# PeihaoChen/WS-MGMap

Measured on AMD Instinct MI355X. Metric: policy steps/sec (fwd+bwd), CMA batch=8 seq=64, higher is better.
Workload: dtype bf16

## Files before the change

include/wsmgmap.h:

```cpp
#ifndef WSMGMAP_H
#define WSMGMAP_H

#include <stdint.h>

#ifdef __cplusplus
extern "C" {
#endif

typedef void* wsmg_stream_t;

#define WSMG_EINVAL (-1)
#define WSMG_ENOMEM (-2)

int wsmg_abi_version(void);
const char* wsmg_build_info(void);


int wsmg_bev_index(const float* depth, int B, int Hd, int Wd, float depth_scale, int Hf, int Wf, int E,
                   float local_scale, int32_t* lin_idx, wsmg_stream_t stream);

int wsmg_bev_scatter_max(const float* feat, const int32_t* lin_idx, int B, int Cf, int Hf, int Wf, int C,
                         int E, float* out, wsmg_stream_t stream);

int wsmg_bev_rotate(const float* in, const float* heading, float sign, int B, int C, int E, float* out,
                    wsmg_stream_t stream);

int wsmg_map_fuse(const float* ego_rot, float* global_map, const float* gps, const float* masks, int B,
                  int C, int E, int G, float resolution, wsmg_stream_t stream);

int wsmg_bev_scatter_rotate(const float* feat, const int32_t* lin_idx, const float* heading, float sign, int B, int Cf, int Hf,
                            int Wf, int C, int E, float* out_planes, wsmg_stream_t stream);
int wsmg_bev_index_compact(const float* depth, int B, int Hd, int Wd, float depth_scale, int Hf, int Wf, int E, float local_scale,
                           int32_t* lin_idx, uint32_t* clist, int32_t* cnt, wsmg_stream_t stream);
int wsmg_bev_scatter_rotate_compact(const float* feat, const uint32_t* clist, const int32_t* cnt, const float* heading, float sign, int B,
                                    int Cf, int Hf, int Wf, int C, int E, float* out_planes, wsmg_stream_t stream);
int wsmg_map_fuse_planes(const float* ego_rot_planes, float* global_map, const float* gps, const float* masks, int B, int C,
                         int E, int G, float resolution, wsmg_stream_t stream);

int wsmg_map_retrieve(const float* global_map, const float* gps, const float* compass, int B, int C, int E,
                      int G, float resolution, float* scratch, float* out, wsmg_stream_t stream);
int wsmg_map_retrieve_fused(const float* global_map, const float* gps, const float* compass, int B, int C, int E, int G,
                            float resolution, float* out, wsmg_stream_t stream);
int wsmg_map_retrieve_tiled(const float* global_map, const float* gps, const float* compass, int B, int C, int E, int G,
                            float resolution, float* out, wsmg_stream_t stream);

int wsmg_bev_project(const float* depth, const float* feat, const float* heading, float sign, int B, int Hd, int Wd, float depth_scale,
                     int Cf, int Hf, int Wf, int C, int E, float local_scale, int32_t* lin_idx , float* out_planes,
                     wsmg_stream_t stream);
int wsmg_map_fuse_retrieve(const float* ego_rot_planes, float* global_map, const float* gps, const float* compass,
                           const float* masks, int B, int C, int E, int G, float resolution, float* out, wsmg_stream_t stream);

int wsmg_conv2d_fwd(const float* x, const float* w_ohwi, const float* bias, float* y, int B, int H, int W,
                    int Cin, int Cout, int KH, int KW, int stride, int pad, int OH, int OW,
                    wsmg_stream_t stream);

int wsmg_conv2d_bwd_data(const float* dy, const float* w_ihwo, float* dx, int B, int H, int W, int Cin,
                         int Cout, int KH, int KW, int stride, int pad, int OH, int OW,
                         wsmg_stream_t stream);

int wsmg_conv2d_bwd_weight(const float* x, const float* dy, float* dw_ohwi, int B, int H, int W, int Cin,
                           int Cout, int KH, int KW, int stride, int pad, int OH, int OW,
                           wsmg_stream_t stream);

int wsmg_channel_sum(const float* x, int64_t rows, int C, float* out, double* workspace,
                     int64_t workspace_bytes, wsmg_stream_t stream);
int64_t wsmg_channel_reduce_workspace_bytes(int64_t rows, int C);

int wsmg_bn_act_fwd(const float* x, const float* residual, const float* gamma, const float* beta,
                    float* running_mean, float* running_var, float momentum, float eps, int train,
                    int relu, int64_t rows, int C, float* y, float* save_mean, float* save_invstd,
                    double* workspace, int64_t workspace_bytes, wsmg_stream_t stream);

int wsmg_bn_act_bwd(const float* dy, const float* x, const float* y, const float* gamma, const float* beta,
                    const float* save_mean, const float* save_invstd, int relu, int64_t rows, int C,
                    float* dx, float* dresidual, float* dgamma, float* dbeta, double* workspace,
                    int64_t workspace_bytes, wsmg_stream_t stream);

int wsmg_add3_bf16(const void* a, const void* b, const void* c, void* y, int64_t n, wsmg_stream_t stream);

int wsmg_relu_fwd(const float* x, float* y, int64_t n, wsmg_stream_t stream);
int wsmg_token_grad_merge(float* dx, const float* x, const float* g, int B, int I, int C, int relu, wsmg_stream_t stream);
int wsmg_relu_bwd(const float* dy, const float* y, float* dx, int64_t n, wsmg_stream_t stream);
int wsmg_maxpool3x3s2_fwd(const float* x, float* y, int B, int H, int W, int C, int OH, int OW,
                          wsmg_stream_t stream);
int wsmg_maxpool3x3s2_bwd(const float* dy, const float* x, float* dx, int B, int H, int W, int C, int OH,
                          int OW, wsmg_stream_t stream);
int wsmg_upsample2x_fwd(const float* x, float* y, int B, int H, int W, int C, wsmg_stream_t stream);
int wsmg_upsample2x_bwd(const float* dy, float* dx, int B, int H, int W, int C, wsmg_stream_t stream);
int wsmg_avgpool2_fwd(const float* x, float* y, int B, int H, int W, int C, wsmg_stream_t stream);
int wsmg_avgpool2_bwd(const float* dy, float* dx, int B, int H, int W, int C, wsmg_stream_t stream);

int wsmg_nchw_to_nhwc(const float* x, float* y, int B, int C_src, int H, int W, int C_dst,
                      wsmg_stream_t stream);
int wsmg_nhwc_to_nchw(const float* x, float* y, int B, int C_src, int H, int W, int C_dst,
                      wsmg_stream_t stream);

int wsmg_attn_fwd(const float* q, const float* k, const float* v, const uint8_t* mask, float scale, int B,
                  int I, int C, float* out, float* attn, wsmg_stream_t stream);

int wsmg_attn_bwd(const float* q, const float* k, const float* v, const float* attn, const float* dout,
                  const float* dattn, float scale, int B, int I, int C, float* dq, float* dk, float* dv,
                  wsmg_stream_t stream);

int wsmg_conv2d_fwd_bf16(const void* x, const void* w_ohwi, const float* bias, void* y, int out_f32, int B, int H,
                         int W, int Cin, int Cout, int KH, int KW, int stride, int pad, int OH, int OW,
                         wsmg_stream_t stream);
int wsmg_conv2d_splitk_plan(int B, int OH, int OW, int Cin, int Cout, int KH, int KW, int* ksplit, long long* part_floats);
int wsmg_conv2d_fwd_bf16_splitk(const void* x, const void* w_ohwi, const float* bias, void* y, int flags, int ksplit,
                                float* part, int B, int H, int W, int Cin, int Cout, int KH, int KW, int stride, int pad,
                                int OH, int OW, wsmg_stream_t stream);
int wsmg_conv_transpose2d_infer_bf16(const void* x, const void* w_ihwo, const float* bias, void* y, int flags, int B, int H, int W,
                                     int Cin, int Cout, int KH, int KW, int stride, int pad, int OH, int OW, wsmg_stream_t stream);
int wsmg_conv2d_bwd_data_bf16(const void* dy, const void* w_ihwo, void* dx, int out_f32, int B, int H, int W,
                              int Cin, int Cout, int KH, int KW, int stride, int pad, int OH, int OW,
                              wsmg_stream_t stream);
int wsmg_conv2d_fwd_bf16_stats(const void* x, const void* w_ohwi, const float* bias, void* y, int out_f32, double* stats,
                               int nslab, int B, int H, int W, int Cin, int Cout, int KH, int KW, int stride, int pad, int OH,
                               int OW, wsmg_stream_t stream);
int wsmg_conv2d_bwd_data_bf16_stats(const void* dy, const void* w_ihwo, void* dx, int out_f32, double* stats, int nslab, int B,
                                    int H, int W, int Cin, int Cout, int KH, int KW, int stride, int pad, int OH, int OW,
                                    wsmg_stream_t stream);
int wsmg_conv2d_bwd_data_bf16_ex(const void* dy, const void* w_ihwo, void* dx, const void* relu_y, void* dx2, int split_c, int B, int H,
                                 int W, int Cin, int Cout, int KH, int KW, int stride, int pad, int OH, int OW, wsmg_stream_t stream);
int wsmg_conv2d_fwd_bf16_ex(const void* x, const void* w_ohwi, const float* bias, void* y, int flags, double* stats, int nslab, int y_ld,
                            int B, int H, int W, int Cin, int Cout, int KH, int KW, int stride, int pad, int OH, int OW,
                            wsmg_stream_t stream);
typedef struct {
  const float* x;
  float* out;
  int rows, cols;
} WsmgColsumDesc;
int wsmg_colsum_multi(const WsmgColsumDesc* descs, int n, wsmg_stream_t stream);
typedef struct {
  void* dst;
  const void* src;
  long long bytes;
} WsmgCopyDesc;
int wsmg_copy_multi(const WsmgCopyDesc* descs, int n, wsmg_stream_t stream);
int wsmg_copy_multi_guarded(const WsmgCopyDesc* descs, int n, const float* guard, wsmg_stream_t stream);
int wsmg_linear_rows(const float* x, const float* w, const float* bias, float* y, int B, int K, int O, int act, int pool,
                     wsmg_stream_t stream);
int wsmg_act_heads(const float* feat, int B, int K, const float* w_prog, const float* b_prog, const float* w_mean,
                   const float* b_mean, const float* logstd, int A, const float* w_crit, const float* b_crit, const float* noise,
                   float* prog, float* value, float* action, float* logp, wsmg_stream_t stream);
int wsmg_path_kl_fwd(const float* dis, const float* lo, const float* hi, const float* att, int B, int H, int W, int S, float tau,
                     float* target, float* kl, wsmg_stream_t stream);
int wsmg_path_kl_bwd(const float* gkl, const float* target, const float* att, int B, int n, float* datt, wsmg_stream_t stream);

typedef struct {
  float* param;
  const float* grad;
  float* exp_avg;
  float* exp_avg_sq;
  long long n;
} WsmgAdamDesc;
int wsmg_adam_step_multi(const WsmgAdamDesc* descs, int n, float lr, float beta1, float beta2, float eps, float weight_decay,
                         double bias_correction1, double bias_correction2, wsmg_stream_t stream);
int wsmg_adam_step_multi_dev(const WsmgAdamDesc* descs, int n, float lr, float beta1, float beta2, float eps, float weight_decay,
                             const float* step_dev, wsmg_stream_t stream);
int wsmg_grad_norm_multi(const WsmgAdamDesc* descs, int n, double* partials, long long partials_cap, float max_norm,
                         int skip_nonfinite, float* guard, float* step_dev, wsmg_stream_t stream);
int wsmg_adam_step_multi_guarded(const WsmgAdamDesc* descs, int n, float lr, float beta1, float beta2, float eps, float weight_decay,
                                 const float* step_dev, const float* guard, wsmg_stream_t stream);

int wsmg_conv_debug_win3_tile(int mt);
int wsmg_bn_act_fwd_bf16_pre(const void* x, const void* residual, const float* gamma, const float* beta, float* running_mean,
                             float* running_var, float momentum, float eps, int relu, int64_t rows, int C, void* y,
                             float* save_mean, float* save_invstd, double* stats, int nslab, wsmg_stream_t stream);
int wsmg_conv2d_bwd_weight_bf16(const void* x, const void* dy, float* dw_ohwi, int B, int H, int W, int Cin,
                                int Cout, int KH, int KW, int stride, int pad, int OH, int OW,
                                wsmg_stream_t stream);
int wsmg_channel_sum_bf16(const void* x, int64_t rows, int C, float* out, double* workspace,
                          int64_t workspace_bytes, wsmg_stream_t stream);
int wsmg_bn_act_fwd_bf16(const void* x, const void* residual, const float* gamma, const float* beta,
                         float* running_mean, float* running_var, float momentum, float eps, int train,
                         int relu, int64_t rows, int C, void* y, float* save_mean, float* save_invstd,
                         double* workspace, int64_t workspace_bytes, wsmg_stream_t stream);
int wsmg_bn_act_bwd_bf16(const void* dy, const void* x, const void* y, const float* gamma, const float* beta,
                         const float* save_mean, const float* save_invstd, int relu, int64_t rows, int C,
                         void* dx, void* dresidual, float* dgamma, float* dbeta, double* workspace,
                         int64_t workspace_bytes, wsmg_stream_t stream);
int wsmg_relu_fwd_bf16(const void* x, void* y, int64_t n, wsmg_stream_t stream);
int wsmg_token_grad_merge_bf16(void* dx, const void* x, const float* g, int B, int I, int C, int relu, wsmg_stream_t stream);
int wsmg_relu_bwd_bf16(const void* dy, const void* y, void* dx, int64_t n, wsmg_stream_t stream);
int wsmg_maxpool3x3s2_fwd_bf16(const void* x, void* y, int B, int H, int W, int C, int OH, int OW,
                               wsmg_stream_t stream);
int wsmg_maxpool3x3s2_bwd_bf16(const void* dy, const void* x, void* dx, int B, int H, int W, int C, int OH,
                               int OW, wsmg_stream_t stream);
int wsmg_maxpool3x3s2_fwd_idx_bf16(const void* x, void* y, uint32_t* idx, int B, int H, int W, int C, int OH, int OW, wsmg_stream_t stream);
int wsmg_maxpool3x3s2_bwd_idx_bf16(const void* dy, const uint32_t* idx, void* dx, int B, int H, int W, int C, int OH, int OW,
                                   wsmg_stream_t stream);
int wsmg_upsample2x_fwd_bf16(const void* x, void* y, int B, int H, int W, int C, wsmg_stream_t stream);
int wsmg_upsample2x_bwd_bf16(const void* dy, void* dx, int B, int H, int W, int C, wsmg_stream_t stream);
int wsmg_avgpool2_fwd_bf16(const void* x, void* y, int B, int H, int W, int C, wsmg_stream_t stream);
int wsmg_avgpool2_bwd_bf16(const void* dy, void* dx, int B, int H, int W, int C, wsmg_stream_t stream);
int wsmg_nchw_to_nhwc_bf16(const float* x, void* y, int B, int C_src, int H, int W, int C_dst,
                           wsmg_stream_t stream);
int wsmg_nhwc_to_nchw_bf16(const void* x, float* y, int B, int C_src, int H, int W, int C_dst,
                           wsmg_stream_t stream);
int wsmg_attn_fwd_bf16(const float* q, const void* k, const void* v, const uint8_t* mask, float scale, int B,
                       int I, int C, float* out, float* attn, wsmg_stream_t stream);
int wsmg_attn_bwd_bf16(const float* q, const void* k, const void* v, const float* attn, const float* dout,
                       const float* dattn, float scale, int B, int I, int C, float* dq, void* dk, void* dv,
                       wsmg_stream_t stream);

int wsmg_attn_shared_fwd(const float* q, const float* k_sets, const float* v_sets, const uint8_t* mask_sets,
                         const int64_t* row_index, float scale, int B, int I, int C, float* out, float* attn,
                         wsmg_stream_t stream);
int wsmg_attn_shared_bwd(const float* q, const float* k_sets, const float* v_sets, const float* attn, const float* dout,
                         const float* dattn, const int64_t* row_index, float scale, int B, int I, int C, float* dq,
                         float* dlogits, wsmg_stream_t stream);
int wsmg_attn_shared_fwd_bf16(const float* q, const void* k_sets, const void* v_sets, const uint8_t* mask_sets,
                              const int64_t* row_index, float scale, int B, int I, int C, float* out, float* attn,
                              wsmg_stream_t stream);
int wsmg_attn_shared_bwd_bf16(const float* q, const void* k_sets, const void* v_sets, const float* attn, const float* dout,
                              const float* dattn, const int64_t* row_index, float scale, int B, int I, int C, float* dq,
                              float* dlogits, wsmg_stream_t stream);

int wsmg_attn_fp8_row_fwd(const float* q, const float* w_k, const uint8_t* x_e4m3, const float* x_scale, const int* lengths,
                          float scale, int B, int L, int C, float* q_folded, float* out, float* attn, wsmg_stream_t stream);
int wsmg_attn_fp8_fold(const float* in, const float* w, int B, int C, int transpose, float* out, wsmg_stream_t stream);
int wsmg_attn_fp8_splits(int B, int L);
int64_t wsmg_attn_fp8_workspace_bytes(int B, int L);
int wsmg_attn_fp8_fwd(const float* q_folded, const uint8_t* x_e4m3, const float* x_scale, const int* lengths, float scale, int B,
                      int L, int C, float* out, float* attn, void* workspace, unsigned* ticket, wsmg_stream_t stream);
int wsmg_attn_fp8_bwd(const float* q_folded, const uint8_t* x_e4m3, const float* x_scale, const float* attn, const float* dout,
                      const float* dattn, float scale, int B, int L, int C, float* dq_folded, float* dx, wsmg_stream_t stream);
int wsmg_quantize_e4m3_dev(const float* x, int64_t n, const float* scale, uint8_t* y, wsmg_stream_t stream);
int wsmg_quantize_e4m3(const float* x, int64_t n, float inv_scale, uint8_t* y, wsmg_stream_t stream);

#define WSMG_RELAYOUT_MAX 32
typedef struct {
  const float* w_oihw;
  void* w_ohwi;
  void* w_ihwo;
  int O, I, KH, KW, I_pad, reserved;
} WsmgRelayoutDesc;
int wsmg_weight_relayout_multi(const WsmgRelayoutDesc* descs, int n, int bf16, wsmg_stream_t stream);
int wsmg_weight_relayout(const float* w_oihw, int O, int I, int KH, int KW, int I_pad, float* w_ohwi, float* w_ihwo,
                         wsmg_stream_t stream);
int wsmg_weight_relayout_bf16(const float* w_oihw, int O, int I, int KH, int KW, int I_pad, void* w_ohwi, void* w_ihwo,
                              wsmg_stream_t stream);
int wsmg_weight_grad_to_oihw(const float* dw_ohwi, int O, int I, int KH, int KW, int I_pad, float* dw_oihw,
                             wsmg_stream_t stream);

int wsmg_conv2d_bwd_weight_bf16_plan(int B, int H, int W, int Cin, int Cout, int KH, int KW, int stride, int pad, int OH, int OW,
                                     int* nsplit, long long* ws_floats);
int wsmg_conv2d_bwd_weight_bf16_slabs(const void* x, const void* dy, float* ws, int nsplit, long long ws_floats, int B, int H, int W,
                                      int Cin, int Cout, int KH, int KW, int stride, int pad, int OH, int OW, wsmg_stream_t stream);
int wsmg_conv2d_bwd_weight_plan(int B, int H, int W, int Cin, int Cout, int KH, int KW, int stride, int pad, int OH, int OW,
                                int* nsplit, long long* ws_floats);
int wsmg_conv2d_bwd_weight_slabs(const float* x, const float* dy, float* ws, int nsplit, long long ws_floats, int B, int H, int W,
                                 int Cin, int Cout, int KH, int KW, int stride, int pad, int OH, int OW, wsmg_stream_t stream);
int wsmg_weight_grad_reduce_oihw(const float* ws, int nsplit, int O, int I, int KH, int KW, int I_pad, float* dw_oihw,
                                 wsmg_stream_t stream);

int wsmg_bn_act_bwd_ld(const float* dy, int64_t ld_dy, const float* x, const float* y, const float* gamma, const float* beta,
                       const float* save_mean, const float* save_invstd, int relu, int64_t rows, int C, float* dx, float* dresidual,
                       float* dgamma, float* dbeta, double* workspace, int64_t workspace_bytes, wsmg_stream_t stream);
int wsmg_bn_act_bwd_ld_bf16(const void* dy, int64_t ld_dy, const void* x, const void* y, const float* gamma, const float* beta,
                            const float* save_mean, const float* save_invstd, int relu, int64_t rows, int C, void* dx,
                            void* dresidual, float* dgamma, float* dbeta, double* workspace, int64_t workspace_bytes,
                            wsmg_stream_t stream);
int wsmg_bn_act_bwd_ld_bf16_lo(const void* dy, int64_t ld_dy, const void* x, const void* y, const float* gamma, const float* beta,
                               const float* save_mean, const float* save_invstd, int relu, int64_t rows, int C, void* dx, void* dx_lo,
                               void* dresidual, float* dgamma, float* dbeta, double* workspace, int64_t workspace_bytes,
                               wsmg_stream_t stream);
int wsmg_relu_bwd_rows_bf16(const void* dy, int64_t ld_dy, const void* y, void* dx, int64_t rows, int C, wsmg_stream_t stream);
int wsmg_upsample2x_bwd_ld(const float* dy, int64_t ld_dy, float* dx, int B, int H, int W, int C, wsmg_stream_t stream);
int wsmg_upsample2x_bwd_ld_bf16(const void* dy, int64_t ld_dy, void* dx, int B, int H, int W, int C, wsmg_stream_t stream);
int wsmg_cat_channels(const void* a, const void* b, void* y, int64_t rows, int bytes_a, int bytes_b, wsmg_stream_t stream);
int wsmg_upsample2x_cat_bf16(const void* a, const void* b, void* y, int B, int H, int W, int Ca, int Cb, wsmg_stream_t stream);

int wsmg_ce_nhwc_fwd(const float* logits, const int64_t* target, int64_t rows, int classes, float* loss, wsmg_stream_t stream);
int wsmg_ce_nhwc_bwd(const float* logits, const int64_t* target, const float* gloss, int64_t rows, int classes,
                     float* dlogits, wsmg_stream_t stream);
int wsmg_ce_nhwc_fwd_bf16(const void* logits, const int64_t* target, int64_t rows, int classes, float* loss, wsmg_stream_t stream);
int wsmg_ce_nhwc_bwd_bf16(const void* logits, const int64_t* target, const float* gloss, int64_t rows, int classes,
                          void* dlogits, wsmg_stream_t stream);

int wsmg_collate_pad(const void* const* src, const int* lengths, int N, int T, int64_t elems, int src_dtype,
                     float pad, float* dst, wsmg_stream_t stream);
int wsmg_collate_pad_nhwc_bf16(const void* const* src, const int* lengths, int N, int T, int C, int HW, float pad, void* dst,
                               wsmg_stream_t stream);
int wsmg_collate_ego_sparse_nhwc_bf16(const void* const* bits, const void* const* off, const void* const* base,
                                      const void* const* vals, const int* lengths, int N, int T, int C, int HW, float pad,
                                      void* dst, wsmg_stream_t stream);
int wsmg_ego_sparse_pack(const float* x, int B, int C, int HW, uint8_t* bits, uint32_t* off, int64_t* nnz, void* vals,
                         wsmg_stream_t stream);

int64_t wsmg_gru_workspace_bytes(int T);
int wsmg_gru_fwd(const float* gi, const float* w_hh, const float* b_hh, const float* h0, const float* masks,
                 int T, int N, int hidden, float* y, float* save_r, float* save_z, float* save_n,
                 float* save_ghn, void* sync_ws, wsmg_stream_t stream);
int wsmg_gru_bwd(const float* dy, const float* dhT, const float* w_hh, const float* h0, const float* masks,
                 const float* y, const float* save_r, const float* save_z, const float* save_n,
                 const float* save_ghn, int T, int N, int hidden, float* dgi, float* dgh, float* dh0,
                 void* sync_ws, wsmg_stream_t stream);
int wsmg_gru_fwd_owned(const float* gi, const float* w_hh, const float* b_hh, const float* h0, const float* masks,
                       int T, int N, int hidden, float* y, float* save_r, float* save_z, float* save_n,
                       float* save_ghn, void* sync_ws, wsmg_stream_t stream);
int wsmg_gru_bwd_owned(const float* dy, const float* dhT, const float* w_hh, const float* h0, const float* masks,
                       const float* y, const float* save_r, const float* save_z, const float* save_n, const float* save_ghn,
                       int T, int N, int hidden, float* dgi, float* dgh, float* dh0, void* sync_ws, wsmg_stream_t stream);

int64_t wsmg_lstm_state_workspace_bytes(int T);
int wsmg_lstm_state_fwd(const float* gi, const float* w_hh, const float* b_hh, const float* h0, const float* c0,
                        const float* masks, int T, int N, int hidden, float* y, float* c_T, float* save_gates,
                        float* save_c, void* sync_ws, wsmg_stream_t stream);
int wsmg_lstm_state_bwd(const float* dy, const float* dhT, const float* dcT, const float* w_hh, const float* c0,
                        const float* masks, const float* save_gates, const float* save_c, int T, int N, int hidden,
                        float* dgates, float* dh0, float* dc0, void* sync_ws, wsmg_stream_t stream);

#define WSMG_CELL_LSTM 0
#define WSMG_CELL_GRU 1
int64_t wsmg_instr_rnn_workspace_bytes(int cell, int hidden, int dirs, int L);
int wsmg_instr_rnn_fwd(int cell, const float* gi, const float* w_hh, const float* b_hh, const int32_t* lengths, int U, int L,
                       int hidden, int dirs, float* out, float* save_gates, float* save_c, void* state_ws,
                       wsmg_stream_t stream);
int wsmg_instr_rnn_bwd(int cell, const float* dout, const float* w_hh, const int32_t* lengths, const float* out,
                       const float* save_gates, const float* save_c, int U, int L, int hidden, int dirs, float* dgi,
                       float* dgh, void* state_ws, wsmg_stream_t stream);
int64_t wsmg_lstm_workspace_bytes(int L);
int wsmg_lstm_fwd(const float* gi, const float* w_hh, const float* b_hh, const int32_t* lengths, int U, int L,
                  int hidden, float* out, float* save_gates, float* save_c, void* state_ws,
                  wsmg_stream_t stream);
int wsmg_lstm_bwd(const float* dout, const float* w_hh, const int32_t* lengths, const float* save_gates,
                  const float* save_c, int U, int L, int hidden, float* dgates, void* state_ws,
                  wsmg_stream_t stream);

int wsmg_group_norm_nhwc_bf16(const void* x, int x_f32, const void* residual, const float* gamma, const float* beta, int B,
                              int HW, int C, int G, float eps, int relu, void* y, wsmg_stream_t stream);

int wsmg_rnn_status(int clear);
int wsmg_rnn_debug_inject(unsigned bits);
int wsmg_gru_fwd_chain(const float* gi, const float* w_hh, const float* b_hh, const float* h0, const float* masks,
                       int T, int N, int hidden, float* y, float* save_r, float* save_z, float* save_n,
                       float* save_ghn, void* sync_ws, int steps_per_chunk, const unsigned* in_count, unsigned in_target,
                       unsigned* out_count, wsmg_stream_t stream);
int wsmg_gru_bwd_chain(const float* dy, const float* dhT, const float* w_hh, const float* h0, const float* masks,
                       const float* y, const float* save_r, const float* save_z, const float* save_n,
                       const float* save_ghn, int T, int N, int hidden, float* dgi, float* dgh, float* dh0,
                       void* sync_ws, int steps_per_chunk, const unsigned* in_count, unsigned in_target, unsigned* out_count,
                       wsmg_stream_t stream);
int wsmg_gru_chain_workgroups(void);
int wsmg_lstm_state_fwd_chain(const float* gi, const float* w_hh, const float* b_hh, const float* h0, const float* c0,
                              const float* masks, int T, int N, int hidden, float* y, float* c_T, float* save_gates,
                              float* save_c, void* sync_ws, int steps_per_chunk, const unsigned* in_count, unsigned in_target,
                              unsigned* out_count, wsmg_stream_t stream);
int wsmg_lstm_state_bwd_chain(const float* dy, const float* dhT, const float* dcT, const float* w_hh, const float* c0,
                              const float* masks, const float* save_gates, const float* save_c, int T, int N, int hidden,
                              float* dgates, float* dh0, float* dc0, void* sync_ws, int steps_per_chunk, const unsigned* in_count,
                              unsigned in_target, unsigned* out_count, wsmg_stream_t stream);
int wsmg_lstm_state_chain_workgroups(void);
int wsmg_rnn_debug_spin_limit(unsigned limit);

int wsmg_update_heads_fwd(const float* x, const float* wm, const float* bm, const float* wp, const float* bp, const float* progress,
                          int B, int K, int A, float* pred, float* prog, float* prog_rows, wsmg_stream_t stream);
int wsmg_update_heads_bwd(const float* x, const float* wm, const float* wp, const float* prog, const float* progress,
                          const float* dpred, const float* dprog, const float* dprog_rows, int B, int K, int A, float* dx, float* dwm,
                          float* dbm, float* dwp, float* dbp, wsmg_stream_t stream);
int wsmg_aux_reduce_fwd(const float* const* rows, const float* alpha, int L, const unsigned char* mask, int B, float* out2,
                        wsmg_stream_t stream);
int wsmg_aux_reduce_bwd(const float* alpha, int L, const unsigned char* mask, const float* nsel, const float* daux, int B,
                        float* drows, wsmg_stream_t stream);
int wsmg_dagger_loss_fwd(const float* pred, const float* waypoint, int ld_waypoint, const float* weights, const float* aux, int T,
                         int N, int A, float* out2, float* den, wsmg_stream_t stream);
int wsmg_dagger_loss_bwd(const float* pred, const float* waypoint, int ld_waypoint, const float* weights, const float* den,
                         const float* dloss, int T, int N, int A, float* dpred, wsmg_stream_t stream);

long long wsmg_cls_tail_workspace_floats(int B);
int wsmg_cls_tail_fwd_bf16(const void* y2, const float* gamma, const float* beta, const float* mean, const float* invstd,
                           const float* w6, const float* b6, int classes, const float* gt, int Hg, int Wg, int B, int H, int W,
                           void* sem, void* pooled, float* ce_rows, wsmg_stream_t stream);
int wsmg_cls_tail_bwd_bf16(const void* y2, const float* gamma, const float* beta, const float* mean, const float* invstd,
                           const float* w6, const float* b6, int classes, const float* gt, int Hg, int Wg, const float* g_rows,
                           const void* dpooled, int B, int H, int W, void* dbn, float* workspace, long long workspace_floats,
                           float* dgamma, float* dbeta, float* dw6, float* db6, wsmg_stream_t stream);
int wsmg_bn_stats_finalize(double* stats, int nslab, int C, int64_t rows, float momentum, float eps, float* running_mean,
                           float* running_var, float* save_mean, float* save_invstd, wsmg_stream_t stream);
int wsmg_bn_bwd_apply_bf16(const void* dy, const void* x, const float* gamma, const float* mean, const float* invstd,
                           const float* dgamma, const float* dbeta, int64_t rows, int C, void* dx, wsmg_stream_t stream);

int wsmg_attn_fp8_mfma_fwd(const uint8_t* q_codes, const float* q_scale, const uint8_t* k_codes, const float* k_scale,
                           const uint8_t* v_codes, const float* v_scale, const int* lengths, const int* row_ids,
                           const int* set_start, float scale, int B, int U, int L, int C, float* out, float* attn,
                           wsmg_stream_t stream);

int wsmg_attn_fp8_mfma_bwd(const uint8_t* q_codes, const float* q_scale, const uint8_t* k_codes, const float* k_scale,
                           const uint8_t* v_codes, const float* v_scale, const int* row_ids, const int* set_start,
                           const int64_t* inverse, const float* attn, const float* dout, const float* dattn, float scale, int B, int U,
                           int L, int C, float* dq, float* dk, float* dv, float* dl_scratch, wsmg_stream_t stream);

int wsmg_attn_fp8_prep(const float* q, const float* k_sets, const float* v_sets, const int64_t* inverse, int B, int U, int L, int C,
                       float q_scale, float k_scale, float v_scale, uint8_t* q_codes, uint8_t* k_codes, uint8_t* v_codes,
                       float* scales, int* row_ids, int* set_start, unsigned* amax_ws, wsmg_stream_t stream);

int wsmg_attn_fp8_mfma_fused(const float* q, const float* k_sets, const float* v_sets, const int64_t* inverse, const int* lengths,
                             float q_scale, float k_scale, float v_scale, float scale, int B, int U, int L, int C,
                             unsigned* workspace, unsigned arrivals_before, int epoch, float* scales_out, float* out, float* attn,
                             wsmg_stream_t stream);
int wsmg_attn_fp8_mfma_fused_arrivals(int B, int U, int L, int C);

int wsmg_mean_rows(const float* x, int64_t R, int n, float* out, wsmg_stream_t stream);

int wsmg_instruction_dedup(const void* tokens, int is_f32, int B, int L, long long* uniq, long long* inverse, long long* meta,
                           wsmg_stream_t stream);

int wsmg_rows_gemm_f32(const float* a0, int lda0, int ka0, const float* a1, int lda1, int ka1, const float* a2, int lda2, int ka2,
                       const float* w, int ldw, int w_is_kn, const float* bias, const float* mask, int ldmask, int relu,
                       float* c0, int ldc0, int nc0, float* c1, int ldc1, int nc1, float* c2, int ldc2, int nc2,
                       const float* cin0, int ldcin0, const float* cin1, int ldcin1, const float* cin2, int ldcin2,
                       int M, const unsigned* wait_count, unsigned wait_target, unsigned* signal_count, int fail_bit,
                       unsigned* gate_word, wsmg_stream_t stream);
int wsmg_rows_gemm_supported(int K);
int wsmg_rows_gemm_workgroups(int M, int N);

int wsmg_debug_occupy(int n_workgroups, int lds_bytes, int max_ms, const int* stop_flag, unsigned* arrived, wsmg_stream_t stream);

#ifdef __cplusplus
}
#endif
#endif
```

ws-mgmap_amd/csrc/wsmg_conv_bf16.hip:

```cpp
#include <stdlib.h>

#include "wsmg_common.h"
#include "wsmg_relu_mask.h"

namespace {

typedef __bf16 bf16_t;
typedef short bf16x8 __attribute__((ext_vector_type(8)));
typedef short bf16x4 __attribute__((ext_vector_type(4)));
typedef unsigned int u32x4 __attribute__((ext_vector_type(4)));

constexpr int BM = 128;

__device__ __forceinline__ int xcd_swizzle(int bid, int nb) {
  const int q = nb >> 3, r = nb & 7, x = bid & 7;
  return x * q + (x < r ? x : r) + (bid >> 3);
}

__device__ __forceinline__ unsigned short f2bf_bits(float f) {
  bf16_t b = (bf16_t)f;
  return __builtin_bit_cast(unsigned short, b);
}

__device__ __forceinline__ __amdgpu_buffer_rsrc_t make_rsrc(const void* p, unsigned bytes) {
  return __builtin_amdgcn_make_buffer_rsrc(const_cast<void*>(p), 0, (int)bytes, 0x00020000);
}
__device__ __forceinline__ u32x4 buf_load16(__amdgpu_buffer_rsrc_t r, int byte_off) {
  return __builtin_amdgcn_raw_buffer_load_b128(r, byte_off, 0, 0);
}

struct ConvArgsB {
  const bf16_t* src;
  const bf16_t* wt;
  const float* bias;
  void* dst;
  int B, SH, SW, Kc, TH, TW, N, KH, KW, stride, pad;
  int mtiles, ntiles;
  int out_f32;
  unsigned src_bytes, wt_bytes;
  double* stats;
  int nslab;
  int ksplit;
  float* part;
  int dst_ld;
  const bf16_t* relu_z;
  void* dst2;
  int split_c;
};

template <bool BWD, int BN, int BK, int PF, bool SPLIT = false>
__global__ __launch_bounds__(256) void conv_igemm_bf16_kernel(ConvArgsB a) {
  constexpr int LDB = BK * 2 + 16;
  constexpr int SEGS = BK / 8;
  constexpr int RPP = 256 / SEGS;
  constexpr int APASS = BM / RPP;
  constexpr int BPASS = BN / RPP;
  constexpr int NT = BN / 64;
  constexpr int OPITCH = BN * 2 + 16;
  constexpr int SMEM = (BM + BN) * LDB > BM * OPITCH ? (BM + BN) * LDB : BM * OPITCH;
  __shared__ __attribute__((aligned(16))) unsigned char smem[SMEM];
  unsigned char* const As = smem;
  unsigned char* const Bs = smem + BM * LDB;
  __shared__ int dpix[BM];
  const int tid = threadIdx.x;
  const int lane = tid & 63, wave = tid >> 6;
  const int tiles = a.mtiles * a.ntiles;
  const int swz = xcd_swizzle(blockIdx.x, gridDim.x);
  const int split = SPLIT ? swz / tiles : 0;
  const int logical = SPLIT ? swz - split * tiles : swz;
  const int m0 = (logical / a.ntiles) * BM, n0 = (logical % a.ntiles) * BN;
  const int seg = tid % SEGS;
  const int lrow = tid / SEGS;

  int cy = 0, cx = 0, ty0 = 0, tx0 = 0, tstep = 1, THc = a.TH, TWc = a.TW, KHc = a.KH, KWc = a.KW;
  if (BWD && a.stride == 2) {
    cy = blockIdx.y >> 1; cx = blockIdx.y & 1;
    ty0 = (cy + a.pad) & 1; tx0 = (cx + a.pad) & 1;
    tstep = 2;
    THc = (a.TH - ty0 + 1) >> 1; TWc = (a.TW - tx0 + 1) >> 1;
    KHc = (a.KH - cy + 1) >> 1; KWc = (a.KW - cx + 1) >> 1;
  }
  const int Mc = a.B * THc * TWc;
  if (m0 >= Mc) return;

  const int sg = BWD ? -1 : 1;
  int roff[APASS];
  unsigned ymask[APASS], xmask[APASS];
  int rb_ = (m0 + lrow) / (THc * TWc);
  int ry_, rx_;
  {
    const int r0 = (m0 + lrow) - rb_ * (THc * TWc);
    ry_ = r0 / TWc;
    rx_ = r0 - ry_ * TWc;
  }
#pragma unroll
  for (int i = 0; i < APASS; ++i) {
    int m = m0 + lrow + RPP * i;
    bool pv = m < Mc;
    const int b = pv ? rb_ : 0, iy = pv ? ry_ : 0, ix = pv ? rx_ : 0;
    rx_ += RPP;
    while (rx_ >= TWc) { rx_ -= TWc; ++ry_; }
    while (ry_ >= THc) { ry_ -= THc; ++rb_; }
    int ty = ty0 + iy * tstep, tx = tx0 + ix * tstep;
    int py, px;
    if (BWD) {
      py = (a.stride == 2) ? ((ty + a.pad - cy) >> 1) : ty + a.pad;
      px = (a.stride == 2) ? ((tx + a.pad - cx) >> 1) : tx + a.pad;
    } else {
      py = ty * a.stride - a.pad;
      px = tx * a.stride - a.pad;
    }
    auto tapmask = [&](int p, int S_, int n) -> unsigned {
      int lo = BWD ? p - (S_ - 1) : -p, hi = BWD ? p : S_ - 1 - p;
      lo = lo < 0 ? 0 : lo;
      hi = hi > n - 1 ? n - 1 : hi;
      return hi >= lo ? ((2u << hi) - 1u) & ~((1u << lo) - 1u) : 0u;
    };
    const unsigned ym = tapmask(py, a.SH, KHc), xm = tapmask(px, a.SW, KWc);
    ymask[i] = pv ? ym : 0u;
    xmask[i] = xm;
    roff[i] = ((b * a.SH + py) * a.SW + px) * a.Kc + seg * 8;
    if (seg == 0) dpix[lrow + RPP * i] = pv ? (b * a.TH + ty) * a.TW + tx : -1;
  }
  const int taps = a.KH * a.KW;
  int woff[BPASS];
#pragma unroll
  for (int i = 0; i < BPASS; ++i) {
    int n = n0 + lrow + RPP * i;
    woff[i] = n < a.N ? n * taps * a.Kc + seg * 8 : -0x40000000;
  }
  const int kchunks = a.Kc / BK;
  const int all_steps = KHc * KWc * kchunks;
  const int per_split = SPLIT ? (all_steps + a.ksplit - 1) / a.ksplit : all_steps;
  const int step_begin = split * per_split;
  const int steps = SPLIT ? (all_steps - step_begin < per_split ? all_steps - step_begin : per_split) : all_steps;
  const __amdgpu_buffer_rsrc_t rs_src = make_rsrc(a.src, a.src_bytes);
  const __amdgpu_buffer_rsrc_t rs_wt = make_rsrc(a.wt, a.wt_bytes);

  int it_ch = 0, it_ay = 0, it_ax = 0, it_left = steps;
  if (SPLIT) {
    const int tp = KHc * KWc;
    it_ch = step_begin / tp;
    const int rem = step_begin - it_ch * tp;
    it_ay = rem / KWc;
    it_ax = rem - it_ay * KWc;
  }
  u32x4 ra[PF][APASS], rb[PF][BPASS];
  auto gload = [&](u32x4 (&ra)[APASS], u32x4 (&rb)[BPASS]) {
    const int ky = BWD ? cy + it_ay * tstep : it_ay, kx = BWD ? cx + it_ax * tstep : it_ax;
    const int sdelta = sg * (it_ay * a.SW + it_ax) * a.Kc + it_ch * BK;
    const bool more = SPLIT ? it_left > 0 : it_ch < kchunks;
    if (SPLIT) --it_left;
    const int wdelta = more ? (ky * a.KW + kx) * a.Kc + it_ch * BK : -0x20000000;
    const unsigned live = more ? 1u : 0u;
#pragma unroll
    for (int i = 0; i < APASS; ++i) {
      bool ok = ((ymask[i] >> it_ay) & (xmask[i] >> it_ax) & live) != 0;
      ra[i] = buf_load16(rs_src, ok ? (roff[i] + sdelta) * 2 : -1);
    }
#pragma unroll
    for (int i = 0; i < BPASS; ++i) rb[i] = buf_load16(rs_wt, (woff[i] + wdelta) * 2);
    if (++it_ax == KWc) { it_ax = 0; if (++it_ay == KHc) { it_ay = 0; ++it_ch; } }
  };
  auto lstore = [&](const u32x4 (&ra)[APASS], const u32x4 (&rb)[BPASS]) {
#pragma unroll
    for (int i = 0; i < APASS; ++i) *reinterpret_cast<u32x4*>(&As[(lrow + RPP * i) * LDB + seg * 16]) = ra[i];
#pragma unroll
    for (int i = 0; i < BPASS; ++i) *reinterpret_cast<u32x4*>(&Bs[(lrow + RPP * i) * LDB + seg * 16]) = rb[i];
  };

  const int wm = (wave & 1) * 64, wn = (wave >> 1) * (BN / 2);
  const int r = lane & 31, h = lane >> 5;
  f32x16 acc[2][NT];
#pragma unroll
  for (int t = 0; t < 2; ++t)
#pragma unroll
    for (int u = 0; u < NT; ++u)
#pragma unroll
      for (int i = 0; i < 16; ++i) acc[t][u][i] = 0.f;

  gload(ra[0], rb[0]);
  lstore(ra[0], rb[0]);
  __syncthreads();
#pragma unroll
  for (int j = 1; j < PF; ++j) gload(ra[j], rb[j]);
  for (int step0 = 0; step0 < steps; step0 += PF) {
#pragma unroll
    for (int j = 0; j < PF; ++j) {
      gload(ra[j], rb[j]);
#pragma unroll
      for (int ks = 0; ks < BK / 16; ++ks) {
        bf16x8 af[2], bf[NT];
#pragma unroll
        for (int t = 0; t < 2; ++t)
          af[t] = *reinterpret_cast<const bf16x8*>(&As[(wm + 32 * t + r) * LDB + ks * 32 + h * 16]);
#pragma unroll
        for (int u = 0; u < NT; ++u)
          bf[u] = *reinterpret_cast<const bf16x8*>(&Bs[(wn + 32 * u + r) * LDB + ks * 32 + h * 16]);
#pragma unroll
        for (int t = 0; t < 2; ++t)
#pragma unroll
          for (int u = 0; u < NT; ++u)
            acc[t][u] = __builtin_amdgcn_mfma_f32_32x32x16_bf16(af[t], bf[u], acc[t][u], 0, 0, 0);
      }
      __syncthreads();
      lstore(ra[(j + 1) % PF], rb[(j + 1) % PF]);
      __syncthreads();
    }
  }

  if (SPLIT) {
    float* const mine = a.part + (size_t)split * Mc * a.N;
#pragma unroll
    for (int u = 0; u < NT; ++u) {
      const int n = n0 + wn + 32 * u + r;
      if (n >= a.N) continue;
#pragma unroll
      for (int t = 0; t < 2; ++t)
#pragma unroll
        for (int g = 0; g < 16; ++g) {
          const int m = m0 + wm + 32 * t + (g & 3) + 8 * (g >> 2) + 4 * h;
          if (m < Mc) mine[(size_t)m * a.N + n] = acc[t][u][g];
        }
    }
    return;
  }

  constexpr int OP = OPITCH;
  {
    if ((a.out_f32 & 1) == 0 && (a.N & 7) == 0) {
      const bool relu_here = (a.out_f32 & 6) == 2;
#pragma unroll
      for (int u = 0; u < NT; ++u) {
        const int col = wn + 32 * u + r;
        const float bv = (a.bias && n0 + col < a.N) ? a.bias[n0 + col] : 0.f;
        float sv = 0.f, qv = 0.f;
#pragma unroll
        for (int t = 0; t < 2; ++t)
#pragma unroll
          for (int g = 0; g < 16; ++g) {
            const int row = wm + 32 * t + (g & 3) + 8 * (g >> 2) + 4 * h;
            float v = acc[t][u][g] + bv;
            if (relu_here) v = v > 0.f ? v : 0.f;
            const unsigned short o = f2bf_bits(v);
            *reinterpret_cast<unsigned short*>(smem + row * OP + col * 2) = o;
            if (a.stats) {
              const float vr = m0 + row < Mc ? __uint_as_float((unsigned)o << 16) : 0.f;
              sv += vr;
              qv = fmaf(vr, vr, qv);
            }
          }
        if (a.stats) {
          sv += __shfl_xor(sv, 32, 64);
          qv += __shfl_xor(qv, 32, 64);
          if (h == 0 && n0 + col < a.N) {
            double* st = a.stats + (size_t)((logical / a.ntiles) % a.nslab) * 2 * a.N + n0 + col;
            atomicAdd(st, (double)sv);
            atomicAdd(st + a.N, (double)qv);
          }
        }
      }
      __syncthreads();
      constexpr int CPR = BN / 8;
      const int ldd = a.dst_ld ? a.dst_ld : a.N;
      constexpr int ROWS = BM * CPR / 256;
      u32x4 zr[ROWS];
      if (a.relu_z) {
#pragma unroll
        for (int j = 0; j < ROWS; ++j) {
          const int c = tid + 256 * j;
          const int row = c / CPR, ch = c - row * CPR;
          const int dp = dpix[row];
          const int n = n0 + ch * 8;
          zr[j] = (dp >= 0 && n < a.N) ? *reinterpret_cast<const u32x4*>(a.relu_z + (size_t)dp * a.N + n) : u32x4{0u, 0u, 0u, 0u};
        }
      }
#pragma unroll
      for (int j = 0; j < BM * CPR / 256; ++j) {
        const int c = tid + 256 * j;
        const int row = c / CPR, ch = c - row * CPR;
        const int dp = dpix[row];
        const int n = n0 + ch * 8;
        if (dp < 0 || n >= a.N) continue;
        u32x4* out = reinterpret_cast<u32x4*>(reinterpret_cast<unsigned char*>(a.dst) + ((size_t)dp * ldd + n) * 2);
        if (a.dst2) {
          const bool hi = n >= a.split_c;
          out = reinterpret_cast<u32x4*>(reinterpret_cast<unsigned char*>(hi ? a.dst2 : a.dst) +
                                         ((size_t)dp * (hi ? a.N - a.split_c : a.split_c) + (hi ? n - a.split_c : n)) * 2);
        }
        u32x4 v = *reinterpret_cast<const u32x4*>(smem + row * OP + ch * 16);
        if (a.relu_z) v = relu_mask8(v, zr[j]);
        if (a.out_f32 & 4) {
          const u32x4 old = *out;
#pragma unroll
          for (int q = 0; q < 4; ++q) {
            float lo = __uint_as_float(v[q] << 16) + __uint_as_float(old[q] << 16);
            float hi = __uint_as_float(v[q] & 0xffff0000u) + __uint_as_float(old[q] & 0xffff0000u);
            if (a.out_f32 & 2) { lo = lo > 0.f ? lo : 0.f; hi = hi > 0.f ? hi : 0.f; }
            v[q] = (unsigned)f2bf_bits(lo) | ((unsigned)f2bf_bits(hi) << 16);
          }
        }
        *out = v;
      }
      return;
    }
  }
#pragma unroll
  for (int u = 0; u < NT; ++u) {
    const int n = n0 + wn + 32 * u + r;
    if (n >= a.N) continue;
    const float bv = a.bias ? a.bias[n] : 0.f;
#pragma unroll
    for (int t = 0; t < 2; ++t) {
#pragma unroll
      for (int g = 0; g < 16; ++g) {
        int row = wm + 32 * t + (g & 3) + 8 * (g >> 2) + 4 * h;
        int dp = dpix[row];
        if (dp < 0) continue;
        float v = acc[t][u][g] + bv;
        if (a.out_f32 & 4) {
          const size_t o = (size_t)dp * a.N + n;
          v += (a.out_f32 & 1) ? reinterpret_cast<const float*>(a.dst)[o]
                               : __uint_as_float((unsigned)reinterpret_cast<const unsigned short*>(a.dst)[o] << 16);
        }
        if (a.out_f32 & 2) v = v > 0.f ? v : 0.f;
        if (a.out_f32 & 1)
          reinterpret_cast<float*>(a.dst)[(size_t)dp * a.N + n] = v;
        else
          reinterpret_cast<unsigned short*>(a.dst)[(size_t)dp * a.N + n] = f2bf_bits(v);
      }
    }
  }
}

constexpr int WKP = 64;
constexpr int X_LD = 64;

struct WgradArgsB {
  const bf16_t* x;
  const bf16_t* dy;
  float* dw;
  int B, H, W, Cin, Cout, KH, KW, stride, pad, OH, OW;
  int units;
  int64_t npix, chunk;
  unsigned x_bytes, dy_bytes;
  int gx, gy;
  int64_t slab;
};

__device__ __forceinline__ bf16x4 tr_read(const unsigned char* p) {
  return __builtin_amdgcn_ds_read_tr16_b64_v4i16((bf16x4 __attribute__((address_space(3)))*)(p));
}

template <int TC, int TU, int PF, int UPT>
__global__ __launch_bounds__(256) void conv_wgrad_bf16_kernel(WgradArgsB a) {
  constexpr int WCO = 32 * TC;
  constexpr int WUN = 4 * TU;
  constexpr int NG = WUN / UPT;
  constexpr int D_LD = TC == 4 ? 320 : 192;
  constexpr int DSEG = 4 * TC;
  constexpr int DROWS = 256 / DSEG;
  __shared__ __attribute__((aligned(16))) unsigned char Ds[WKP * D_LD];
  __shared__ __attribute__((aligned(16))) unsigned char Xs[WUN * WKP * X_LD];
  const int tid = threadIdx.x;
  const int lane = tid & 63, wave = tid >> 6;
  const int logical = xcd_swizzle(blockIdx.x, gridDim.x);
  const int gxy = a.gx * a.gy;
  const int bz = logical / gxy, bxy = logical - bz * gxy;
  const int u0 = (bxy % a.gx) * WUN;
  const int co0 = (bxy / a.gx) * WCO;
  const int64_t p_begin = (int64_t)bz * a.chunk;
  int64_t p_end = p_begin + a.chunk;
  if (p_end > a.npix) p_end = a.npix;
  const int cchunks = a.Cin / 32;
  const int ohw = a.OH * a.OW;

  int gky[NG], gkx[NG], gci[NG];
  bool gok[NG];
#pragma unroll
  for (int g = 0; g < NG; ++g) {
    int uu = u0 + g * UPT;
    gok[g] = uu < a.units;
    int t = gok[g] ? uu / cchunks : 0;
    gci[g] = gok[g] ? (uu - t * cchunks) * 32 : 0;
    gky[g] = t / a.KW;
    gkx[g] = t - gky[g] * a.KW;
  }
  const int dpx = tid / DSEG, dseg = tid % DSEG;
  const int xpx = tid >> 2, xseg = tid & 3;

  f32x16 acc[TC][TU];
#pragma unroll
  for (int t = 0; t < TC; ++t)
#pragma unroll
    for (int u = 0; u < TU; ++u)
#pragma unroll
      for (int i = 0; i < 16; ++i) acc[t][u][i] = 0.f;

  const __amdgpu_buffer_rsrc_t rs_x = make_rsrc(a.x, a.x_bytes);
  const __amdgpu_buffer_rsrc_t rs_dy = make_rsrc(a.dy, a.dy_bytes);
  const bool co_ok = (co0 + dseg * 8) < a.Cout;
  int gdelta[NG];
#pragma unroll
  for (int g = 0; g < NG; ++g) gdelta[g] = (gky[g] * a.W + gkx[g]) * a.Cin + gci[g] + xseg * 8;
  int it_b, it_oy, it_ox;
  {
    int64_t p = p_begin + xpx;
    if (p >= a.npix) p = a.npix - 1;
    it_b = (int)(p / ohw);
    int rem = (int)(p - (int64_t)it_b * ohw);
    it_oy = rem / a.OW;
    it_ox = rem - it_oy * a.OW;
  }
  const int adv_b = WKP / ohw, adv_rem = WKP - adv_b * ohw;
  const int adv_oy = adv_rem / a.OW, adv_ox = adv_rem - adv_oy * a.OW;
  int it_p = (int)p_begin;
  const int pend = (int)p_end;
  u32x4 rd[PF][TC], rx[PF][WUN];
  auto gload = [&](u32x4 (&rd)[TC], u32x4 (&rx)[WUN]) {
#pragma unroll
    for (int i = 0; i < TC; ++i) {
      int p = it_p + dpx + DROWS * i;
      bool ok = co_ok && p < pend;
      rd[i] = buf_load16(rs_dy, ok ? (p * a.Cout + co0 + dseg * 8) * 2 : -1);
    }
    const bool pok = (it_p + xpx) < pend;
    const int y0 = it_oy * a.stride - a.pad, x0 = it_ox * a.stride - a.pad;
    const int base = ((it_b * a.H + y0) * a.W + x0) * a.Cin;
#pragma unroll
    for (int g = 0; g < NG; ++g) {
      bool ok = pok && gok[g] && (unsigned)(y0 + gky[g]) < (unsigned)a.H && (unsigned)(x0 + gkx[g]) < (unsigned)a.W;
      const int off = ok ? (base + gdelta[g]) * 2 : (int)0x80000000;
#pragma unroll
      for (int j = 0; j < UPT; ++j) rx[g * UPT + j] = buf_load16(rs_x, off + 64 * j);
    }
    it_p += WKP;
    it_ox += adv_ox;
    if (it_ox >= a.OW) { it_ox -= a.OW; ++it_oy; }
    it_oy += adv_oy;
    if (it_oy >= a.OH) { it_oy -= a.OH; ++it_b; }
    it_b += adv_b;
  };
  auto lstore = [&](const u32x4 (&rd)[TC], const u32x4 (&rx)[WUN]) {
#pragma unroll
    for (int i = 0; i < TC; ++i) *reinterpret_cast<u32x4*>(&Ds[(dpx + DROWS * i) * D_LD + dseg * 16]) = rd[i];
#pragma unroll
    for (int u = 0; u < WUN; ++u) *reinterpret_cast<u32x4*>(&Xs[(u * WKP + xpx) * X_LD + xseg * 16]) = rx[u];
  };

  const int li = lane & 15, q = li >> 2, p4 = li & 3;
  const int half16 = (lane >> 4) & 1;
  const int h = lane >> 5;
  const unsigned char* a_base = &Ds[(8 * h + q) * D_LD + (half16 * 16 + p4 * 4) * 2];
  const unsigned char* b_base = &Xs[(wave * TU * WKP + 8 * h + q) * X_LD + (half16 * 16 + p4 * 4) * 2];

  gload(rd[0], rx[0]);
  lstore(rd[0], rx[0]);
  __syncthreads();
#pragma unroll
  for (int j = 1; j < PF; ++j) gload(rd[j], rx[j]);
  for (int64_t pb = p_begin; pb < p_end; pb += (int64_t)PF * WKP) {
#pragma unroll
    for (int j = 0; j < PF; ++j) {
      gload(rd[j], rx[j]);
#pragma unroll
      for (int ks = 0; ks < WKP / 16; ++ks) {
        bf16x8 af[TC], bfr[TU];
#pragma unroll
        for (int t = 0; t < TC; ++t) {
          bf16x4 l = tr_read(a_base + 64 * t + (16 * ks) * D_LD), hh = tr_read(a_base + 64 * t + (16 * ks + 4) * D_LD);
          af[t] = __builtin_shufflevector(l, hh, 0, 1, 2, 3, 4, 5, 6, 7);
        }
#pragma unroll
        for (int u = 0; u < TU; ++u) {
          const unsigned char* bp = b_base + u * WKP * X_LD;
          bf16x4 l = tr_read(bp + (16 * ks) * X_LD), hh = tr_read(bp + (16 * ks + 4) * X_LD);
          bfr[u] = __builtin_shufflevector(l, hh, 0, 1, 2, 3, 4, 5, 6, 7);
        }
#pragma unroll
        for (int u = 0; u < TU; ++u)
#pragma unroll
          for (int t = 0; t < TC; ++t) acc[t][u] = __builtin_amdgcn_mfma_f32_32x32x16_bf16(af[t], bfr[u], acc[t][u], 0, 0, 0);
      }
      __syncthreads();
      lstore(rd[(j + 1) % PF], rx[(j + 1) % PF]);
      __syncthreads();
    }
  }
  const int r = lane & 31;
  const int taps = a.KH * a.KW;
#pragma unroll
  for (int u = 0; u < TU; ++u) {
    const int uu = u0 + wave * TU + u;
    if (uu >= a.units) continue;
    const int tap = uu / cchunks;
    const int ci = (uu - tap * cchunks) * 32 + r;
#pragma unroll
    for (int t = 0; t < TC; ++t) {
#pragma unroll
      for (int g = 0; g < 16; ++g) {
        int co = co0 + 32 * t + (g & 3) + 8 * (g >> 2) + 4 * h;
        if (co < a.Cout) {
          float* const q = a.dw + (size_t)bz * a.slab + ((size_t)co * taps + tap) * a.Cin + ci;
          if (a.slab) *q = acc[t][u][g];
          else atomicAdd(q, acc[t][u][g]);
        }
      }
    }
  }
}

int check_conv(int B, int H, int W, int Cin, int Cout, int KH, int KW, int stride, int pad, int OH, int OW) {
  if (B <= 0 || H <= 0 || W <= 0 || Cin <= 0 || Cout <= 0 || KH <= 0 || KW <= 0) return WSMG_EINVAL;
  if (Cin % 32 || Cout % 32) return WSMG_EINVAL;
  if (stride != 1 && stride != 2) return WSMG_EINVAL;
  if (OH != (H + 2 * pad - KH) / stride + 1 || OW != (W + 2 * pad - KW) / stride + 1) return WSMG_EINVAL;
  if ((int64_t)B * H * W >= (1ll << 31) || (int64_t)B * OH * OW >= (1ll << 31)) return WSMG_EINVAL;
  if ((int64_t)B * H * W * Cin * 2 >= (1ll << 31) || (int64_t)B * OH * OW * Cout * 2 >= (1ll << 31)) return WSMG_EINVAL;
  return 0;
}


int g_win3_tile = -1;
int win3_tile() {
  if (g_win3_tile < 0) g_win3_tile = WSMG_TUNE("WSMG_CONV_WIN3", 1);
  return g_win3_tile;
}
bool k32_choice(int64_t M, int Kc, int N) {
  return win3_tile() == 1 && Kc == 32 && (N == 32 || N == 64 || N == 128) && M >= 2 * 256 * 256 && WSMG_TUNE("WSMG_CONV_K32", 1) != 0;
}
int win3_choice(int64_t M, int Kc, int N) {
  const int t = win3_tile();
  if (t == 0 || M < 256 * 256 || Kc % 32 || N % 32) return 0;
  if (N % 64) {
    const int n32 = WSMG_TUNE("WSMG_CONV_WIN3_N32", 256);
    if (t != 1) return t;
    if (n32 == 0 || M < 2 * 256 * 256) return 0;
    return n32;
  }
  if (Kc < 64) return 0;
  if (N % 128) {
    const int n64 = WSMG_TUNE("WSMG_CONV_WIN3_N64", 1);
    if (t != 1) return t;
    if (n64 == 0 || M < 2 * 256 * 256 || (Kc < 128 && N < 192)) return 0;
    return n64 == 1 ? 512 : n64;
  }
  if (t != 1) return t;
  if (M < 2 * 256 * 256) return 0;
  return ((M + 511) / 512) * (N / 128) >= 1024 ? 512 : 256;
}

template <bool BWD>
int launch_igemm(ConvArgsB& a, int64_t mrows, int classes, hipStream_t s) {
  const bool bk64 = (a.Kc % 64) == 0;
  const bool bn128 = a.N >= 128;
  const int bn = bn128 ? 128 : 64;
  a.mtiles = (int)wsmg_cdiv(mrows, BM);
  a.ntiles = (int)wsmg_cdiv(a.N, bn);
  dim3 grid((unsigned)(a.mtiles * a.ntiles), (unsigned)classes);
  if (bk64 && bn128)
    hipLaunchKernelGGL((conv_igemm_bf16_kernel<BWD, 128, 64, 1>), grid, dim3(256), 0, s, a);
  else if (bk64)
    hipLaunchKernelGGL((conv_igemm_bf16_kernel<BWD, 64, 64, 1>), grid, dim3(256), 0, s, a);
  else if (bn128)
    hipLaunchKernelGGL((conv_igemm_bf16_kernel<BWD, 128, 32, 1>), grid, dim3(256), 0, s, a);
  else
    hipLaunchKernelGGL((conv_igemm_bf16_kernel<BWD, 64, 32, 1>), grid, dim3(256), 0, s, a);
  return 0;
}

int splitk_plan(int64_t M, int Kc, int N, int KH, int KW) {
  const int bk = (Kc % 64) == 0 ? 64 : 32;
  const int steps = KH * KW * (Kc / bk);
  const int tiles = (int)(wsmg_cdiv(M, BM) * wsmg_cdiv(N, 64));
  const int target = 256, minsteps = 4, maxtiles = 128;
  if (tiles >= maxtiles || steps < 4 * minsteps || (N & 7)) return 1;
  int ks = (int)wsmg_cdiv(target, tiles);
  if (ks > steps / minsteps) ks = steps / minsteps;
  if (ks > 32) ks = 32;
  if (ks < 2) return 1;
  const int per = (int)wsmg_cdiv(steps, ks);
  return (int)wsmg_cdiv(steps, per);
}

__global__ __launch_bounds__(256) void splitk_finish_kernel(const float* __restrict__ part, const float* __restrict__ bias,
                                                            void* __restrict__ y, int64_t MN8, int N, int ksplit, int flags) {
  const int64_t i = (int64_t)blockIdx.x * 256 + threadIdx.x;
  if (i >= MN8) return;
  typedef float f32x4v __attribute__((ext_vector_type(4)));
  const int n = (int)((i * 8) % N);
  float v[8];
#pragma unroll
  for (int j = 0; j < 8; ++j) v[j] = 0.f;
  const f32x4v* p = reinterpret_cast<const f32x4v*>(part) + i * 2;
  for (int s = 0; s < ksplit; ++s, p += MN8 * 2) {
    const f32x4v a0 = p[0], a1 = p[1];
#pragma unroll
    for (int j = 0; j < 4; ++j) { v[j] += a0[j]; v[4 + j] += a1[j]; }
  }
  if (bias) {
#pragma unroll
    for (int j = 0; j < 8; ++j) v[j] += bias[n + j];
  }
  if (flags & 1) {
    f32x4v* o = reinterpret_cast<f32x4v*>(y) + i * 2;
    if (flags & 4) {
      const f32x4v a0 = o[0], a1 = o[1];
#pragma unroll
      for (int j = 0; j < 4; ++j) { v[j] += a0[j]; v[4 + j] += a1[j]; }
    }
    if (flags & 2) {
#pragma unroll
      for (int j = 0; j < 8; ++j) v[j] = v[j] > 0.f ? v[j] : 0.f;
    }
    o[0] = f32x4v{v[0], v[1], v[2], v[3]};
    o[1] = f32x4v{v[4], v[5], v[6], v[7]};
  } else {
    u32x4* o = reinterpret_cast<u32x4*>(y) + i;
    if (flags & 4) {
      const u32x4 old = *o;
#pragma unroll
      for (int j = 0; j < 4; ++j) {
        v[2 * j] += __uint_as_float(old[j] << 16);
        v[2 * j + 1] += __uint_as_float(old[j] & 0xffff0000u);
      }
    }
    u32x4 out;
#pragma unroll
    for (int j = 0; j < 4; ++j) {
      float lo = v[2 * j], hi = v[2 * j + 1];
      if (flags & 2) { lo = lo > 0.f ? lo : 0.f; hi = hi > 0.f ? hi : 0.f; }
      out[j] = (unsigned)f2bf_bits(lo) | ((unsigned)f2bf_bits(hi) << 16);
    }
    *o = out;
  }
}

}

extern "C" int wsmg_conv2d_splitk_plan(int B, int OH, int OW, int Cin, int Cout, int KH, int KW, int* ksplit,
                                       long long* part_floats) {
  if (!ksplit || !part_floats) return WSMG_EINVAL;
  *ksplit = splitk_plan((int64_t)B * OH * OW, Cin, Cout, KH, KW);
  *part_floats = (long long)*ksplit * B * OH * OW * Cout;
  return 0;
}

extern "C" int wsmg_conv2d_fwd_bf16_splitk(const void* x, const void* w_ohwi, const float* bias, void* y, int flags, int ksplit,
                                           float* part, int B, int H, int W, int Cin, int Cout, int KH, int KW,
                                           int stride, int pad, int OH, int OW, wsmg_stream_t stream) {
  if (int e = check_conv(B, H, W, Cin, Cout, KH, KW, stride, pad, OH, OW)) return e;
  const int64_t M = (int64_t)B * OH * OW;
  if (ksplit < 2 || ksplit != splitk_plan(M, Cin, Cout, KH, KW) || !part || (flags & ~7)) return WSMG_EINVAL;
  ConvArgsB a{(const bf16_t*)x, (const bf16_t*)w_ohwi, nullptr, y, B, H, W, Cin, OH, OW, Cout, KH, KW, stride, pad, 0, 0, flags,
              (unsigned)((size_t)B * H * W * Cin * 2), (unsigned)((size_t)Cout * KH * KW * Cin * 2), nullptr, 0, ksplit, part};
  a.mtiles = (int)wsmg_cdiv(M, BM);
  a.ntiles = (int)wsmg_cdiv(Cout, 64);
  dim3 grid((unsigned)(a.mtiles * a.ntiles * ksplit));
  if (Cin % 64 == 0)
    hipLaunchKernelGGL((conv_igemm_bf16_kernel<false, 64, 64, 1, true>), grid, dim3(256), 0, wsmg_s(stream), a);
  else
    hipLaunchKernelGGL((conv_igemm_bf16_kernel<false, 64, 32, 1, true>), grid, dim3(256), 0, wsmg_s(stream), a);
  const int64_t mn8 = M * Cout / 8;
  hipLaunchKernelGGL(splitk_finish_kernel, dim3((unsigned)wsmg_cdiv(mn8, 256)), dim3(256), 0, wsmg_s(stream), part, bias, y, mn8,
                     Cout, ksplit, flags);
  WSMG_RETURN_LAUNCH();
}

namespace {
int conv_fwd_bf16_impl(const void* x, const void* w_ohwi, const float* bias, void* y, int out_f32, double* stats, int nslab, int y_ld, int B, int H, int W, int Cin, int Cout, int KH, int KW, int stride, int pad,
                       int OH, int OW, wsmg_stream_t stream) {
  if (int e = check_conv(B, H, W, Cin, Cout, KH, KW, stride, pad, OH, OW)) return e;
  if (stats && (nslab <= 0 || (out_f32 & 5) != 0 || (Cout & 7) != 0)) return WSMG_EINVAL;
  const bool ex = y_ld && y_ld != Cout;
  if (ex) {
    if ((out_f32 & 5) != 0 || (Cout & 7) != 0) return WSMG_EINVAL;
    if (y_ld && (y_ld < Cout || (y_ld & 7) || ((uintptr_t)y & 15))) return WSMG_EINVAL;
    if ((int64_t)B * OH * OW * (y_ld ? y_ld : Cout) * 2 >= (1ll << 31)) return WSMG_EINVAL;
  }
  if (!ex && Cin == 64 && Cout == 64 && KH == 8 && KW == 8 && stride == 2 && pad == 3 && (out_f32 & 5) == 0) {
    if (WSMG_TUNE("WSMG_CONV_WIN", 1)) {
      int rc = wsmg_conv_win_fwd_bf16(x, w_ohwi, bias, y, (out_f32 & 2) != 0, stats, nslab, B, H, W, Cin, Cout, KH, KW, stride, pad, OH, OW, wsmg_s(stream));
      if (rc != WSMG_EINVAL) return rc;
    }
  }
  if (KH == 3 && KW == 3 && stride == 1 && pad == 1 && OH == H && OW == W && (out_f32 & 5) == 0) {
    if (k32_choice((int64_t)B * OH * OW, Cin, Cout)) {
      int rc = wsmg_conv_win3_k32_bf16(0, x, w_ohwi, bias, y, (out_f32 & 2) != 0, stats, nslab, B, H, W, Cout, y_ld, wsmg_s(stream));
      if (rc != WSMG_EINVAL) return rc;
    }
    if (const int mt = win3_choice((int64_t)B * OH * OW, Cin, Cout)) {
      int rc = wsmg_conv_win3_bf16(0, x, w_ohwi, bias, y, (out_f32 & 2) != 0, stats, nslab, B, H, W, Cin, Cout, mt, win3_tile() == 1, nullptr, y_ld, nullptr, 0, wsmg_s(stream));
      if (rc != WSMG_EINVAL) return rc;
    }
  }
  ConvArgsB a{(const bf16_t*)x, (const bf16_t*)w_ohwi, bias, y, B, H, W, Cin, OH, OW, Cout, KH, KW, stride, pad, 0, 0, out_f32,
              (unsigned)((size_t)B * H * W * Cin * 2), (unsigned)((size_t)Cout * KH * KW * Cin * 2), stats, nslab};
  a.dst_ld = y_ld;
  if (int e = launch_igemm<false>(a, (int64_t)B * OH * OW, 1, wsmg_s(stream))) return e;
  WSMG_RETURN_LAUNCH();
}
}

extern "C" int wsmg_conv2d_fwd_bf16_stats(const void* x, const void* w_ohwi, const float* bias, void* y, int out_f32,
                                          double* stats, int nslab, int B, int H, int W, int Cin, int Cout, int KH, int KW,
                                          int stride, int pad, int OH, int OW, wsmg_stream_t stream) {
  return conv_fwd_bf16_impl(x, w_ohwi, bias, y, out_f32, stats, nslab, 0, B, H, W, Cin, Cout, KH, KW, stride, pad, OH, OW, stream);
}

extern "C" int wsmg_conv2d_fwd_bf16_ex(const void* x, const void* w_ohwi, const float* bias, void* y, int flags, double* stats, int nslab,
                                       int y_ld, int B, int H, int W, int Cin, int Cout, int KH, int KW,
                                       int stride, int pad, int OH, int OW, wsmg_stream_t stream) {
  return conv_fwd_bf16_impl(x, w_ohwi, bias, y, flags, stats, nslab, y_ld, B, H, W, Cin, Cout, KH, KW, stride, pad, OH, OW, stream);
}

extern "C" int wsmg_conv_debug_win3_tile(int mt) {
  const int old = win3_tile();
  if (mt == 0 || mt == 1 || mt == 256 || mt == 512) g_win3_tile = mt;
  return old;
}

extern "C" int wsmg_conv2d_fwd_bf16(const void* x, const void* w_ohwi, const float* bias, void* y, int out_f32, int B,
                                    int H, int W, int Cin, int Cout, int KH, int KW, int stride, int pad, int OH,
                                    int OW, wsmg_stream_t stream) {
  return wsmg_conv2d_fwd_bf16_stats(x, w_ohwi, bias, y, out_f32, nullptr, 0, B, H, W, Cin, Cout, KH, KW, stride, pad, OH, OW, stream);
}

namespace {
int conv_bwd_data_bf16_impl(const void* dy, const void* w_ihwo, void* dx, int out_f32, double* stats, int nslab, const void* relu_y,
                            void* dx2, int split_c, int B, int H, int W, int Cin, int Cout, int KH, int KW, int stride, int pad, int OH,
                            int OW, wsmg_stream_t stream) {
  if (int e = check_conv(B, H, W, Cin, Cout, KH, KW, stride, pad, OH, OW)) return e;
  if (stats && (nslab <= 0 || (out_f32 & 5) != 0 || (Cin & 7) != 0)) return WSMG_EINVAL;
  if (relu_y && ((out_f32 & 5) != 0 || (Cin & 7) != 0 || ((uintptr_t)relu_y & 15))) return WSMG_EINVAL;
  if (dx2 && ((out_f32 & 5) != 0 || (Cin & 7) != 0 || split_c <= 0 || split_c >= Cin || (split_c & 7) || ((uintptr_t)dx2 & 15))) return WSMG_EINVAL;
  if (KH == 3 && KW == 3 && stride == 1 && pad == 1 && OH == H && OW == W && (out_f32 & 7) == 0) {
    if (!relu_y && !dx2 && k32_choice((int64_t)B * H * W, Cout, Cin)) {
      int rc = wsmg_conv_win3_k32_bf16(1, dy, w_ihwo, nullptr, dx, 0, stats, nslab, B, H, W, Cin, 0, wsmg_s(stream));
      if (rc != WSMG_EINVAL) return rc;
    }
    if (const int mt = win3_choice((int64_t)B * H * W, Cout, Cin)) {
      int rc = wsmg_conv_win3_bf16(1, dy, w_ihwo, nullptr, dx, 0, stats, nslab, B, H, W, Cout, Cin, mt, win3_tile() == 1, relu_y, 0, dx2, split_c, wsmg_s(stream));
      if (rc != WSMG_EINVAL) return rc;
    }
  }
  if (KH == 4 && KW == 4 && stride == 2 && pad == 1 && Cin == 32 && Cout == 64 && H == 2 * OH && W == 2 * OW && (out_f32 & 7) == 0 &&
      !relu_y && !dx2 && win3_tile() == 1 && (int64_t)B * OH * OW >= 2 * 256 * 256 && WSMG_TUNE("WSMG_CONVT_K4S2", 1) != 0) {
    int rc = wsmg_convt_k4s2_bf16(dy, w_ihwo, dx, stats, nslab, B, OH, OW, wsmg_s(stream));
    if (rc != WSMG_EINVAL) return rc;
  }
  ConvArgsB a{(const bf16_t*)dy, (const bf16_t*)w_ihwo, nullptr, dx, B, OH, OW, Cout, H, W, Cin, KH, KW, stride, pad, 0, 0, out_f32,
              (unsigned)((size_t)B * OH * OW * Cout * 2), (unsigned)((size_t)Cout * KH * KW * Cin * 2), stats, nslab};
  a.relu_z = (const bf16_t*)relu_y;
  a.dst2 = dx2;
  a.split_c = split_c;
  int classes = 1;
  int64_t mmax = (int64_t)B * H * W;
  if (stride == 2) {
    classes = 4;
    mmax = (int64_t)B * ((H + 1) / 2) * ((W + 1) / 2);
  }
  if (int e = launch_igemm<true>(a, mmax, classes, wsmg_s(stream))) return e;
  WSMG_RETURN_LAUNCH();
}
}

extern "C" int wsmg_conv2d_bwd_data_bf16_stats(const void* dy, const void* w_ihwo, void* dx, int out_f32, double* stats, int nslab,
                                               int B, int H, int W, int Cin, int Cout, int KH, int KW, int stride, int pad,
                                               int OH, int OW, wsmg_stream_t stream) {
  return conv_bwd_data_bf16_impl(dy, w_ihwo, dx, out_f32, stats, nslab, nullptr, nullptr, 0, B, H, W, Cin, Cout, KH, KW, stride, pad, OH, OW, stream);
}

extern "C" int wsmg_conv2d_bwd_data_bf16_ex(const void* dy, const void* w_ihwo, void* dx, const void* relu_y, void* dx2, int split_c,
                                            int B, int H, int W, int Cin, int Cout, int KH, int KW, int stride, int pad, int OH, int OW,
                                            wsmg_stream_t stream) {
  return conv_bwd_data_bf16_impl(dy, w_ihwo, dx, 0, nullptr, 0, relu_y, dx2, split_c, B, H, W, Cin, Cout, KH, KW, stride, pad, OH, OW, stream);
}

extern "C" int wsmg_conv_transpose2d_infer_bf16(const void* x, const void* w_ihwo, const float* bias, void* y, int flags, int B,
                                                int H, int W, int Cin, int Cout, int KH, int KW, int stride, int pad, int OH,
                                                int OW, wsmg_stream_t stream) {
  if (int e = check_conv(B, H, W, Cin, Cout, KH, KW, stride, pad, OH, OW)) return e;
  if (flags & ~3) return WSMG_EINVAL;
  ConvArgsB a{(const bf16_t*)x, (const bf16_t*)w_ihwo, bias, y, B, OH, OW, Cout, H, W, Cin, KH, KW, stride, pad, 0, 0, flags,
              (unsigned)((size_t)B * OH * OW * Cout * 2), (unsigned)((size_t)Cout * KH * KW * Cin * 2), nullptr, 0};
  int classes = 1;
  int64_t mmax = (int64_t)B * H * W;
  if (stride == 2) {
    classes = 4;
    mmax = (int64_t)B * ((H + 1) / 2) * ((W + 1) / 2);
  }
  launch_igemm<true>(a, mmax, classes, wsmg_s(stream));
  WSMG_RETURN_LAUNCH();
}

extern "C" int wsmg_conv2d_bwd_data_bf16(const void* dy, const void* w_ihwo, void* dx, int out_f32, int B, int H, int W,
                                         int Cin, int Cout, int KH, int KW, int stride, int pad, int OH, int OW,
                                         wsmg_stream_t stream) {
  return wsmg_conv2d_bwd_data_bf16_stats(dy, w_ihwo, dx, out_f32, nullptr, 0, B, H, W, Cin, Cout, KH, KW, stride, pad, OH, OW, stream);
}

namespace {
struct WgradPlan {
  int kind;
  int nsplit;
  int tc, tu, gx, gy;
  int64_t chunk;
};

WgradPlan wgrad_plan_bf16(int B, int H, int W, int Cin, int Cout, int KH, int KW, int stride, int pad, int OH, int OW) {
  WgradPlan p{0, 0, 0, 0, 0, 0, 0};
  if (WSMG_TUNE("WSMG_WGRAD_WIN", 1)) {
    if (const int n = wsmg_conv_win_wgrad_splits(B, H, W, Cin, Cout, KH, KW, stride, pad, OH, OW)) { p.kind = 1; p.nsplit = n; return p; }
  }
  if (const int n = wsmg_conv_s2_wgrad_splits(B, H, W, Cin, Cout, KH, KW, stride, pad, OH, OW)) { p.kind = 3; p.nsplit = n; return p; }
  const int use_w3w = WSMG_TUNE("WSMG_WGRAD_WIN3", 1);
  if (KH == 3 && KW == 3 && stride == 1 && pad == 1 && OH == H && OW == W && use_w3w && win3_tile() && (int64_t)B * H * W >= 256 * 256) {
    if (const int n = wsmg_conv_win3_wgrad_splits(B, H, W, Cin, Cout)) { p.kind = 2; p.nsplit = n; return p; }
  }
  const int units = KH * KW * (Cin / 32);
  const int64_t npix = (int64_t)B * OH * OW;
  int tc = (Cout % 128 == 0 && units >= 48) ? 4 : 2, tu = (tc == 4 || (Cin == 64 && units >= 128)) ? 2 : 1;
  const int gx = (int)wsmg_cdiv(units, 4 * tu), gy = (int)wsmg_cdiv(Cout, 32 * tc);
  const double gflop = 2.0 * (double)npix * Cout * Cin * KH * KW * 1e-9;
  int64_t target = tc == 4 ? 1024 : (gflop < 40.0 ? 768 : 2048);
  int64_t want = wsmg_cdiv(target, (int64_t)gx * gy);
  int64_t maxz = wsmg_cdiv(npix, WKP * 8);
  int64_t gz = want < 1 ? 1 : (want > maxz ? maxz : want);
  if (gz < 1) gz = 1;
  if (gz > 65535) gz = 65535;
  p.chunk = wsmg_cdiv(wsmg_cdiv(npix, gz), WKP) * WKP;
  p.nsplit = (int)wsmg_cdiv(npix, p.chunk);
  p.tc = tc; p.tu = tu; p.gx = gx; p.gy = gy;
  return p;
}

int launch_wgrad_bf16(const void* x, const void* dy, float* dw, long long slab_floats, int B, int H, int W, int Cin, int Cout, int KH,
                      int KW, int stride, int pad, int OH, int OW, hipStream_t stream) {
  const WgradPlan p = wgrad_plan_bf16(B, H, W, Cin, Cout, KH, KW, stride, pad, OH, OW);
  if (p.kind == 1) return wsmg_conv_win_wgrad_bf16(x, dy, dw, slab_floats, B, H, W, Cin, Cout, KH, KW, stride, pad, OH, OW, stream);
  if (p.kind == 2) return wsmg_conv_win3_wgrad_bf16(x, dy, dw, slab_floats, B, H, W, Cin, Cout, stream);
  if (p.kind == 3) return wsmg_conv_s2_wgrad_bf16(x, dy, dw, slab_floats, B, H, W, Cin, Cout, KH, KW, stride, pad, OH, OW, stream);
  WgradArgsB a{(const bf16_t*)x, (const bf16_t*)dy, dw, B, H, W, Cin, Cout, KH, KW, stride, pad, OH, OW, 0, 0, 0,
               (unsigned)((size_t)B * H * W * Cin * 2), (unsigned)((size_t)B * OH * OW * Cout * 2), 0, 0, (int64_t)slab_floats};
  a.units = KH * KW * (Cin / 32);
  a.npix = (int64_t)B * OH * OW;
  a.chunk = p.chunk;
  a.gx = p.gx;
  a.gy = p.gy;
  const int tc = p.tc, tu = p.tu;
  dim3 grid((unsigned)((int64_t)p.gx * p.gy * p.nsplit));
  const int cch = Cin / 32, wun = 4 * tu;
  int upt = 1;
  for (int c = wun; c > 1; c >>= 1)
    if (cch % c == 0) { upt = c; break; }
#define WSMG_WGRAD(TC_, TU_, UPT_) \
  hipLaunchKernelGGL((conv_wgrad_bf16_kernel<TC_, TU_, 1, UPT_>), grid, dim3(256), 0, stream, a)
#define WSMG_WGRAD_U4(TC_, TU_) \
  do { if (upt >= 4) WSMG_WGRAD(TC_, TU_, 4); else if (upt == 2) WSMG_WGRAD(TC_, TU_, 2); else WSMG_WGRAD(TC_, TU_, 1); } while (0)
  if (tc == 4) {
    if (upt == 8) WSMG_WGRAD(4, 2, 8); else WSMG_WGRAD_U4(4, 2);
  } else if (tu == 2) {
    if (upt != 2) return WSMG_EINVAL;
    WSMG_WGRAD(2, 2, 2);
  } else {
    WSMG_WGRAD_U4(2, 1);
  }
#undef WSMG_WGRAD_U4
#undef WSMG_WGRAD
  WSMG_RETURN_LAUNCH();
}
}

extern "C" int wsmg_conv2d_bwd_weight_bf16(const void* x, const void* dy, float* dw_ohwi, int B, int H, int W, int Cin,
                                           int Cout, int KH, int KW, int stride, int pad, int OH, int OW,
                                           wsmg_stream_t stream) {
  if (int e = check_conv(B, H, W, Cin, Cout, KH, KW, stride, pad, OH, OW)) return e;
  return launch_wgrad_bf16(x, dy, dw_ohwi, 0, B, H, W, Cin, Cout, KH, KW, stride, pad, OH, OW, wsmg_s(stream));
}

extern "C" int wsmg_conv2d_bwd_weight_bf16_plan(int B, int H, int W, int Cin, int Cout, int KH, int KW, int stride, int pad, int OH,
                                                int OW, int* nsplit, long long* ws_floats) {
  if (!nsplit || !ws_floats) return WSMG_EINVAL;
  if (int e = check_conv(B, H, W, Cin, Cout, KH, KW, stride, pad, OH, OW)) return e;
  const WgradPlan p = wgrad_plan_bf16(B, H, W, Cin, Cout, KH, KW, stride, pad, OH, OW);
  *nsplit = p.nsplit;
  *ws_floats = (long long)p.nsplit * Cout * KH * KW * Cin;
  return 0;
}

extern "C" int wsmg_conv2d_bwd_weight_bf16_slabs(const void* x, const void* dy, float* ws, int nsplit, long long ws_floats, int B, int H,
                                                 int W, int Cin, int Cout, int KH, int KW, int stride, int pad, int OH, int OW,
                                                 wsmg_stream_t stream) {
  if (int e = check_conv(B, H, W, Cin, Cout, KH, KW, stride, pad, OH, OW)) return e;
  const WgradPlan p = wgrad_plan_bf16(B, H, W, Cin, Cout, KH, KW, stride, pad, OH, OW);
  const long long slab = (long long)Cout * KH * KW * Cin;
  if (!ws || nsplit != p.nsplit || ws_floats < slab * p.nsplit) return WSMG_EINVAL;
  return launch_wgrad_bf16(x, dy, ws, slab, B, H, W, Cin, Cout, KH, KW, stride, pad, OH, OW, wsmg_s(stream));
}
```

ws-mgmap_amd/wsmgmap/_abi.py:

```python
import ctypes
import os

_HERE = os.path.dirname(os.path.abspath(__file__))
LIB_PATH = os.path.join(_HERE, "lib", "libwsmgmap.so")
if os.environ.get("WSMG_LIB"):
    LIB_PATH = os.environ["WSMG_LIB"]

c_p = ctypes.c_void_p
c_i = ctypes.c_int
c_l = ctypes.c_int64
c_f = ctypes.c_float


class WsmgError(RuntimeError):
    pass


class CopyDesc(ctypes.Structure):
    _fields_ = [("dst", ctypes.c_void_p), ("src", ctypes.c_void_p), ("bytes", ctypes.c_longlong)]


class RelayoutDesc(ctypes.Structure):
    _fields_ = [("w_oihw", c_p), ("w_ohwi", c_p), ("w_ihwo", c_p), ("O", c_i), ("I", c_i), ("KH", c_i), ("KW", c_i),
                ("I_pad", c_i), ("reserved", c_i)]


class ColsumDesc(ctypes.Structure):
    _fields_ = [("x", c_p), ("out", c_p), ("rows", c_i), ("cols", c_i)]


_SIG = {
    "wsmg_abi_version": [],
    "wsmg_build_info": [],
    "wsmg_bev_index": [c_p, c_i, c_i, c_i, c_f, c_i, c_i, c_i, c_f, c_p, c_p],
    "wsmg_bev_scatter_max": [c_p, c_p, c_i, c_i, c_i, c_i, c_i, c_i, c_p, c_p],
    "wsmg_bev_rotate": [c_p, c_p, c_f, c_i, c_i, c_i, c_p, c_p],
    "wsmg_map_fuse": [c_p, c_p, c_p, c_p, c_i, c_i, c_i, c_i, c_f, c_p],
    "wsmg_map_retrieve": [c_p, c_p, c_p, c_i, c_i, c_i, c_i, c_f, c_p, c_p, c_p],
    "wsmg_map_retrieve_fused": [c_p, c_p, c_p, c_i, c_i, c_i, c_i, c_f, c_p, c_p],
    "wsmg_map_retrieve_tiled": [c_p, c_p, c_p, c_i, c_i, c_i, c_i, c_f, c_p, c_p],
    "wsmg_bev_scatter_rotate": [c_p, c_p, c_p, c_f, c_i, c_i, c_i, c_i, c_i, c_i, c_p, c_p],
    "wsmg_map_fuse_planes": [c_p, c_p, c_p, c_p, c_i, c_i, c_i, c_i, c_f, c_p],
    "wsmg_conv2d_fwd": [c_p, c_p, c_p, c_p] + [c_i] * 11 + [c_p],
    "wsmg_conv2d_bwd_data": [c_p, c_p, c_p] + [c_i] * 11 + [c_p],
    "wsmg_conv2d_bwd_weight": [c_p, c_p, c_p] + [c_i] * 11 + [c_p],
    "wsmg_channel_sum": [c_p, c_l, c_i, c_p, c_p, c_l, c_p],
    "wsmg_channel_reduce_workspace_bytes": [c_l, c_i],
    "wsmg_bn_act_fwd": [c_p, c_p, c_p, c_p, c_p, c_p, c_f, c_f, c_i, c_i, c_l, c_i, c_p, c_p, c_p, c_p, c_l, c_p],
    "wsmg_bn_act_bwd": [c_p, c_p, c_p, c_p, c_p, c_p, c_p, c_i, c_l, c_i, c_p, c_p, c_p, c_p, c_p, c_l, c_p],
    "wsmg_relu_fwd": [c_p, c_p, c_l, c_p],
    "wsmg_relu_bwd": [c_p, c_p, c_p, c_l, c_p],
    "wsmg_token_grad_merge": [c_p, c_p, c_p, c_i, c_i, c_i, c_i, c_p],
    "wsmg_maxpool3x3s2_fwd": [c_p, c_p, c_i, c_i, c_i, c_i, c_i, c_i, c_p],
    "wsmg_maxpool3x3s2_bwd": [c_p, c_p, c_p, c_i, c_i, c_i, c_i, c_i, c_i, c_p],
    "wsmg_upsample2x_fwd": [c_p, c_p, c_i, c_i, c_i, c_i, c_p],
    "wsmg_upsample2x_bwd": [c_p, c_p, c_i, c_i, c_i, c_i, c_p],
    "wsmg_avgpool2_fwd": [c_p, c_p, c_i, c_i, c_i, c_i, c_p],
    "wsmg_avgpool2_bwd": [c_p, c_p, c_i, c_i, c_i, c_i, c_p],
    "wsmg_nchw_to_nhwc": [c_p, c_p, c_i, c_i, c_i, c_i, c_i, c_p],
    "wsmg_nhwc_to_nchw": [c_p, c_p, c_i, c_i, c_i, c_i, c_i, c_p],
    "wsmg_attn_fwd": [c_p, c_p, c_p, c_p, c_f, c_i, c_i, c_i, c_p, c_p, c_p],
    "wsmg_attn_bwd": [c_p, c_p, c_p, c_p, c_p, c_p, c_f, c_i, c_i, c_i, c_p, c_p, c_p, c_p],
}
for _n in ["wsmg_token_grad_merge", "wsmg_channel_sum", "wsmg_bn_act_fwd", "wsmg_bn_act_bwd", "wsmg_relu_fwd", "wsmg_relu_bwd",
           "wsmg_maxpool3x3s2_fwd", "wsmg_maxpool3x3s2_bwd", "wsmg_upsample2x_fwd", "wsmg_upsample2x_bwd",
           "wsmg_avgpool2_fwd", "wsmg_avgpool2_bwd", "wsmg_nchw_to_nhwc", "wsmg_nhwc_to_nchw", "wsmg_attn_fwd",
           "wsmg_attn_bwd", "wsmg_conv2d_bwd_weight"]:
    _SIG[_n + "_bf16"] = list(_SIG[_n])
_SIG["wsmg_conv2d_fwd_bf16"] = [c_p, c_p, c_p, c_p, c_i] + [c_i] * 11 + [c_p]
_SIG["wsmg_conv2d_bwd_data_bf16"] = [c_p, c_p, c_p, c_i] + [c_i] * 11 + [c_p]
_SIG["wsmg_conv_transpose2d_infer_bf16"] = [c_p, c_p, c_p, c_p, c_i] + [c_i] * 11 + [c_p]
_SIG["wsmg_conv2d_splitk_plan"] = [c_i] * 7 + [c_p, c_p]
_SIG["wsmg_conv2d_fwd_bf16_splitk"] = [c_p, c_p, c_p, c_p, c_i, c_i, c_p] + [c_i] * 11 + [c_p]
_SIG["wsmg_conv2d_fwd_bf16_stats"] = [c_p, c_p, c_p, c_p, c_i, c_p, c_i] + [c_i] * 11 + [c_p]
_SIG["wsmg_conv2d_bwd_data_bf16_stats"] = [c_p, c_p, c_p, c_i, c_p, c_i] + [c_i] * 11 + [c_p]
_SIG["wsmg_bn_act_fwd_bf16_pre"] = [c_p, c_p, c_p, c_p, c_p, c_p, c_f, c_f, c_i, c_l, c_i, c_p, c_p, c_p, c_p, c_i, c_p]
_SIG["wsmg_attn_shared_fwd"] = [c_p, c_p, c_p, c_p, c_p, c_f, c_i, c_i, c_i, c_p, c_p, c_p]
_SIG["wsmg_attn_shared_bwd"] = [c_p, c_p, c_p, c_p, c_p, c_p, c_p, c_f, c_i, c_i, c_i, c_p, c_p, c_p]
_SIG["wsmg_attn_shared_fwd_bf16"] = list(_SIG["wsmg_attn_shared_fwd"])
_SIG["wsmg_attn_shared_bwd_bf16"] = list(_SIG["wsmg_attn_shared_bwd"])
_SIG["wsmg_attn_fp8_fold"] = [c_p, c_p, c_i, c_i, c_i, c_p, c_p]
_SIG["wsmg_attn_fp8_splits"] = [c_i, c_i]
_SIG["wsmg_attn_fp8_workspace_bytes"] = [c_i, c_i]
_SIG["wsmg_attn_fp8_fwd"] = [c_p, c_p, c_p, c_p, c_f, c_i, c_i, c_i, c_p, c_p, c_p, c_p, c_p]
_SIG["wsmg_attn_fp8_bwd"] = [c_p, c_p, c_p, c_p, c_p, c_p, c_f, c_i, c_i, c_i, c_p, c_p, c_p]
_SIG["wsmg_quantize_e4m3_dev"] = [c_p, c_l, c_p, c_p, c_p]
_SIG["wsmg_quantize_e4m3"] = [c_p, c_l, c_f, c_p, c_p]
_SIG["wsmg_weight_relayout"] = [c_p, c_i, c_i, c_i, c_i, c_i, c_p, c_p, c_p]
_SIG["wsmg_weight_relayout_bf16"] = list(_SIG["wsmg_weight_relayout"])
_SIG["wsmg_weight_relayout_multi"] = [c_p, c_i, c_i, c_p]
_SIG["wsmg_weight_grad_to_oihw"] = [c_p, c_i, c_i, c_i, c_i, c_i, c_p, c_p]
_SIG["wsmg_conv2d_bwd_weight_plan"] = [c_i] * 11 + [c_p, c_p]
_SIG["wsmg_conv2d_bwd_weight_bf16_plan"] = list(_SIG["wsmg_conv2d_bwd_weight_plan"])
_SIG["wsmg_conv2d_bwd_weight_slabs"] = [c_p, c_p, c_p, c_i, c_l] + [c_i] * 11 + [c_p]
_SIG["wsmg_conv2d_bwd_weight_bf16_slabs"] = list(_SIG["wsmg_conv2d_bwd_weight_slabs"])
_SIG["wsmg_weight_grad_reduce_oihw"] = [c_p, c_i, c_i, c_i, c_i, c_i, c_i, c_p, c_p]
_SIG["wsmg_update_heads_fwd"] = [c_p] * 6 + [c_i] * 3 + [c_p] * 3 + [c_p]
_SIG["wsmg_update_heads_bwd"] = [c_p] * 8 + [c_i] * 3 + [c_p] * 5 + [c_p]
_SIG["wsmg_aux_reduce_fwd"] = [c_p, c_p, c_i, c_p, c_i, c_p, c_p]
_SIG["wsmg_aux_reduce_bwd"] = [c_p, c_i, c_p, c_p, c_p, c_i, c_p, c_p]
_SIG["wsmg_dagger_loss_fwd"] = [c_p, c_p, c_i, c_p, c_p, c_i, c_i, c_i, c_p, c_p, c_p]
_SIG["wsmg_dagger_loss_bwd"] = [c_p, c_p, c_i, c_p, c_p, c_p, c_i, c_i, c_i, c_p, c_p]
_SIG["wsmg_cls_tail_workspace_floats"] = [c_i]
_SIG["wsmg_cls_tail_fwd_bf16"] = [c_p] * 7 + [c_i, c_p, c_i, c_i, c_i, c_i, c_i, c_p, c_p, c_p, c_p]
_SIG["wsmg_cls_tail_bwd_bf16"] = [c_p] * 7 + [c_i, c_p, c_i, c_i, c_p, c_p, c_i, c_i, c_i, c_p, c_p, c_l, c_p, c_p, c_p, c_p, c_p]
_SIG["wsmg_bn_stats_finalize"] = [c_p, c_i, c_i, c_l, c_f, c_f, c_p, c_p, c_p, c_p, c_p]
_SIG["wsmg_bn_bwd_apply_bf16"] = [c_p] * 7 + [c_l, c_i, c_p, c_p]
_SIG["wsmg_attn_fp8_mfma_fwd"] = [c_p] * 9 + [c_f, c_i, c_i, c_i, c_i, c_p, c_p, c_p]
_SIG["wsmg_maxpool3x3s2_fwd_idx_bf16"] = [c_p, c_p, c_p, c_i, c_i, c_i, c_i, c_i, c_i, c_p]
_SIG["wsmg_maxpool3x3s2_bwd_idx_bf16"] = [c_p, c_p, c_p, c_i, c_i, c_i, c_i, c_i, c_i, c_p]
_SIG["wsmg_add3_bf16"] = [c_p, c_p, c_p, c_p, c_l, c_p]
_SIG["wsmg_attn_fp8_prep"] = [c_p] * 4 + [c_i, c_i, c_i, c_i, c_f, c_f, c_f] + [c_p] * 8
_SIG["wsmg_mean_rows"] = [c_p, c_l, c_i, c_p, c_p]
_SIG["wsmg_bn_act_bwd_ld"] = [c_p, c_l] + _SIG["wsmg_bn_act_bwd"][1:]
_SIG["wsmg_bn_act_bwd_ld_bf16"] = list(_SIG["wsmg_bn_act_bwd_ld"])
_SIG["wsmg_bn_act_bwd_ld_bf16_lo"] = [c_p, c_l] + [c_p] * 6 + [c_i, c_l, c_i] + [c_p] * 6 + [c_l, c_p]
_SIG["wsmg_upsample2x_bwd_ld"] = [c_p, c_l, c_p, c_i, c_i, c_i, c_i, c_p]
_SIG["wsmg_upsample2x_bwd_ld_bf16"] = list(_SIG["wsmg_upsample2x_bwd_ld"])
_SIG["wsmg_relu_bwd_rows_bf16"] = [c_p, c_l, c_p, c_p, c_l, c_i, c_p]
_SIG["wsmg_cat_channels"] = [c_p, c_p, c_p, c_l, c_i, c_i, c_p]
_SIG["wsmg_upsample2x_cat_bf16"] = [c_p, c_p, c_p, c_i, c_i, c_i, c_i, c_i, c_p]
_SIG["wsmg_ce_nhwc_fwd"] = [c_p, c_p, c_l, c_i, c_p, c_p]
_SIG["wsmg_ce_nhwc_bwd"] = [c_p, c_p, c_p, c_l, c_i, c_p, c_p]
_SIG["wsmg_ce_nhwc_fwd_bf16"] = list(_SIG["wsmg_ce_nhwc_fwd"])
_SIG["wsmg_ce_nhwc_bwd_bf16"] = list(_SIG["wsmg_ce_nhwc_bwd"])
_SIG["wsmg_collate_pad"] = [c_p, c_p, c_i, c_i, c_l, c_i, c_f, c_p, c_p]
_SIG["wsmg_collate_pad_nhwc_bf16"] = [c_p, c_p, c_i, c_i, c_i, c_i, c_f, c_p, c_p]
_SIG["wsmg_gru_workspace_bytes"] = [c_i]
_SIG["wsmg_gru_fwd"] = [c_p] * 5 + [c_i] * 3 + [c_p] * 6 + [c_p]
_SIG["wsmg_gru_bwd"] = [c_p] * 10 + [c_i] * 3 + [c_p] * 4 + [c_p]
_SIG["wsmg_gru_fwd_owned"] = list(_SIG["wsmg_gru_fwd"])
_SIG["wsmg_gru_bwd_owned"] = list(_SIG["wsmg_gru_bwd"])
_SIG["wsmg_lstm_state_workspace_bytes"] = [c_i]
_SIG["wsmg_lstm_state_fwd"] = [c_p] * 6 + [c_i] * 3 + [c_p] * 5 + [c_p]
_SIG["wsmg_lstm_state_bwd"] = [c_p] * 8 + [c_i] * 3 + [c_p] * 4 + [c_p]
_SIG["wsmg_lstm_workspace_bytes"] = [c_i]
_SIG["wsmg_lstm_fwd"] = [c_p] * 4 + [c_i] * 3 + [c_p] * 4 + [c_p]
_SIG["wsmg_lstm_bwd"] = [c_p] * 5 + [c_i] * 3 + [c_p] * 2 + [c_p]
_SIG["wsmg_instr_rnn_workspace_bytes"] = [c_i] * 4
_SIG["wsmg_instr_rnn_fwd"] = [c_i] + [c_p] * 4 + [c_i] * 4 + [c_p] * 4 + [c_p]
_SIG["wsmg_instr_rnn_bwd"] = [c_i] + [c_p] * 6 + [c_i] * 4 + [c_p] * 3 + [c_p]
_SIG["wsmg_group_norm_nhwc_bf16"] = [c_p, c_i, c_p, c_p, c_p, c_i, c_i, c_i, c_i, c_f, c_i, c_p, c_p]
_SIG["wsmg_rnn_status"] = [c_i]
_SIG["wsmg_rnn_debug_spin_limit"] = [ctypes.c_uint]
_SIG["wsmg_rnn_debug_inject"] = [ctypes.c_uint]
_SIG["wsmg_instruction_dedup"] = [c_p, c_i, c_i, c_i, c_p, c_p, c_p, c_p]
_SIG["wsmg_conv_debug_win3_tile"] = [c_i]
_SIG["wsmg_copy_multi"] = [c_p, c_i, c_p]
_SIG["wsmg_copy_multi_guarded"] = [c_p, c_i, c_p, c_p]
_SIG["wsmg_linear_rows"] = [c_p, c_p, c_p, c_p, c_i, c_i, c_i, c_i, c_i, c_p]
_SIG["wsmg_act_heads"] = [c_p, c_i, c_i, c_p, c_p, c_p, c_p, c_p, c_i, c_p, c_p, c_p, c_p, c_p, c_p, c_p, c_p]
_SIG["wsmg_path_kl_fwd"] = [c_p, c_p, c_p, c_p, c_i, c_i, c_i, c_i, c_f, c_p, c_p, c_p]
_SIG["wsmg_path_kl_bwd"] = [c_p, c_p, c_p, c_i, c_i, c_p, c_p]
_SIG["wsmg_adam_step_multi"] = [c_p, c_i, c_f, c_f, c_f, c_f, c_f, ctypes.c_double, ctypes.c_double, c_p]
_SIG["wsmg_adam_step_multi_dev"] = [c_p, c_i, c_f, c_f, c_f, c_f, c_f, c_p, c_p]
_SIG["wsmg_grad_norm_multi"] = [c_p, c_i, c_p, ctypes.c_longlong, c_f, c_i, c_p, c_p, c_p]
_SIG["wsmg_adam_step_multi_guarded"] = [c_p, c_i, c_f, c_f, c_f, c_f, c_f, c_p, c_p, c_p]
_SIG["wsmg_rows_gemm_f32"] = ([c_p, c_i, c_i] * 3 + [c_p, c_i, c_i, c_p, c_p, c_i, c_i] + [c_p, c_i, c_i] * 3 + [c_p, c_i] * 3
                              + [c_i, c_p, ctypes.c_uint, c_p, c_i, c_p, c_p])
_SIG["wsmg_rows_gemm_workgroups"] = [c_i, c_i]
_SIG["wsmg_rows_gemm_supported"] = [c_i]
_SIG["wsmg_gru_fwd_chain"] = [c_p] * 5 + [c_i] * 3 + [c_p] * 6 + [c_i, c_p, ctypes.c_uint, c_p, c_p]
_SIG["wsmg_gru_bwd_chain"] = [c_p] * 10 + [c_i] * 3 + [c_p] * 4 + [c_i, c_p, ctypes.c_uint, c_p, c_p]
_SIG["wsmg_gru_chain_workgroups"] = []
_SIG["wsmg_lstm_state_fwd_chain"] = [c_p] * 6 + [c_i] * 3 + [c_p] * 5 + [c_i, c_p, ctypes.c_uint, c_p, c_p]
_SIG["wsmg_lstm_state_bwd_chain"] = [c_p] * 8 + [c_i] * 3 + [c_p] * 4 + [c_i, c_p, ctypes.c_uint, c_p, c_p]
_SIG["wsmg_lstm_state_chain_workgroups"] = []
_SIG["wsmg_attn_fp8_mfma_fused"] = [c_p] * 5 + [c_f] * 4 + [c_i] * 4 + [c_p, ctypes.c_uint, c_i, c_p, c_p, c_p, c_p]
_SIG["wsmg_attn_fp8_mfma_fused_arrivals"] = [c_i] * 4
_SIG["wsmg_attn_fp8_mfma_bwd"] = [c_p] * 12 + [c_f] + [c_i] * 4 + [c_p] * 5
_SIG["wsmg_collate_ego_sparse_nhwc_bf16"] = [c_p] * 5 + [c_i] * 4 + [c_f, c_p, c_p]
_SIG["wsmg_ego_sparse_pack"] = [c_p, c_i, c_i, c_i, c_p, c_p, c_p, c_p, c_p]
_SIG["wsmg_debug_occupy"] = [c_i, c_i, c_i, c_p, c_p, c_p]
_SIG["wsmg_conv2d_bwd_data_bf16_ex"] = [c_p] * 5 + [c_i] * 12 + [c_p]
_SIG["wsmg_conv2d_fwd_bf16_ex"] = [c_p] * 4 + [c_i, c_p, c_i, c_i] + [c_i] * 11 + [c_p]
_SIG["wsmg_bev_index_compact"] = [c_p, c_i, c_i, c_i, c_f, c_i, c_i, c_i, c_f, c_p, c_p, c_p, c_p]
_SIG["wsmg_bev_scatter_rotate_compact"] = [c_p, c_p, c_p, c_p, c_f] + [c_i] * 6 + [c_p, c_p]
_SIG["wsmg_colsum_multi"] = [c_p, c_i, c_p]
_SIG["wsmg_map_fuse_retrieve"] = [c_p] * 5 + [c_i] * 4 + [c_f, c_p, c_p]
_SIG["wsmg_bev_project"] = [c_p, c_p, c_p, c_f, c_i, c_i, c_i, c_f] + [c_i] * 5 + [c_f, c_p, c_p, c_p]
_SIG["wsmg_attn_fp8_row_fwd"] = [c_p] * 5 + [c_f, c_i, c_i, c_i] + [c_p] * 4
_RESTYPE = {"wsmg_cls_tail_workspace_floats": c_l, "wsmg_attn_fp8_workspace_bytes": c_l, "wsmg_lstm_workspace_bytes": c_l, "wsmg_build_info": ctypes.c_char_p, "wsmg_channel_reduce_workspace_bytes": c_l, "wsmg_gru_workspace_bytes": c_l, "wsmg_lstm_state_workspace_bytes": c_l,
            "wsmg_instr_rnn_workspace_bytes": c_l}

_lib = None


def lib():
    global _lib
    if _lib is None:
        if not os.path.exists(LIB_PATH):
            raise WsmgError(
                f"{LIB_PATH} not found: build it with `make -C ws-mgmap_amd/csrc` "
                "(or __graft_entry__.build()). The HIP kernels are mandatory; there is no fallback path.")
        try:
            L = ctypes.CDLL(LIB_PATH)
        except OSError as e:
            raise WsmgError(f"cannot load {LIB_PATH}: {e}") from e
        for name, args in _SIG.items():
            try:
                fn = getattr(L, name)
            except AttributeError as e:
                raise WsmgError(f"{LIB_PATH} does not export {name}") from e
            fn.argtypes = args
            fn.restype = _RESTYPE.get(name, c_i)
        info = L.wsmg_build_info() or b""
        if b"rnn-nopk" not in info:
            raise WsmgError(f"{LIB_PATH} ({info.decode(errors='replace')}) was not built with the RNN kernels' compiler flags "
                            "(no 'rnn-nopk' in wsmg_build_info()): rebuild with `make -C ws-mgmap_amd/csrc`")
        _lib = L
    return _lib


def call(name, *args):
    rc = getattr(lib(), name)(*args)
    if rc != 0:
        kind = {-1: "WSMG_EINVAL (rejected arguments)", -2: "WSMG_ENOMEM (workspace too small)"}.get(rc, f"hipError_t {rc}")
        raise WsmgError(f"{name} failed: {kind}")


rnn_timeouts = 0


defer_rnn_status = False

STATUS_BITS = ((1, "gru_fwd"), (2, "gru_bwd"), (4, "lstm_fwd"), (8, "lstm_bwd"), (16, "attn_fp8_fused barrier"), (32, "lstm_state_fwd"),
               (64, "lstm_state_bwd"), (128, "instr_rnn_fwd"), (256, "instr_rnn_bwd"))


def check_rnn_status(sync=False, force=False):
    global rnn_timeouts
    if defer_rnn_status and not force:
        return
    if sync:
        import torch
        if torch.cuda.is_available():
            torch.cuda.synchronize()
    v = lib().wsmg_rnn_status(1)
    if v:
        rnn_timeouts += 1
        names = [n for b, n in STATUS_BITS if v & b]
        raise WsmgError("persistent kernel(s) timed out waiting for their cooperating workgroups: " + ", ".join(names) +
                        " — their outputs were filled with NaN; results since the previous check are invalid "
                        "(the persistent kernels need all their workgroups resident at once: too many concurrent persistent "
                        "kernels for the free CUs?  net.recurrent_chunks = 0 runs one at a time)")


def take_rnn_status():
    global rnn_timeouts
    v = int(lib().wsmg_rnn_status(1))
    if v:
        rnn_timeouts += 1
    return v


def status_names(bits):
    return [n for b, n in STATUS_BITS if bits & b]


def exported_names():
    return list(_SIG)
```

ws-mgmap_amd/wsmgmap/debug.py:

```python
import os

_TABLE = [
    ("recurrent_chunks", "WSMG_RECURRENT_CHUNKS", 4, int, "time chunks of the pipelined recurrent core (wsmgmap/recurrent.py); 0 = the staged route"),
    ("rows_gemm", "WSMG_ROWS_GEMM", True, bool, "the recurrent core's dense layers as one launch each (csrc/wsmg_rows_gemm.hip); 0: the GEMM library"),
    ("fp8_fused", "WSMG_FP8_FUSED", True, bool, "ops.attention_fp8_shared as one launch (wsmg_attn_fp8_mfma_fused) where its grid barrier is safe"),
    ("fp8_row_fused", "WSMG_FP8_ROW_FUSED", True, bool, "single-query fp8 attention (one token set per row) as one launch: fold + attention per row (round 6)"),
    ("recurrent_chain", "WSMG_RECURRENT_CHAIN", True, bool, "each recurrence of the pipelined core as ONE launch chained to the attention stage by device-side counters"),
    ("decoder_streams", "WSMG_DECODER_STREAMS", 1, int, "0: map decoder on one stream; 1: side stream unless ranks share a GPU; 2: always"),
    ("early_dedup", "WSMG_EARLY_DEDUP", True, bool, "instruction dedup on its own stream when the producer marked the tokens ready (ops.mark_inputs_ready)"),
    ("early_dedup_dp", "WSMG_EARLY_DEDUP_DP", False, bool, "the early dedup also under a process group (needs the exchange on a policy stream: GradAllReducer(exchange_stream=...))"),
    ("rollout_fold", "WSMG_ROLLOUT_FOLD", True, bool, "rollout map stack with BatchNorm-folded cached operands"),
    ("depth_engine", "WSMG_DEPTH_ENGINE", False, bool, "frozen depth ResNet50 on the bf16 NHWC engine (5 % error: opt-in)"),
    ("fused_cls_tail", "WSMG_FUSED_CLS_TAIL", True, bool, "classifier tail (BN + ReLU + 1x1 + CE + pool) in one pass per direction"),
    ("bn_fused_stats", "WSMG_BN_FUSED_STATS", True, bool, "BatchNorm sums in the producing convolution's epilogue"),
    ("relu_producer_mask", "WSMG_RELU_PRODUCER_MASK", True, bool, "fused-ReLU masks of map_encoded / map_classified_linear in map_cated_linear's backward-data epilogue (round 6)"),
    ("conv_into_cat", "WSMG_CONV_INTO_CAT", True, bool, "map_encoded / map_classified_linear write straight into their slices of the concatenation (round 6)"),
    ("strided_grads", "WSMG_STRIDED_GRADS", True, bool, "channel slices of a concatenation's gradient read in place"),
    ("wgrad_atomics", "WSMG_WGRAD_ATOMICS", False, bool, "weight gradients through float atomics instead of slabs + ordered reduce (not bit-reproducible)"),
    ("conv_splitk", "WSMG_CONV_SPLITK", True, bool, "split-K for rollout-size layers"),
    ("rows_linear", "WSMG_ROWS_LINEAR", True, bool, "one-launch dense layers for <= 16 rows"),
    ("bev_fused", "WSMG_BEV_FUSED", True, bool, "scatter + rotation in one launch, plane-consuming fuse"),
    ("bev_compact", "WSMG_BEV_COMPACT", True, bool, "BEV: the index launch packs the valid sources and the scatter walks only those (round 6)"),
    ("bev_one_launch", "WSMG_BEV_ONE_LAUNCH", -1, int, "BEV: index + scatter + rotation as one launch (wsmg_bev_project) and fuse + retrieve as one (wsmg_map_fuse_retrieve); -1: where profiles/bev_fuse_retrieve.txt has them measured and not slower (fuse + retrieve at B = 1 of E = 100, C = 64, G = 240), 0: never, 1: wherever the shapes allow"),
    ("rnn_stock", "WSMG_RNN_STOCK", False, bool, "the three recurrences on the stock (MIOpen) GRU / LSTM: no persistent kernel at all (bench.py's last fallback; needs recurrent_chunks = 0)"),
    ("rnn_poison", "WSMG_RNN_POISON", False, bool, "NaN-fill the persistent kernels' workspaces first (stress tool)"),
    ("feeder_pin", "WSMG_FEEDER_PIN", True, bool, "register the feeder's shared-memory ring as pinned memory"),
    ("keep_blas", "WSMG_KEEP_BLAS", False, bool, "leave torch's BLAS backend choice alone (default: rocBLAS)"),
]


class Switches:
    def __init__(self):
        self.reload()

    def reload(self):
        for attr, var, default, kind, _ in _TABLE:
            raw = os.environ.get(var)
            if raw is None:
                val = default
            elif kind is bool:
                val = raw not in ("0", "", "false", "False")
            else:
                val = kind(raw)
            setattr(self, attr, val)
        return self

    def describe(self):
        return "\n".join("    %-20s %-27s %-8s %s" % (a, v, d, m) for a, v, d, _, m in _TABLE)


sw = Switches()
__doc__ += sw.describe() + "\n"
```

ws-mgmap_amd/wsmgmap/ops/conv.py:

```python
import ctypes

import torch

from .. import _abi
from ..debug import sw
from .core import _p, _raw_stream, _stream, _req, _f32, _sfx, _workspace, _rows_of, _conv_out, _launch, _zeros_f32, _prelaid, _join_side_at_end, TokenGradSink
from .nhwc import cat_channels
from .norm import channel_sum



def prelayout_conv_weights(weights, dtype):
    descs, keep = [], []
    for w in weights:
        if w.dim() != 4 or not w.is_cuda or w.dtype != torch.float32 or not w.is_contiguous():
            continue
        O, I, KH, KW = w.shape
        cin_pad = (I + 31) // 32 * 32
        key = (w.data_ptr(), w._version, cin_pad, dtype)
        if key in _prelaid:
            continue
        ohwi = torch.empty(O, KH, KW, cin_pad, device=w.device, dtype=dtype)
        ihwo = torch.empty(cin_pad, KH, KW, O, device=w.device, dtype=dtype)
        _prelaid[key] = (ohwi, ihwo)
        descs.append(_abi.RelayoutDesc(w.data_ptr(), ohwi.data_ptr(), ihwo.data_ptr(), O, I, KH, KW, cin_pad, 0))
        keep.append(w)
    if descs:
        arr = (_abi.RelayoutDesc * len(descs))(*descs)
        _abi.call("wsmg_weight_relayout_multi", ctypes.cast(arr, ctypes.c_void_p), len(descs), int(dtype == torch.bfloat16), _stream())


def _weight_layouts(w_oihw, cin_pad, dtype, need_ihwo):
    hit = _prelaid.get((w_oihw.data_ptr(), w_oihw._version, cin_pad, dtype))
    if hit is not None:
        return hit[0], (hit[1] if need_ihwo else None)
    O, I, KH, KW = w_oihw.shape
    w_ohwi = torch.empty(O, KH, KW, cin_pad, device=w_oihw.device, dtype=dtype)
    w_ihwo = torch.empty(cin_pad, KH, KW, O, device=w_oihw.device, dtype=dtype) if need_ihwo else None
    _abi.call("wsmg_weight_relayout" + ("_bf16" if dtype == torch.bfloat16 else ""), _p(w_oihw), O, I, KH, KW, cin_pad,
              _p(w_ohwi), _p(w_ihwo), _stream())
    return w_ohwi, w_ihwo


def _weight_grad_oihw(dw_ohwi, I):
    O, KH, KW, Ipad = dw_ohwi.shape
    out = torch.empty(O, I, KH, KW, device=dw_ohwi.device, dtype=torch.float32)
    _abi.call("wsmg_weight_grad_to_oihw", _p(dw_ohwi), O, I, KH, KW, Ipad, _p(out), _stream())
    return out


_wgrad_ws = {}


def _wgrad_workspace(device, floats):
    key = (device.index, _raw_stream())
    ws = _wgrad_ws.get(key)
    if ws is None or ws.numel() < floats:
        if ws is not None:
            ws.record_stream(torch.cuda.current_stream())
        ws = torch.empty(max(int(floats), 1 << 24), device=device, dtype=torch.float32)
        _wgrad_ws[key] = ws
    return ws


def _weight_grad(sfx, x, dy, dims, fl, Cin_w):
    B, H, W, Cin, Cout, KH, KW, stride, pad, OH, OW = dims
    if sw.wgrad_atomics:
        dw_ohwi = _zeros_f32((Cout, KH, KW, Cin), x.device)
        _launch("wsmg_conv2d_bwd_weight" + sfx, fl, _p(x), _p(dy), _p(dw_ohwi), *dims, _stream())
        return _weight_grad_oihw(dw_ohwi, Cin_w)
    nsplit, floats = ctypes.c_int(0), ctypes.c_longlong(0)
    _abi.call("wsmg_conv2d_bwd_weight" + sfx + "_plan", *dims, ctypes.cast(ctypes.byref(nsplit), ctypes.c_void_p),
              ctypes.cast(ctypes.byref(floats), ctypes.c_void_p))
    ws = _wgrad_workspace(x.device, floats.value)
    _launch("wsmg_conv2d_bwd_weight" + sfx + "_slabs", fl, _p(x), _p(dy), _p(ws), nsplit.value, floats.value, *dims, _stream())
    out = torch.empty(Cout, Cin_w, KH, KW, device=x.device, dtype=torch.float32)
    _launch("wsmg_weight_grad_reduce_oihw", 0.0, _p(ws), nsplit.value, Cout, Cin_w, KH, KW, Cin, _p(out), _stream(),
            prof_as="wsmg_conv2d_bwd_weight" + sfx + "_slabs")
    return out


class ReluSink:

    def __init__(self):
        self.relu = False
        self.masked = False


def _mask_of(mask_z, mask_sinks):
    if mask_z is None or not mask_sinks or not sw.relu_producer_mask or not all(m.relu for m in mask_sinks):
        return None
    for m in mask_sinks:
        m.masked = True
    return mask_z


class _Conv2d(torch.autograd.Function):

    @staticmethod
    def forward(ctx, x, w_oihw, bias, stride, pad, bias_grad_zero=False, relu=False, stats=None, relu_sink=None, into=None, lo_sink=None):
        _req(x, w_oihw, bias)
        _f32(w_oihw, bias)
        sfx = _sfx(x)
        B, H, W, Cin = x.shape
        Cout, Cin_w, KH, KW = w_oihw.shape
        assert Cin >= Cin_w, (x.shape, w_oihw.shape)
        w, w_ihwo = _weight_layouts(w_oihw.contiguous(), Cin, x.dtype, ctx.needs_input_grad[0])
        OH, OW = _conv_out(H, KH, stride, pad), _conv_out(W, KW, stride, pad)
        fl = 2.0 * B * OH * OW * Cout * Cin * KH * KW
        dims = (B, H, W, Cin, Cout, KH, KW, stride, pad, OH, OW)
        if into is not None and sfx and stats is None:
            base, c_off = into
            y = base[..., c_off:c_off + Cout]
            _launch("wsmg_conv2d_fwd_bf16_ex", fl, _p(x), _p(w), _p(bias), ctypes.c_void_p(base.data_ptr() + c_off * 2), 2 if relu else 0,
                    None, 0, base.shape[-1], *dims, _stream())
        else:
            y = torch.empty(B, OH, OW, Cout, device=x.device, dtype=x.dtype)
            if sfx and stats is not None:
                _launch("wsmg_conv2d_fwd_bf16_stats", fl, _p(x), _p(w), _p(bias), _p(y), 2 if relu else 0, _p(stats), stats.shape[0],
                        *dims, _stream())
            elif sfx:
                _launch("wsmg_conv2d_fwd_bf16", fl, _p(x), _p(w), _p(bias), _p(y), 2 if relu else 0, *dims, _stream())
            else:
                _launch("wsmg_conv2d_fwd", fl, _p(x), _p(w), _p(bias), _p(y), *dims, _stream())
                if relu:
                    _abi.call("wsmg_relu_fwd", _p(y), _p(y), y.numel(), _stream())
        ctx.save_for_backward(x, w_ihwo, y if relu else None)
        ctx.cfg = dims + (bias is not None, sfx, Cin_w)
        ctx.bias_grad_zero = bool(bias_grad_zero)
        ctx.relu_sink = relu_sink if relu else None
        if ctx.relu_sink is not None:
            relu_sink.relu = True
        ctx.lo_sink = lo_sink if sfx else None
        return y

    @staticmethod
    def backward(ctx, dy):
        x, w_ihwo, y_relu = ctx.saved_tensors
        *dims, has_bias, sfx, Cin_w = ctx.cfg
        B, H, W, Cin, Cout, KH, KW, stride, pad, OH, OW = dims
        if ctx.relu_sink is not None and ctx.relu_sink.masked:
            y_relu = None
        if y_relu is not None:
            masked = torch.empty(y_relu.shape, device=y_relu.device, dtype=y_relu.dtype)
            dy, ld = _rows_of(dy, Cout) if sfx else (dy.contiguous(), Cout)
            if not y_relu.is_contiguous():
                y_relu = y_relu.contiguous()
            if ld != Cout:
                _abi.call("wsmg_relu_bwd_rows_bf16", _p(dy), ld, _p(y_relu), _p(masked), dy.numel() // Cout, Cout, _stream())
            else:
                _abi.call("wsmg_relu_bwd" + sfx, _p(dy), _p(y_relu), _p(masked), dy.numel(), _stream())
            dy = masked
        else:
            dy = dy.contiguous()
        dx = dw = db = None
        fl = 2.0 * B * OH * OW * Cout * Cin * KH * KW
        if ctx.needs_input_grad[0]:
            dx = torch.empty_like(x)
            if sfx:
                _launch("wsmg_conv2d_bwd_data_bf16", fl, _p(dy), _p(w_ihwo), _p(dx), 0, *dims, _stream())
            else:
                _launch("wsmg_conv2d_bwd_data", fl, _p(dy), _p(w_ihwo), _p(dx), *dims, _stream())
        if ctx.needs_input_grad[1]:
            dw = _weight_grad(sfx, x, dy, dims, fl, Cin_w)
            lo = ctx.lo_sink.take() if ctx.lo_sink is not None else None
            if lo is not None and lo.shape == dy.shape:
                dw = dw + _weight_grad(sfx, x, lo, dims, fl, Cin_w)
        if has_bias and ctx.needs_input_grad[2]:
            db = _zeros_f32((Cout,), dy.device) if ctx.bias_grad_zero else channel_sum(dy.view(-1, Cout))
        return dx, dw, db, None, None, None, None, None, None, None, None


class _ConvT2d(torch.autograd.Function):

    @staticmethod
    def forward(ctx, x, w_iohw, stride, pad, stats=None):
        _req(x, w_iohw)
        _f32(w_iohw)
        sfx = _sfx(x)
        B, Hs, Ws, Ct_in = x.shape
        O, I, KH, KW = w_iohw.shape
        assert O == Ct_in
        Hb, Wb = (Hs - 1) * stride - 2 * pad + KH, (Ws - 1) * stride - 2 * pad + KW
        w, w_ihwo = _weight_layouts(w_iohw.contiguous(), I, x.dtype, True)
        y = torch.empty(B, Hb, Wb, I, device=x.device, dtype=x.dtype)
        fl = 2.0 * B * Hs * Ws * O * I * KH * KW
        dims = (B, Hb, Wb, I, O, KH, KW, stride, pad, Hs, Ws)
        if sfx and stats is not None:
            _launch("wsmg_conv2d_bwd_data_bf16_stats", fl, _p(x), _p(w_ihwo), _p(y), 0, _p(stats), stats.shape[0], *dims, _stream())
        elif sfx:
            _launch("wsmg_conv2d_bwd_data_bf16", fl, _p(x), _p(w_ihwo), _p(y), 0, *dims, _stream())
        else:
            _launch("wsmg_conv2d_bwd_data", fl, _p(x), _p(w_ihwo), _p(y), *dims, _stream())
        ctx.save_for_backward(x, w)
        ctx.cfg = dims + (sfx,)
        return y

    @staticmethod
    def backward(ctx, dy):
        x, w = ctx.saved_tensors
        *dims, sfx = ctx.cfg
        B, Hb, Wb, I, O, KH, KW, stride, pad, Hs, Ws = dims
        dy = dy.contiguous()
        dx = dw = None
        fl = 2.0 * B * Hs * Ws * O * I * KH * KW
        if ctx.needs_input_grad[0]:
            dx = torch.empty_like(x)
            if sfx:
                _launch("wsmg_conv2d_fwd_bf16", fl, _p(dy), _p(w), None, _p(dx), 0, *dims, _stream())
            else:
                _launch("wsmg_conv2d_fwd", fl, _p(dy), _p(w), None, _p(dx), *dims, _stream())
        if ctx.needs_input_grad[1]:
            dw = _weight_grad(sfx, dy, x, tuple(dims), fl, I)
        return dx, dw, None, None, None


def conv2d(x, weight_oihw, bias, stride=1, pad=0, bias_grad_zero=False, relu=False, stats=None, relu_sink=None, into=None, lo_sink=None):
    return _Conv2d.apply(x, weight_oihw, bias, stride, pad, bias_grad_zero, relu, stats, relu_sink, into, lo_sink)


class _Conv2dCat2(torch.autograd.Function):

    @staticmethod
    def forward(ctx, a, b, base, w_oihw, bias, relu, relu_sink, mask_sinks):
        _req(base, w_oihw, bias)
        _f32(w_oihw, bias)
        B, H, W, Cin = base.shape
        Cout, Cin_w, KH, KW = w_oihw.shape
        assert Cin == Cin_w and KH == 3 and KW == 3 and base.dtype == torch.bfloat16
        w, w_ihwo = _weight_layouts(w_oihw.contiguous(), Cin, base.dtype, True)
        y = torch.empty(B, H, W, Cout, device=base.device, dtype=base.dtype)
        fl = 2.0 * B * H * W * Cout * Cin * 9
        dims = (B, H, W, Cin, Cout, 3, 3, 1, 1, H, W)
        _launch("wsmg_conv2d_fwd_bf16", fl, _p(base), _p(w), _p(bias), _p(y), 2 if relu else 0, *dims, _stream())
        ctx.save_for_backward(base, w_ihwo, y if relu else None)
        ctx.cfg = dims + (bias is not None, a.shape[-1])
        ctx.relu_sink = relu_sink if relu else None
        if ctx.relu_sink is not None:
            relu_sink.relu = True
        ctx.mask_sinks = mask_sinks
        return y

    @staticmethod
    def backward(ctx, dy):
        base, w_ihwo, y_relu = ctx.saved_tensors
        *dims, has_bias, ca = ctx.cfg
        B, H, W, Cin, Cout = dims[:5]
        if ctx.relu_sink is not None and ctx.relu_sink.masked:
            y_relu = None
        if y_relu is not None:
            masked = torch.empty_like(y_relu)
            dy = dy.contiguous()
            _abi.call("wsmg_relu_bwd_bf16", _p(dy), _p(y_relu), _p(masked), dy.numel(), _stream())
            dy = masked
        else:
            dy = dy.contiguous()
        fl = 2.0 * B * H * W * Cout * Cin * 9
        da = torch.empty(B, H, W, ca, device=dy.device, dtype=dy.dtype)
        db = torch.empty(B, H, W, Cin - ca, device=dy.device, dtype=dy.dtype)
        _launch("wsmg_conv2d_bwd_data_bf16_ex", fl, _p(dy), _p(w_ihwo), _p(da), _p(_mask_of(base, ctx.mask_sinks)), _p(db), ca, *dims, _stream())
        dw = _weight_grad("_bf16", base, dy, tuple(dims), fl, Cin) if ctx.needs_input_grad[3] else None
        dbias = channel_sum(dy.view(-1, Cout)) if (has_bias and ctx.needs_input_grad[4]) else None
        return da, db, None, dw, dbias, None, None, None


def conv2d_over_written_parts(a, b, base, weight_oihw, bias, relu=True, relu_sink=None, mask_sinks=None):
    ca, cb = a.shape[-1], b.shape[-1]
    ok = (base.dtype == torch.bfloat16 and base.is_contiguous() and base.shape[-1] == ca + cb and ca % 8 == 0 and cb % 8 == 0
          and a.data_ptr() == base.data_ptr() and b.data_ptr() == base.data_ptr() + ca * base.element_size()
          and a.stride() == base.stride() and b.stride() == base.stride() and tuple(weight_oihw.shape[1:]) == (ca + cb, 3, 3))
    if not ok:
        return conv2d(cat_channels(a.contiguous(), b.contiguous()), weight_oihw, bias, 1, 1, relu=relu, relu_sink=relu_sink)
    return _Conv2dCat2.apply(a, b, base, weight_oihw, bias, relu, relu_sink, mask_sinks)


def conv2d_cat(xs, weight_oihw, bias, stride=1, pad=0, bias_grad_zero=False, relu=False, relu_sink=None):
    xs = list(xs)
    x = xs[0] if len(xs) == 1 else (cat_channels(xs[0], xs[1]) if len(xs) == 2 else torch.cat(xs, dim=-1))
    return conv2d(x, weight_oihw, bias, stride, pad, bias_grad_zero, relu, relu_sink=relu_sink)


_splitk_plans = {}


def _splitk_plan(B, OH, OW, Cin, Cout, KH, KW):
    key = (B, OH, OW, Cin, Cout, KH, KW)
    plan = _splitk_plans.get(key)
    if plan is None:
        ks, floats = ctypes.c_int(0), ctypes.c_longlong(0)
        _abi.call("wsmg_conv2d_splitk_plan", B, OH, OW, Cin, Cout, KH, KW, ctypes.cast(ctypes.byref(ks), ctypes.c_void_p),
                  ctypes.cast(ctypes.byref(floats), ctypes.c_void_p))
        plan = _splitk_plans[key] = (ks.value, floats.value)
    return plan


def conv2d_infer_bf16(x, w_ohwi_bf16, bias, stride, pad, relu, out_f32=False, add_to=None):
    _req(x, w_ohwi_bf16, bias, add_to)
    if x.dtype != torch.bfloat16 or w_ohwi_bf16.dtype != torch.bfloat16:
        raise _abi.WsmgError("conv2d_infer_bf16 needs bf16 activations and weights")
    B, H, W, Cin = x.shape
    Cout, KH, KW, Cin2 = w_ohwi_bf16.shape
    assert Cin == Cin2, (x.shape, w_ohwi_bf16.shape)
    OH, OW = _conv_out(H, KH, stride, pad), _conv_out(W, KW, stride, pad)
    odt = torch.float32 if out_f32 else torch.bfloat16
    if add_to is not None:
        if add_to.shape != (B, OH, OW, Cout) or add_to.dtype != odt or add_to.device != x.device:
            raise _abi.WsmgError("conv2d_infer_bf16: add_to must have the output's shape, type and device")
        y = add_to
    else:
        y = torch.empty(B, OH, OW, Cout, device=x.device, dtype=odt)
    flags = (2 if relu else 0) | (1 if out_f32 else 0) | (4 if add_to is not None else 0)
    fl = 2.0 * B * OH * OW * Cout * Cin * KH * KW
    dims = (B, H, W, Cin, Cout, KH, KW, stride, pad, OH, OW)
    ks, floats = _splitk_plan(B, OH, OW, Cin, Cout, KH, KW) if sw.conv_splitk else (1, 0)
    if ks > 1:
        part = torch.empty(floats, device=x.device, dtype=torch.float32)
        _launch("wsmg_conv2d_fwd_bf16_splitk", fl, _p(x), _p(w_ohwi_bf16), _p(bias), _p(y), flags, ks, _p(part), *dims, _stream())
    else:
        _launch("wsmg_conv2d_fwd_bf16", fl, _p(x), _p(w_ohwi_bf16), _p(bias), _p(y), flags, *dims, _stream())
    return y


@torch.no_grad()
def copy_multi(dsts, srcs):
    pairs = []
    for d, s in zip(dsts, srcs):
        if (d.is_cuda and s.is_cuda and d.device == s.device and d.dtype == s.dtype and d.shape == s.shape and d.is_contiguous()
                and s.is_contiguous()):
            if d.numel():
                pairs.append((d, s))
        else:
            d.copy_(s)
    if not pairs:
        return
    arr = (_abi.CopyDesc * len(pairs))()
    for i, (d, s) in enumerate(pairs):
        arr[i].dst, arr[i].src, arr[i].bytes = d.data_ptr(), s.data_ptr(), d.numel() * d.element_size()
    _abi.call("wsmg_copy_multi", ctypes.cast(arr, ctypes.c_void_p), len(pairs), _stream())


def conv_transpose2d_infer_bf16(x, w_ihwo_bf16, bias, stride, pad, relu):
    _req(x, w_ihwo_bf16, bias)
    if x.dtype != torch.bfloat16 or w_ihwo_bf16.dtype != torch.bfloat16:
        raise _abi.WsmgError("conv_transpose2d_infer_bf16 needs bf16 activations and weights")
    B, Hs, Ws, Ct_in = x.shape
    I, KH, KW, O = w_ihwo_bf16.shape
    assert O == Ct_in, (x.shape, w_ihwo_bf16.shape)
    Hb, Wb = (Hs - 1) * stride - 2 * pad + KH, (Ws - 1) * stride - 2 * pad + KW
    y = torch.empty(B, Hb, Wb, I, device=x.device, dtype=torch.bfloat16)
    _launch("wsmg_conv_transpose2d_infer_bf16", 2.0 * B * Hs * Ws * O * I * KH * KW, _p(x), _p(w_ihwo_bf16), _p(bias), _p(y),
            2 if relu else 0, B, Hb, Wb, I, O, KH, KW, stride, pad, Hs, Ws, _stream())
    return y


def conv_transpose2d(x, weight_iohw, stride=2, pad=1, stats=None):
    return _ConvT2d.apply(x, weight_iohw, stride, pad, stats)
```

ws-mgmap_amd/wsmgmap/ops/core.py:

```python
import ctypes

import torch

from .. import _abi
from ..debug import sw

_ws_cache = {}


def _p(t):
    return None if t is None else ctypes.c_void_p(t.data_ptr())


if hasattr(torch._C, "_cuda_getCurrentRawStream") and hasattr(torch._C, "_cuda_getDevice"):
    def _raw_stream():
        return torch._C._cuda_getCurrentRawStream(torch._C._cuda_getDevice())
else:
    def _raw_stream():
        return torch.cuda.current_stream().cuda_stream


def _stream():
    return ctypes.c_void_p(_raw_stream())


def _req(*ts):
    for t in ts:
        if t is None:
            continue
        if not t.is_cuda:
            raise _abi.WsmgError("wsmgmap operators need GPU tensors: the HIP path is the only path (no CPU fallback)")
        if not t.is_contiguous():
            raise _abi.WsmgError(f"non-contiguous tensor passed to a wsmgmap kernel: shape {tuple(t.shape)} strides {t.stride()}")


def _f32(*ts):
    for t in ts:
        if t is not None and t.dtype != torch.float32:
            raise _abi.WsmgError(f"this wsmgmap argument must be float32, got {t.dtype}")


def _sfx(t):
    if t.dtype == torch.float32:
        return ""
    if t.dtype == torch.bfloat16:
        return "_bf16"
    raise _abi.WsmgError(f"wsmgmap activations are float32 or bfloat16, got {t.dtype}")


def _workspace(device):
    key = (device.type, device.index, _raw_stream())
    ws = _ws_cache.get(key)
    if ws is None:
        ws = torch.empty(1024 * 2 * 256, dtype=torch.float64, device=device)
        _ws_cache[key] = ws
    return ws


def _rows_of(dy, C):
    if dy.is_contiguous():
        return dy, C
    ld = dy.stride(-2) if dy.dim() >= 2 else 0
    ok = (dy.stride(-1) == 1 and ld >= C and ld % 8 == 0 and dy.data_ptr() % 16 == 0 and C % 8 == 0
          and all(dy.stride(i) == dy.stride(i + 1) * dy.shape[i + 1] for i in range(dy.dim() - 2))
          and sw.strided_grads)
    return (dy, ld) if ok else (dy.contiguous(), C)


def _conv_out(h, k, s, p):
    return (h + 2 * p - k) // s + 1


_prof = None

def _prof_key(name):
    return name.replace("_stats", "").replace("_slabs", "").replace("_ex", "")


KERNEL_OF = {
    "wsmg_conv2d_fwd_bf16_stats": "conv_igemm_bf16_kernel<false, *>",
    "wsmg_conv2d_bwd_data_bf16_stats": "conv_igemm_bf16_kernel<true, *>",
    "wsmg_conv2d_fwd": "conv_igemm_kernel<false, false>",
    "wsmg_conv2d_bwd_data": "conv_igemm_kernel<true, false>",
    "wsmg_conv2d_bwd_weight": "conv_wgrad_kernel<false>",
    "wsmg_conv2d_fwd_bf16": "conv_igemm_bf16_kernel<false, *>",
    "wsmg_conv2d_fwd_bf16_splitk": "conv_igemm_bf16_kernel<false, 64, *, 1, true>",
    "wsmg_conv2d_bwd_data_bf16": "conv_igemm_bf16_kernel<true, *>",
    "wsmg_conv2d_bwd_weight_bf16": "conv_wgrad_bf16_kernel",
}


_prof_only = None


def profile_begin(only=None):
    global _prof, _prof_only
    _prof = {}
    _prof_only = set(only) if only else None


def profile_set_only(only):
    global _prof_only
    if _prof is not None:
        _prof_only = set(only) if only else None


def profile_end():
    global _prof, _prof_only
    rec, _prof, _prof_only = _prof, None, None
    torch.cuda.synchronize()
    out = {}
    for name, items in (rec or {}).items():
        ms = sum(s.elapsed_time(e) for s, e, _, _ in items)
        o = out.setdefault(KERNEL_OF[_prof_key(name)], dict(launches=0, ms_total=0.0, flops_total=0.0, entry=_prof_key(name)))
        o["launches"] += sum(n for _, _, _, n in items)
        o["ms_total"] += ms
        o["flops_total"] += float(sum(f for _, _, f, _ in items))
    return out


def _launch(name, flops, *args, prof_as=None):
    key = prof_as or name
    if _prof is None or (_prof_only is not None and _prof_key(key) not in _prof_only):
        _abi.call(name, *args)
        return
    s, e = torch.cuda.Event(enable_timing=True), torch.cuda.Event(enable_timing=True)
    s.record()
    _abi.call(name, *args)
    e.record()
    _prof.setdefault(key, []).append((s, e, flops, 0 if prof_as else 1))


_marks = None


def marks_begin():
    global _marks
    _marks = []


def marks_end():
    global _marks
    out, _marks = _marks, None
    return out


def mark(name, tensor=None):
    if _marks is None:
        return
    e = torch.cuda.Event(enable_timing=True)
    e.record()
    _marks.append(("f:" + name, e))
    if tensor is not None and tensor.requires_grad:
        def hook(g, name=name):
            if _marks is not None:
                ev = torch.cuda.Event(enable_timing=True)
                ev.record()
                _marks.append(("b:" + name, ev))
            return g
        tensor.register_hook(hook)


_helper_streams = {}


def helper_stream(name, device=None, priority=0):
    dev = torch.cuda.current_device() if device is None else torch.device(device).index
    key = (dev, name)
    s = _helper_streams.get(key)
    if s is None:
        s = _helper_streams[key] = torch.cuda.Stream(device=dev, priority=priority)
    return s


def ranks_share_gpu():
    import os
    if not (torch.distributed.is_available() and torch.distributed.is_initialized() and torch.distributed.get_world_size() > 1):
        return False
    lws = int(os.environ.get("LOCAL_WORLD_SIZE", "0") or 0)
    return not (0 < lws <= torch.cuda.device_count())


import weakref

_inputs_ready = {}


def mark_inputs_ready(tensor, event=None):
    if not tensor.is_cuda:
        return None
    if event is None:
        event = torch.cuda.Event()
        event.record(torch.cuda.current_stream(tensor.device))
    key = id(tensor)
    _inputs_ready[key] = (weakref.ref(tensor, lambda _r, key=key: _inputs_ready.pop(key, None)), event)
    return event


_inputs_dedup = {}


def attach_instruction_dedup(tensor, dedup):
    key = id(tensor)
    _inputs_dedup[key] = (weakref.ref(tensor, lambda _r, key=key: _inputs_dedup.pop(key, None)), dedup)


def attached_instruction_dedup(tensor):
    e = _inputs_dedup.get(id(tensor))
    return e[1] if e is not None and e[0]() is tensor else None


def inputs_ready_event(tensor):
    e = _inputs_ready.get(id(tensor))
    return e[1] if e is not None and e[0]() is tensor else None


_prelaid = {}


_zero_pool = {}


def _zero_pool_retire():
    for z in _zero_pool.values():
        z["cap"] = max(z["cap"], z["used"])
        z["buf"], z["off"], z["used"], z["armed"] = None, 0, 0, False


chain_in_flight = False


def reset_pass_state():
    global chain_in_flight
    chain_in_flight = False
    TokenGradSink.check_none_pending()
    _prelaid.clear()
    if any(z["armed"] for z in _zero_pool.values()):
        _zero_pool_retire()
    if _side_join_armed:
        for main_id, side_id in list(_side_join_armed):
            for side in _leaf_streams:
                if side.cuda_stream == side_id:
                    torch.cuda.current_stream().wait_stream(side)
        _side_join_armed.clear()


def _zeros_f32(shape, device):
    numel = 1
    for d in shape:
        numel *= int(d)
    n = (numel + 63) // 64 * 64
    engine = torch.autograd.Variable._execution_engine
    z = _zero_pool.setdefault(_raw_stream(), dict(buf=None, off=0, used=0, cap=0, armed=False))
    z["used"] += n
    if not z["armed"]:
        try:
            engine.queue_callback(_zero_pool_retire)
            z["armed"] = True
        except RuntimeError:
            z["used"] -= n
            return torch.zeros(shape, device=device, dtype=torch.float32)
    if z["buf"] is None and z["cap"] >= n:
        z["buf"], z["off"] = torch.zeros(z["cap"], device=device, dtype=torch.float32), 0
    if z["buf"] is None or z["off"] + n > z["buf"].numel() or z["buf"].device != device:
        return torch.zeros(shape, device=device, dtype=torch.float32)
    out = z["buf"][z["off"]:z["off"] + numel].view(shape)
    z["off"] += n
    return out


_side_join_armed = set()
_leaf_streams = []


def _join_side_at_end(main, side, strict=False):
    key = (main.cuda_stream, side.cuda_stream)
    if key in _side_join_armed:
        return

    def join():
        _side_join_armed.discard(key)
        main.wait_stream(side)
        cur = torch.cuda.current_stream(main.device)
        if cur.cuda_stream != main.cuda_stream:
            cur.wait_stream(side)
    try:
        torch.autograd.Variable._execution_engine.queue_callback(join)
        _side_join_armed.add(key)
    except RuntimeError:
        if strict:
            raise
        main.wait_stream(side)


class TokenGradSink:
    _pending = []

    def __init__(self):
        self.dx = None
        self.relu = False
        self.masked = False

    def park(self, dx):
        self.dx = dx
        TokenGradSink._pending.append(self)

    def take(self):
        dx, self.dx = self.dx, None
        if self in TokenGradSink._pending:
            TokenGradSink._pending.remove(self)
        return dx

    @staticmethod
    def check_none_pending():
        if TokenGradSink._pending:
            TokenGradSink._pending.clear()
            raise _abi.WsmgError("a map-token gradient parked by the attention's backward was never merged (the token mean's "
                                 "backward did not run): gradients of the previous pass are incomplete")
```

Measured before the change: 51930.

## Fuse backward-data and weight-gradient of small conv layers into one launch

Adds a paired bf16 conv backward kernel that computes the input gradient and the weight-gradient slabs in a single launch, with the implicit-GEMM and wgrad bodies moved into shared include/helpers so one grid can dispatch both. Python picks the paired path when both gradients are needed and the combined workgroup count stays under a per-CU limit, then runs the ordered slab reduce. The goal is fewer launches and better occupancy for small layers whose two separate kernels each underfill the GPU. In exchange, LDS sizing becomes the maximum of both kernels, and a larger grid adds some scheduling overhead.

```diff
diff --git a/include/wsmgmap.h b/include/wsmgmap.h
--- a/include/wsmgmap.h
+++ b/include/wsmgmap.h
@@ -250,6 +250,12 @@
                                       int Cin, int Cout, int KH, int KW, int stride, int pad, int OH, int OW, wsmg_stream_t stream);
 int wsmg_conv2d_bwd_weight_plan(int B, int H, int W, int Cin, int Cout, int KH, int KW, int stride, int pad, int OH, int OW,
                                 int* nsplit, long long* ws_floats);
+
+int wsmg_conv2d_bwd_pair_bf16_plan(int B, int H, int W, int Cin, int Cout, int KH, int KW, int stride, int pad, int OH, int OW,
+                                   int* nsplit, long long* ws_floats, long long* workgroups);
+int wsmg_conv2d_bwd_pair_bf16(const void* dy, const void* w_ihwo, void* dx, const void* x, float* ws, int nsplit, long long ws_floats,
+                              int B, int H, int W, int Cin, int Cout, int KH, int KW, int stride, int pad, int OH, int OW,
+                              wsmg_stream_t stream);
 int wsmg_conv2d_bwd_weight_slabs(const float* x, const float* dy, float* ws, int nsplit, long long ws_floats, int B, int H, int W,
                                  int Cin, int Cout, int KH, int KW, int stride, int pad, int OH, int OW, wsmg_stream_t stream);
 int wsmg_weight_grad_reduce_oihw(const float* ws, int nsplit, int O, int I, int KH, int KW, int I_pad, float* dw_oihw,
diff --git a/ws-mgmap_amd/csrc/wsmg_conv_bf16.hip b/ws-mgmap_amd/csrc/wsmg_conv_bf16.hip
--- a/ws-mgmap_amd/csrc/wsmg_conv_bf16.hip
+++ b/ws-mgmap_amd/csrc/wsmg_conv_bf16.hip
@@ -48,289 +48,18 @@
   int split_c;
 };
 
+template <int BN, int BK>
+constexpr int igemm_tile_bytes() {
+  return (BM + BN) * (BK * 2 + 16) > BM * (BN * 2 + 16) ? (BM + BN) * (BK * 2 + 16) : BM * (BN * 2 + 16);
+}
+
 template <bool BWD, int BN, int BK, int PF, bool SPLIT = false>
 __global__ __launch_bounds__(256) void conv_igemm_bf16_kernel(ConvArgsB a) {
-  constexpr int LDB = BK * 2 + 16;
-  constexpr int SEGS = BK / 8;
-  constexpr int RPP = 256 / SEGS;
-  constexpr int APASS = BM / RPP;
-  constexpr int BPASS = BN / RPP;
-  constexpr int NT = BN / 64;
-  constexpr int OPITCH = BN * 2 + 16;
-  constexpr int SMEM = (BM + BN) * LDB > BM * OPITCH ? (BM + BN) * LDB : BM * OPITCH;
-  __shared__ __attribute__((aligned(16))) unsigned char smem[SMEM];
-  unsigned char* const As = smem;
-  unsigned char* const Bs = smem + BM * LDB;
+  __shared__ __attribute__((aligned(16))) unsigned char smem[igemm_tile_bytes<BN, BK>()];
   __shared__ int dpix[BM];
   const int tid = threadIdx.x;
-  const int lane = tid & 63, wave = tid >> 6;
-  const int tiles = a.mtiles * a.ntiles;
-  const int swz = xcd_swizzle(blockIdx.x, gridDim.x);
-  const int split = SPLIT ? swz / tiles : 0;
-  const int logical = SPLIT ? swz - split * tiles : swz;
-  const int m0 = (logical / a.ntiles) * BM, n0 = (logical % a.ntiles) * BN;
-  const int seg = tid % SEGS;
-  const int lrow = tid / SEGS;
-
-  int cy = 0, cx = 0, ty0 = 0, tx0 = 0, tstep = 1, THc = a.TH, TWc = a.TW, KHc = a.KH, KWc = a.KW;
-  if (BWD && a.stride == 2) {
-    cy = blockIdx.y >> 1; cx = blockIdx.y & 1;
-    ty0 = (cy + a.pad) & 1; tx0 = (cx + a.pad) & 1;
-    tstep = 2;
-    THc = (a.TH - ty0 + 1) >> 1; TWc = (a.TW - tx0 + 1) >> 1;
-    KHc = (a.KH - cy + 1) >> 1; KWc = (a.KW - cx + 1) >> 1;
-  }
-  const int Mc = a.B * THc * TWc;
-  if (m0 >= Mc) return;
-
-  const int sg = BWD ? -1 : 1;
-  int roff[APASS];
-  unsigned ymask[APASS], xmask[APASS];
-  int rb_ = (m0 + lrow) / (THc * TWc);
-  int ry_, rx_;
-  {
-    const int r0 = (m0 + lrow) - rb_ * (THc * TWc);
-    ry_ = r0 / TWc;
-    rx_ = r0 - ry_ * TWc;
-  }
-#pragma unroll
-  for (int i = 0; i < APASS; ++i) {
-    int m = m0 + lrow + RPP * i;
-    bool pv = m < Mc;
-    const int b = pv ? rb_ : 0, iy = pv ? ry_ : 0, ix = pv ? rx_ : 0;
-    rx_ += RPP;
-    while (rx_ >= TWc) { rx_ -= TWc; ++ry_; }
-    while (ry_ >= THc) { ry_ -= THc; ++rb_; }
-    int ty = ty0 + iy * tstep, tx = tx0 + ix * tstep;
-    int py, px;
-    if (BWD) {
-      py = (a.stride == 2) ? ((ty + a.pad - cy) >> 1) : ty + a.pad;
-      px = (a.stride == 2) ? ((tx + a.pad - cx) >> 1) : tx + a.pad;
-    } else {
-      py = ty * a.stride - a.pad;
-      px = tx * a.stride - a.pad;
-    }
-    auto tapmask = [&](int p, int S_, int n) -> unsigned {
-      int lo = BWD ? p - (S_ - 1) : -p, hi = BWD ? p : S_ - 1 - p;
-      lo = lo < 0 ? 0 : lo;
-      hi = hi > n - 1 ? n - 1 : hi;
-      return hi >= lo ? ((2u << hi) - 1u) & ~((1u << lo) - 1u) : 0u;
-    };
-    const unsigned ym = tapmask(py, a.SH, KHc), xm = tapmask(px, a.SW, KWc);
-    ymask[i] = pv ? ym : 0u;
-    xmask[i] = xm;
-    roff[i] = ((b * a.SH + py) * a.SW + px) * a.Kc + seg * 8;
-    if (seg == 0) dpix[lrow + RPP * i] = pv ? (b * a.TH + ty) * a.TW + tx : -1;
-  }
-  const int taps = a.KH * a.KW;
-  int woff[BPASS];
-#pragma unroll
-  for (int i = 0; i < BPASS; ++i) {
-    int n = n0 + lrow + RPP * i;
-    woff[i] = n < a.N ? n * taps * a.Kc + seg * 8 : -0x40000000;
-  }
-  const int kchunks = a.Kc / BK;
-  const int all_steps = KHc * KWc * kchunks;
-  const int per_split = SPLIT ? (all_steps + a.ksplit - 1) / a.ksplit : all_steps;
-  const int step_begin = split * per_split;
-  const int steps = SPLIT ? (all_steps - step_begin < per_split ? all_steps - step_begin : per_split) : all_steps;
-  const __amdgpu_buffer_rsrc_t rs_src = make_rsrc(a.src, a.src_bytes);
-  const __amdgpu_buffer_rsrc_t rs_wt = make_rsrc(a.wt, a.wt_bytes);
-
-  int it_ch = 0, it_ay = 0, it_ax = 0, it_left = steps;
-  if (SPLIT) {
-    const int tp = KHc * KWc;
-    it_ch = step_begin / tp;
-    const int rem = step_begin - it_ch * tp;
-    it_ay = rem / KWc;
-    it_ax = rem - it_ay * KWc;
-  }
-  u32x4 ra[PF][APASS], rb[PF][BPASS];
-  auto gload = [&](u32x4 (&ra)[APASS], u32x4 (&rb)[BPASS]) {
-    const int ky = BWD ? cy + it_ay * tstep : it_ay, kx = BWD ? cx + it_ax * tstep : it_ax;
-    const int sdelta = sg * (it_ay * a.SW + it_ax) * a.Kc + it_ch * BK;
-    const bool more = SPLIT ? it_left > 0 : it_ch < kchunks;
-    if (SPLIT) --it_left;
-    const int wdelta = more ? (ky * a.KW + kx) * a.Kc + it_ch * BK : -0x20000000;
-    const unsigned live = more ? 1u : 0u;
-#pragma unroll
-    for (int i = 0; i < APASS; ++i) {
-      bool ok = ((ymask[i] >> it_ay) & (xmask[i] >> it_ax) & live) != 0;
-      ra[i] = buf_load16(rs_src, ok ? (roff[i] + sdelta) * 2 : -1);
-    }
-#pragma unroll
-    for (int i = 0; i < BPASS; ++i) rb[i] = buf_load16(rs_wt, (woff[i] + wdelta) * 2);
-    if (++it_ax == KWc) { it_ax = 0; if (++it_ay == KHc) { it_ay = 0; ++it_ch; } }
-  };
-  auto lstore = [&](const u32x4 (&ra)[APASS], const u32x4 (&rb)[BPASS]) {
-#pragma unroll
-    for (int i = 0; i < APASS; ++i) *reinterpret_cast<u32x4*>(&As[(lrow + RPP * i) * LDB + seg * 16]) = ra[i];
-#pragma unroll
-    for (int i = 0; i < BPASS; ++i) *reinterpret_cast<u32x4*>(&Bs[(lrow + RPP * i) * LDB + seg * 16]) = rb[i];
-  };
-
-  const int wm = (wave & 1) * 64, wn = (wave >> 1) * (BN / 2);
-  const int r = lane & 31, h = lane >> 5;
-  f32x16 acc[2][NT];
-#pragma unroll
-  for (int t = 0; t < 2; ++t)
-#pragma unroll
-    for (int u = 0; u < NT; ++u)
-#pragma unroll
-      for (int i = 0; i < 16; ++i) acc[t][u][i] = 0.f;
-
-  gload(ra[0], rb[0]);
-  lstore(ra[0], rb[0]);
-  __syncthreads();
-#pragma unroll
-  for (int j = 1; j < PF; ++j) gload(ra[j], rb[j]);
-  for (int step0 = 0; step0 < steps; step0 += PF) {
-#pragma unroll
-    for (int j = 0; j < PF; ++j) {
-      gload(ra[j], rb[j]);
-#pragma unroll
-      for (int ks = 0; ks < BK / 16; ++ks) {
-        bf16x8 af[2], bf[NT];
-#pragma unroll
-        for (int t = 0; t < 2; ++t)
-          af[t] = *reinterpret_cast<const bf16x8*>(&As[(wm + 32 * t + r) * LDB + ks * 32 + h * 16]);
-#pragma unroll
-        for (int u = 0; u < NT; ++u)
-          bf[u] = *reinterpret_cast<const bf16x8*>(&Bs[(wn + 32 * u + r) * LDB + ks * 32 + h * 16]);
-#pragma unroll
-        for (int t = 0; t < 2; ++t)
-#pragma unroll
-          for (int u = 0; u < NT; ++u)
-            acc[t][u] = __builtin_amdgcn_mfma_f32_32x32x16_bf16(af[t], bf[u], acc[t][u], 0, 0, 0);
-      }
-      __syncthreads();
-      lstore(ra[(j + 1) % PF], rb[(j + 1) % PF]);
-      __syncthreads();
-    }
-  }
-
-  if (SPLIT) {
-    float* const mine = a.part + (size_t)split * Mc * a.N;
-#pragma unroll
-    for (int u = 0; u < NT; ++u) {
-      const int n = n0 + wn + 32 * u + r;
-      if (n >= a.N) continue;
-#pragma unroll
-      for (int t = 0; t < 2; ++t)
-#pragma unroll
-        for (int g = 0; g < 16; ++g) {
-          const int m = m0 + wm + 32 * t + (g & 3) + 8 * (g >> 2) + 4 * h;
-          if (m < Mc) mine[(size_t)m * a.N + n] = acc[t][u][g];
-        }
-    }
-    return;
-  }
-
-  constexpr int OP = OPITCH;
-  {
-    if ((a.out_f32 & 1) == 0 && (a.N & 7) == 0) {
-      const bool relu_here = (a.out_f32 & 6) == 2;
-#pragma unroll
-      for (int u = 0; u < NT; ++u) {
-        const int col = wn + 32 * u + r;
-        const float bv = (a.bias && n0 + col < a.N) ? a.bias[n0 + col] : 0.f;
-        float sv = 0.f, qv = 0.f;
-#pragma unroll
-        for (int t = 0; t < 2; ++t)
-#pragma unroll
-          for (int g = 0; g < 16; ++g) {
-            const int row = wm + 32 * t + (g & 3) + 8 * (g >> 2) + 4 * h;
-            float v = acc[t][u][g] + bv;
-            if (relu_here) v = v > 0.f ? v : 0.f;
-            const unsigned short o = f2bf_bits(v);
-            *reinterpret_cast<unsigned short*>(smem + row * OP + col * 2) = o;
-            if (a.stats) {
-              const float vr = m0 + row < Mc ? __uint_as_float((unsigned)o << 16) : 0.f;
-              sv += vr;
-              qv = fmaf(vr, vr, qv);
-            }
-          }
-        if (a.stats) {
-          sv += __shfl_xor(sv, 32, 64);
-          qv += __shfl_xor(qv, 32, 64);
-          if (h == 0 && n0 + col < a.N) {
-            double* st = a.stats + (size_t)((logical / a.ntiles) % a.nslab) * 2 * a.N + n0 + col;
-            atomicAdd(st, (double)sv);
-            atomicAdd(st + a.N, (double)qv);
-          }
-        }
-      }
-      __syncthreads();
-      constexpr int CPR = BN / 8;
-      const int ldd = a.dst_ld ? a.dst_ld : a.N;
-      constexpr int ROWS = BM * CPR / 256;
-      u32x4 zr[ROWS];
-      if (a.relu_z) {
-#pragma unroll
-        for (int j = 0; j < ROWS; ++j) {
-          const int c = tid + 256 * j;
-          const int row = c / CPR, ch = c - row * CPR;
-          const int dp = dpix[row];
-          const int n = n0 + ch * 8;
-          zr[j] = (dp >= 0 && n < a.N) ? *reinterpret_cast<const u32x4*>(a.relu_z + (size_t)dp * a.N + n) : u32x4{0u, 0u, 0u, 0u};
-        }
-      }
-#pragma unroll
-      for (int j = 0; j < BM * CPR / 256; ++j) {
-        const int c = tid + 256 * j;
-        const int row = c / CPR, ch = c - row * CPR;
-        const int dp = dpix[row];
-        const int n = n0 + ch * 8;
-        if (dp < 0 || n >= a.N) continue;
-        u32x4* out = reinterpret_cast<u32x4*>(reinterpret_cast<unsigned char*>(a.dst) + ((size_t)dp * ldd + n) * 2);
-        if (a.dst2) {
-          const bool hi = n >= a.split_c;
-          out = reinterpret_cast<u32x4*>(reinterpret_cast<unsigned char*>(hi ? a.dst2 : a.dst) +
-                                         ((size_t)dp * (hi ? a.N - a.split_c : a.split_c) + (hi ? n - a.split_c : n)) * 2);
-        }
-        u32x4 v = *reinterpret_cast<const u32x4*>(smem + row * OP + ch * 16);
-        if (a.relu_z) v = relu_mask8(v, zr[j]);
-        if (a.out_f32 & 4) {
-          const u32x4 old = *out;
-#pragma unroll
-          for (int q = 0; q < 4; ++q) {
-            float lo = __uint_as_float(v[q] << 16) + __uint_as_float(old[q] << 16);
-            float hi = __uint_as_float(v[q] & 0xffff0000u) + __uint_as_float(old[q] & 0xffff0000u);
-            if (a.out_f32 & 2) { lo = lo > 0.f ? lo : 0.f; hi = hi > 0.f ? hi : 0.f; }
-            v[q] = (unsigned)f2bf_bits(lo) | ((unsigned)f2bf_bits(hi) << 16);
-          }
-        }
-        *out = v;
-      }
-      return;
-    }
-  }
-#pragma unroll
-  for (int u = 0; u < NT; ++u) {
-    const int n = n0 + wn + 32 * u + r;
-    if (n >= a.N) continue;
-    const float bv = a.bias ? a.bias[n] : 0.f;
-#pragma unroll
-    for (int t = 0; t < 2; ++t) {
-#pragma unroll
-      for (int g = 0; g < 16; ++g) {
-        int row = wm + 32 * t + (g & 3) + 8 * (g >> 2) + 4 * h;
-        int dp = dpix[row];
-        if (dp < 0) continue;
-        float v = acc[t][u][g] + bv;
-        if (a.out_f32 & 4) {
-          const size_t o = (size_t)dp * a.N + n;
-          v += (a.out_f32 & 1) ? reinterpret_cast<const float*>(a.dst)[o]
-                               : __uint_as_float((unsigned)reinterpret_cast<const unsigned short*>(a.dst)[o] << 16);
-        }
-        if (a.out_f32 & 2) v = v > 0.f ? v : 0.f;
-        if (a.out_f32 & 1)
-          reinterpret_cast<float*>(a.dst)[(size_t)dp * a.N + n] = v;
-        else
-          reinterpret_cast<unsigned short*>(a.dst)[(size_t)dp * a.N + n] = f2bf_bits(v);
-      }
-    }
-  }
+  const int bid = blockIdx.x, nblocks = gridDim.x, cls = blockIdx.y;
+#include "wsmg_conv_bf16_igemm.inc"
 }
 
 constexpr int WKP = 64;
@@ -352,161 +81,47 @@
   return __builtin_amdgcn_ds_read_tr16_b64_v4i16((bf16x4 __attribute__((address_space(3)))*)(p));
 }
 
+template <int TC>
+constexpr int wgrad_d_bytes() { return WKP * (TC == 4 ? 320 : 192); }
+template <int TU>
+constexpr int wgrad_x_bytes() { return 4 * TU * WKP * X_LD; }
+
 template <int TC, int TU, int PF, int UPT>
 __global__ __launch_bounds__(256) void conv_wgrad_bf16_kernel(WgradArgsB a) {
-  constexpr int WCO = 32 * TC;
-  constexpr int WUN = 4 * TU;
-  constexpr int NG = WUN / UPT;
-  constexpr int D_LD = TC == 4 ? 320 : 192;
-  constexpr int DSEG = 4 * TC;
-  constexpr int DROWS = 256 / DSEG;
-  __shared__ __attribute__((aligned(16))) unsigned char Ds[WKP * D_LD];
-  __shared__ __attribute__((aligned(16))) unsigned char Xs[WUN * WKP * X_LD];
+  __shared__ __attribute__((aligned(16))) unsigned char Ds[wgrad_d_bytes<TC>()];
+  __shared__ __attribute__((aligned(16))) unsigned char Xs[wgrad_x_bytes<TU>()];
   const int tid = threadIdx.x;
-  const int lane = tid & 63, wave = tid >> 6;
-  const int logical = xcd_swizzle(blockIdx.x, gridDim.x);
-  const int gxy = a.gx * a.gy;
-  const int bz = logical / gxy, bxy = logical - bz * gxy;
-  const int u0 = (bxy % a.gx) * WUN;
-  const int co0 = (bxy / a.gx) * WCO;
-  const int64_t p_begin = (int64_t)bz * a.chunk;
-  int64_t p_end = p_begin + a.chunk;
-  if (p_end > a.npix) p_end = a.npix;
-  const int cchunks = a.Cin / 32;
-  const int ohw = a.OH * a.OW;
-
-  int gky[NG], gkx[NG], gci[NG];
-  bool gok[NG];
-#pragma unroll
-  for (int g = 0; g < NG; ++g) {
-    int uu = u0 + g * UPT;
-    gok[g] = uu < a.units;
-    int t = gok[g] ? uu / cchunks : 0;
-    gci[g] = gok[g] ? (uu - t * cchunks) * 32 : 0;
-    gky[g] = t / a.KW;
-    gkx[g] = t - gky[g] * a.KW;
-  }
-  const int dpx = tid / DSEG, dseg = tid % DSEG;
-  const int xpx = tid >> 2, xseg = tid & 3;
-
-  f32x16 acc[TC][TU];
-#pragma unroll
-  for (int t = 0; t < TC; ++t)
-#pragma unroll
-    for (int u = 0; u < TU; ++u)
-#pragma unroll
-      for (int i = 0; i < 16; ++i) acc[t][u][i] = 0.f;
-
-  const __amdgpu_buffer_rsrc_t rs_x = make_rsrc(a.x, a.x_bytes);
-  const __amdgpu_buffer_rsrc_t rs_dy = make_rsrc(a.dy, a.dy_bytes);
-  const bool co_ok = (co0 + dseg * 8) < a.Cout;
-  int gdelta[NG];
-#pragma unroll
-  for (int g = 0; g < NG; ++g) gdelta[g] = (gky[g] * a.W + gkx[g]) * a.Cin + gci[g] + xseg * 8;
-  int it_b, it_oy, it_ox;
-  {
-    int64_t p = p_begin + xpx;
-    if (p >= a.npix) p = a.npix - 1;
-    it_b = (int)(p / ohw);
-    int rem = (int)(p - (int64_t)it_b * ohw);
-    it_oy = rem / a.OW;
-    it_ox = rem - it_oy * a.OW;
-  }
-  const int adv_b = WKP / ohw, adv_rem = WKP - adv_b * ohw;
-  const int adv_oy = adv_rem / a.OW, adv_ox = adv_rem - adv_oy * a.OW;
-  int it_p = (int)p_begin;
-  const int pend = (int)p_end;
-  u32x4 rd[PF][TC], rx[PF][WUN];
-  auto gload = [&](u32x4 (&rd)[TC], u32x4 (&rx)[WUN]) {
-#pragma unroll
-    for (int i = 0; i < TC; ++i) {
-      int p = it_p + dpx + DROWS * i;
-      bool ok = co_ok && p < pend;
-      rd[i] = buf_load16(rs_dy, ok ? (p * a.Cout + co0 + dseg * 8) * 2 : -1);
-    }
-    const bool pok = (it_p + xpx) < pend;
-    const int y0 = it_oy * a.stride - a.pad, x0 = it_ox * a.stride - a.pad;
-    const int base = ((it_b * a.H + y0) * a.W + x0) * a.Cin;
-#pragma unroll
-    for (int g = 0; g < NG; ++g) {
-      bool ok = pok && gok[g] && (unsigned)(y0 + gky[g]) < (unsigned)a.H && (unsigned)(x0 + gkx[g]) < (unsigned)a.W;
-      const int off = ok ? (base + gdelta[g]) * 2 : (int)0x80000000;
-#pragma unroll
-      for (int j = 0; j < UPT; ++j) rx[g * UPT + j] = buf_load16(rs_x, off + 64 * j);
-    }
-    it_p += WKP;
-    it_ox += adv_ox;
-    if (it_ox >= a.OW) { it_ox -= a.OW; ++it_oy; }
-    it_oy += adv_oy;
-    if (it_oy >= a.OH) { it_oy -= a.OH; ++it_b; }
-    it_b += adv_b;
-  };
-  auto lstore = [&](const u32x4 (&rd)[TC], const u32x4 (&rx)[WUN]) {
-#pragma unroll
-    for (int i = 0; i < TC; ++i) *reinterpret_cast<u32x4*>(&Ds[(dpx + DROWS * i) * D_LD + dseg * 16]) = rd[i];
-#pragma unroll
-    for (int u = 0; u < WUN; ++u) *reinterpret_cast<u32x4*>(&Xs[(u * WKP + xpx) * X_LD + xseg * 16]) = rx[u];
-  };
-
-  const int li = lane & 15, q = li >> 2, p4 = li & 3;
-  const int half16 = (lane >> 4) & 1;
-  const int h = lane >> 5;
-  const unsigned char* a_base = &Ds[(8 * h + q) * D_LD + (half16 * 16 + p4 * 4) * 2];
-  const unsigned char* b_base = &Xs[(wave * TU * WKP + 8 * h + q) * X_LD + (half16 * 16 + p4 * 4) * 2];
-
-  gload(rd[0], rx[0]);
-  lstore(rd[0], rx[0]);
-  __syncthreads();
-#pragma unroll
-  for (int j = 1; j < PF; ++j) gload(rd[j], rx[j]);
-  for (int64_t pb = p_begin; pb < p_end; pb += (int64_t)PF * WKP) {
-#pragma unroll
-    for (int j = 0; j < PF; ++j) {
-      gload(rd[j], rx[j]);
-#pragma unroll
-      for (int ks = 0; ks < WKP / 16; ++ks) {
-        bf16x8 af[TC], bfr[TU];
-#pragma unroll
-        for (int t = 0; t < TC; ++t) {
-          bf16x4 l = tr_read(a_base + 64 * t + (16 * ks) * D_LD), hh = tr_read(a_base + 64 * t + (16 * ks + 4) * D_LD);
-          af[t] = __builtin_shufflevector(l, hh, 0, 1, 2, 3, 4, 5, 6, 7);
-        }
-#pragma unroll
-        for (int u = 0; u < TU; ++u) {
-          const unsigned char* bp = b_base + u * WKP * X_LD;
-          bf16x4 l = tr_read(bp + (16 * ks) * X_LD), hh = tr_read(bp + (16 * ks + 4) * X_LD);
-          bfr[u] = __builtin_shufflevector(l, hh, 0, 1, 2, 3, 4, 5, 6, 7);
-        }
-#pragma unroll
-        for (int u = 0; u < TU; ++u)
-#pragma unroll
-          for (int t = 0; t < TC; ++t) acc[t][u] = __builtin_amdgcn_mfma_f32_32x32x16_bf16(af[t], bfr[u], acc[t][u], 0, 0, 0);
-      }
-      __syncthreads();
-      lstore(rd[(j + 1) % PF], rx[(j + 1) % PF]);
-      __syncthreads();
-    }
-  }
-  const int r = lane & 31;
-  const int taps = a.KH * a.KW;
-#pragma unroll
-  for (int u = 0; u < TU; ++u) {
-    const int uu = u0 + wave * TU + u;
-    if (uu >= a.units) continue;
-    const int tap = uu / cchunks;
-    const int ci = (uu - tap * cchunks) * 32 + r;
-#pragma unroll
-    for (int t = 0; t < TC; ++t) {
-#pragma unroll
-      for (int g = 0; g < 16; ++g) {
-        int co = co0 + 32 * t + (g & 3) + 8 * (g >> 2) + 4 * h;
-        if (co < a.Cout) {
-          float* const q = a.dw + (size_t)bz * a.slab + ((size_t)co * taps + tap) * a.Cin + ci;
-          if (a.slab) *q = acc[t][u][g];
-          else atomicAdd(q, acc[t][u][g]);
-        }
-      }
-    }
+  const int bid = blockIdx.x, nblocks = gridDim.x;
+#include "wsmg_conv_bf16_wgrad.inc"
+}
+
+struct PairArgsB {
+  ConvArgsB d;
+  WgradArgsB w;
+  int split;
+};
+
+template <int BN, int UPT>
+__global__ __launch_bounds__(256) void conv_bwd_pair_bf16_kernel(PairArgsB pa) {
+  constexpr int IG_LDS = igemm_tile_bytes<BN, 64>() + BM * (int)sizeof(int);
+  constexpr int WG_LDS = wgrad_d_bytes<2>() + wgrad_x_bytes<1>();
+  __shared__ __attribute__((aligned(16))) unsigned char lds[IG_LDS > WG_LDS ? IG_LDS : WG_LDS];
+  const int tid = threadIdx.x;
+  if ((int)blockIdx.x < pa.split) {
+    constexpr bool BWD = true, SPLIT = false;
+    constexpr int BK = 64, PF = 1;
+    const ConvArgsB& a = pa.d;
+    unsigned char* const smem = lds;
+    int* const dpix = reinterpret_cast<int*>(lds + igemm_tile_bytes<BN, 64>());
+    const int bid = blockIdx.x, nblocks = pa.split, cls = 0;
+#include "wsmg_conv_bf16_igemm.inc"
+  } else {
+    constexpr int TC = 2, TU = 1, PF = 1;
+    const WgradArgsB& a = pa.w;
+    unsigned char* const Ds = lds;
+    unsigned char* const Xs = lds + wgrad_d_bytes<2>();
+    const int bid = (int)blockIdx.x - pa.split, nblocks = (int)gridDim.x - pa.split;
+#include "wsmg_conv_bf16_wgrad.inc"
   }
 }
 
@@ -870,6 +485,29 @@
 #undef WSMG_WGRAD
   WSMG_RETURN_LAUNCH();
 }
+
+struct PairPlan {
+  int bn, upt, tiles_d;
+  WgradPlan w;
+};
+
+bool pair_plan_bf16(int B, int H, int W, int Cin, int Cout, int KH, int KW, int stride, int pad, int OH, int OW, PairPlan& pp) {
+  if (stride != 1) return false;
+  if (KH == 3 && KW == 3 && pad == 1 && OH == H && OW == W &&
+      (k32_choice((int64_t)B * H * W, Cout, Cin) || win3_choice((int64_t)B * H * W, Cout, Cin)))
+    return false;
+  if (Cout % 64) return false;
+  pp.w = wgrad_plan_bf16(B, H, W, Cin, Cout, KH, KW, stride, pad, OH, OW);
+  if (pp.w.kind != 0 || pp.w.tc != 2 || pp.w.tu != 1) return false;
+  const int cch = Cin / 32;
+  pp.upt = cch % 4 == 0 ? 4 : (cch % 2 == 0 ? 2 : 1);
+  pp.bn = Cin >= 128 ? 128 : 64;
+  if (!((pp.bn == 64 && pp.upt == 2) || (pp.bn == 128 && pp.upt == 4))) return false;
+  const int64_t tiles = wsmg_cdiv((int64_t)B * H * W, BM) * wsmg_cdiv(Cin, pp.bn);
+  if (tiles + (int64_t)pp.w.gx * pp.w.gy * pp.w.nsplit >= (1ll << 31)) return false;
+  pp.tiles_d = (int)tiles;
+  return true;
+}
 }
 
 extern "C" int wsmg_conv2d_bwd_weight_bf16(const void* x, const void* dy, float* dw_ohwi, int B, int H, int W, int Cin,
@@ -898,3 +536,45 @@
   if (!ws || nsplit != p.nsplit || ws_floats < slab * p.nsplit) return WSMG_EINVAL;
   return launch_wgrad_bf16(x, dy, ws, slab, B, H, W, Cin, Cout, KH, KW, stride, pad, OH, OW, wsmg_s(stream));
 }
+
+extern "C" int wsmg_conv2d_bwd_pair_bf16_plan(int B, int H, int W, int Cin, int Cout, int KH, int KW, int stride, int pad, int OH, int OW,
+                                              int* nsplit, long long* ws_floats, long long* workgroups) {
+  if (!nsplit || !ws_floats || !workgroups) return WSMG_EINVAL;
+  if (int e = check_conv(B, H, W, Cin, Cout, KH, KW, stride, pad, OH, OW)) return e;
+  PairPlan pp;
+  if (!pair_plan_bf16(B, H, W, Cin, Cout, KH, KW, stride, pad, OH, OW, pp)) return WSMG_EINVAL;
+  *nsplit = pp.w.nsplit;
+  *ws_floats = (long long)pp.w.nsplit * Cout * KH * KW * Cin;
+  *workgroups = (long long)pp.tiles_d + (long long)pp.w.gx * pp.w.gy * pp.w.nsplit;
+  return 0;
+}
+
+extern "C" int wsmg_conv2d_bwd_pair_bf16(const void* dy, const void* w_ihwo, void* dx, const void* x, float* ws, int nsplit,
+                                         long long ws_floats, int B, int H, int W, int Cin, int Cout, int KH, int KW, int stride,
+                                         int pad, int OH, int OW, wsmg_stream_t stream) {
+  if (int e = check_conv(B, H, W, Cin, Cout, KH, KW, stride, pad, OH, OW)) return e;
+  PairPlan pp;
+  if (!dy || !w_ihwo || !dx || !x || !ws) return WSMG_EINVAL;
+  if (!pair_plan_bf16(B, H, W, Cin, Cout, KH, KW, stride, pad, OH, OW, pp)) return WSMG_EINVAL;
+  const long long slab = (long long)Cout * KH * KW * Cin;
+  if (nsplit != pp.w.nsplit || ws_floats < slab * pp.w.nsplit) return WSMG_EINVAL;
+  PairArgsB a;
+  a.d = ConvArgsB{(const bf16_t*)dy, (const bf16_t*)w_ihwo, nullptr, dx, B, OH, OW, Cout, H, W, Cin, KH, KW, stride, pad, 0, 0, 0,
+                  (unsigned)((size_t)B * OH * OW * Cout * 2), (unsigned)((size_t)Cout * KH * KW * Cin * 2), nullptr, 0};
+  a.d.mtiles = (int)wsmg_cdiv((int64_t)B * H * W, BM);
+  a.d.ntiles = (int)wsmg_cdiv(Cin, pp.bn);
+  a.w = WgradArgsB{(const bf16_t*)x, (const bf16_t*)dy, ws, B, H, W, Cin, Cout, KH, KW, stride, pad, OH, OW, 0, 0, 0,
+                   (unsigned)((size_t)B * H * W * Cin * 2), (unsigned)((size_t)B * OH * OW * Cout * 2), 0, 0, (int64_t)slab};
+  a.w.units = KH * KW * (Cin / 32);
+  a.w.npix = (int64_t)B * OH * OW;
+  a.w.chunk = pp.w.chunk;
+  a.w.gx = pp.w.gx;
+  a.w.gy = pp.w.gy;
+  a.split = pp.tiles_d;
+  const dim3 grid((unsigned)(pp.tiles_d + pp.w.gx * pp.w.gy * pp.w.nsplit));
+  if (pp.bn == 64)
+    hipLaunchKernelGGL((conv_bwd_pair_bf16_kernel<64, 2>), grid, dim3(256), 0, wsmg_s(stream), a);
+  else
+    hipLaunchKernelGGL((conv_bwd_pair_bf16_kernel<128, 4>), grid, dim3(256), 0, wsmg_s(stream), a);
+  WSMG_RETURN_LAUNCH();
+}
diff --git a/ws-mgmap_amd/csrc/wsmg_conv_bf16_igemm.inc b/ws-mgmap_amd/csrc/wsmg_conv_bf16_igemm.inc
--- /dev/null
+++ b/ws-mgmap_amd/csrc/wsmg_conv_bf16_igemm.inc
@@ -0,0 +1,277 @@
+  constexpr int LDB = BK * 2 + 16;
+  constexpr int SEGS = BK / 8;
+  constexpr int RPP = 256 / SEGS;
+  constexpr int APASS = BM / RPP;
+  constexpr int BPASS = BN / RPP;
+  constexpr int NT = BN / 64;
+  constexpr int OPITCH = BN * 2 + 16;
+  unsigned char* const As = smem;
+  unsigned char* const Bs = smem + BM * LDB;
+  const int lane = tid & 63, wave = tid >> 6;
+  const int tiles = a.mtiles * a.ntiles;
+  const int swz = xcd_swizzle(bid, nblocks);
+  const int split = SPLIT ? swz / tiles : 0;
+  const int logical = SPLIT ? swz - split * tiles : swz;
+  const int m0 = (logical / a.ntiles) * BM, n0 = (logical % a.ntiles) * BN;
+  const int seg = tid % SEGS;
+  const int lrow = tid / SEGS;
+
+  int cy = 0, cx = 0, ty0 = 0, tx0 = 0, tstep = 1, THc = a.TH, TWc = a.TW, KHc = a.KH, KWc = a.KW;
+  if (BWD && a.stride == 2) {
+    cy = cls >> 1; cx = cls & 1;
+    ty0 = (cy + a.pad) & 1; tx0 = (cx + a.pad) & 1;
+    tstep = 2;
+    THc = (a.TH - ty0 + 1) >> 1; TWc = (a.TW - tx0 + 1) >> 1;
+    KHc = (a.KH - cy + 1) >> 1; KWc = (a.KW - cx + 1) >> 1;
+  }
+  const int Mc = a.B * THc * TWc;
+  if (m0 >= Mc) return;
+
+  const int sg = BWD ? -1 : 1;
+  int roff[APASS];
+  unsigned ymask[APASS], xmask[APASS];
+  int rb_ = (m0 + lrow) / (THc * TWc);
+  int ry_, rx_;
+  {
+    const int r0 = (m0 + lrow) - rb_ * (THc * TWc);
+    ry_ = r0 / TWc;
+    rx_ = r0 - ry_ * TWc;
+  }
+#pragma unroll
+  for (int i = 0; i < APASS; ++i) {
+    int m = m0 + lrow + RPP * i;
+    bool pv = m < Mc;
+    const int b = pv ? rb_ : 0, iy = pv ? ry_ : 0, ix = pv ? rx_ : 0;
+    rx_ += RPP;
+    while (rx_ >= TWc) { rx_ -= TWc; ++ry_; }
+    while (ry_ >= THc) { ry_ -= THc; ++rb_; }
+    int ty = ty0 + iy * tstep, tx = tx0 + ix * tstep;
+    int py, px;
+    if (BWD) {
+      py = (a.stride == 2) ? ((ty + a.pad - cy) >> 1) : ty + a.pad;
+      px = (a.stride == 2) ? ((tx + a.pad - cx) >> 1) : tx + a.pad;
+    } else {
+      py = ty * a.stride - a.pad;
+      px = tx * a.stride - a.pad;
+    }
+    auto tapmask = [&](int p, int S_, int n) -> unsigned {
+      int lo = BWD ? p - (S_ - 1) : -p, hi = BWD ? p : S_ - 1 - p;
+      lo = lo < 0 ? 0 : lo;
+      hi = hi > n - 1 ? n - 1 : hi;
+      return hi >= lo ? ((2u << hi) - 1u) & ~((1u << lo) - 1u) : 0u;
+    };
+    const unsigned ym = tapmask(py, a.SH, KHc), xm = tapmask(px, a.SW, KWc);
+    ymask[i] = pv ? ym : 0u;
+    xmask[i] = xm;
+    roff[i] = ((b * a.SH + py) * a.SW + px) * a.Kc + seg * 8;
+    if (seg == 0) dpix[lrow + RPP * i] = pv ? (b * a.TH + ty) * a.TW + tx : -1;
+  }
+  const int taps = a.KH * a.KW;
+  int woff[BPASS];
+#pragma unroll
+  for (int i = 0; i < BPASS; ++i) {
+    int n = n0 + lrow + RPP * i;
+    woff[i] = n < a.N ? n * taps * a.Kc + seg * 8 : -0x40000000;
+  }
+  const int kchunks = a.Kc / BK;
+  const int all_steps = KHc * KWc * kchunks;
+  const int per_split = SPLIT ? (all_steps + a.ksplit - 1) / a.ksplit : all_steps;
+  const int step_begin = split * per_split;
+  const int steps = SPLIT ? (all_steps - step_begin < per_split ? all_steps - step_begin : per_split) : all_steps;
+  const __amdgpu_buffer_rsrc_t rs_src = make_rsrc(a.src, a.src_bytes);
+  const __amdgpu_buffer_rsrc_t rs_wt = make_rsrc(a.wt, a.wt_bytes);
+
+  int it_ch = 0, it_ay = 0, it_ax = 0, it_left = steps;
+  if (SPLIT) {
+    const int tp = KHc * KWc;
+    it_ch = step_begin / tp;
+    const int rem = step_begin - it_ch * tp;
+    it_ay = rem / KWc;
+    it_ax = rem - it_ay * KWc;
+  }
+  u32x4 ra[PF][APASS], rb[PF][BPASS];
+  auto gload = [&](u32x4 (&ra)[APASS], u32x4 (&rb)[BPASS]) {
+    const int ky = BWD ? cy + it_ay * tstep : it_ay, kx = BWD ? cx + it_ax * tstep : it_ax;
+    const int sdelta = sg * (it_ay * a.SW + it_ax) * a.Kc + it_ch * BK;
+    const bool more = SPLIT ? it_left > 0 : it_ch < kchunks;
+    if (SPLIT) --it_left;
+    const int wdelta = more ? (ky * a.KW + kx) * a.Kc + it_ch * BK : -0x20000000;
+    const unsigned live = more ? 1u : 0u;
+#pragma unroll
+    for (int i = 0; i < APASS; ++i) {
+      bool ok = ((ymask[i] >> it_ay) & (xmask[i] >> it_ax) & live) != 0;
+      ra[i] = buf_load16(rs_src, ok ? (roff[i] + sdelta) * 2 : -1);
+    }
+#pragma unroll
+    for (int i = 0; i < BPASS; ++i) rb[i] = buf_load16(rs_wt, (woff[i] + wdelta) * 2);
+    if (++it_ax == KWc) { it_ax = 0; if (++it_ay == KHc) { it_ay = 0; ++it_ch; } }
+  };
+  auto lstore = [&](const u32x4 (&ra)[APASS], const u32x4 (&rb)[BPASS]) {
+#pragma unroll
+    for (int i = 0; i < APASS; ++i) *reinterpret_cast<u32x4*>(&As[(lrow + RPP * i) * LDB + seg * 16]) = ra[i];
+#pragma unroll
+    for (int i = 0; i < BPASS; ++i) *reinterpret_cast<u32x4*>(&Bs[(lrow + RPP * i) * LDB + seg * 16]) = rb[i];
+  };
+
+  const int wm = (wave & 1) * 64, wn = (wave >> 1) * (BN / 2);
+  const int r = lane & 31, h = lane >> 5;
+  f32x16 acc[2][NT];
+#pragma unroll
+  for (int t = 0; t < 2; ++t)
+#pragma unroll
+    for (int u = 0; u < NT; ++u)
+#pragma unroll
+      for (int i = 0; i < 16; ++i) acc[t][u][i] = 0.f;
+
+  gload(ra[0], rb[0]);
+  lstore(ra[0], rb[0]);
+  __syncthreads();
+#pragma unroll
+  for (int j = 1; j < PF; ++j) gload(ra[j], rb[j]);
+  for (int step0 = 0; step0 < steps; step0 += PF) {
+#pragma unroll
+    for (int j = 0; j < PF; ++j) {
+      gload(ra[j], rb[j]);
+#pragma unroll
+      for (int ks = 0; ks < BK / 16; ++ks) {
+        bf16x8 af[2], bf[NT];
+#pragma unroll
+        for (int t = 0; t < 2; ++t)
+          af[t] = *reinterpret_cast<const bf16x8*>(&As[(wm + 32 * t + r) * LDB + ks * 32 + h * 16]);
+#pragma unroll
+        for (int u = 0; u < NT; ++u)
+          bf[u] = *reinterpret_cast<const bf16x8*>(&Bs[(wn + 32 * u + r) * LDB + ks * 32 + h * 16]);
+#pragma unroll
+        for (int t = 0; t < 2; ++t)
+#pragma unroll
+          for (int u = 0; u < NT; ++u)
+            acc[t][u] = __builtin_amdgcn_mfma_f32_32x32x16_bf16(af[t], bf[u], acc[t][u], 0, 0, 0);
+      }
+      __syncthreads();
+      lstore(ra[(j + 1) % PF], rb[(j + 1) % PF]);
+      __syncthreads();
+    }
+  }
+
+  if (SPLIT) {
+    float* const mine = a.part + (size_t)split * Mc * a.N;
+#pragma unroll
+    for (int u = 0; u < NT; ++u) {
+      const int n = n0 + wn + 32 * u + r;
+      if (n >= a.N) continue;
+#pragma unroll
+      for (int t = 0; t < 2; ++t)
+#pragma unroll
+        for (int g = 0; g < 16; ++g) {
+          const int m = m0 + wm + 32 * t + (g & 3) + 8 * (g >> 2) + 4 * h;
+          if (m < Mc) mine[(size_t)m * a.N + n] = acc[t][u][g];
+        }
+    }
+    return;
+  }
+
+  constexpr int OP = OPITCH;
+  {
+    if ((a.out_f32 & 1) == 0 && (a.N & 7) == 0) {
+      const bool relu_here = (a.out_f32 & 6) == 2;
+#pragma unroll
+      for (int u = 0; u < NT; ++u) {
+        const int col = wn + 32 * u + r;
+        const float bv = (a.bias && n0 + col < a.N) ? a.bias[n0 + col] : 0.f;
+        float sv = 0.f, qv = 0.f;
+#pragma unroll
+        for (int t = 0; t < 2; ++t)
+#pragma unroll
+          for (int g = 0; g < 16; ++g) {
+            const int row = wm + 32 * t + (g & 3) + 8 * (g >> 2) + 4 * h;
+            float v = acc[t][u][g] + bv;
+            if (relu_here) v = v > 0.f ? v : 0.f;
+            const unsigned short o = f2bf_bits(v);
+            *reinterpret_cast<unsigned short*>(smem + row * OP + col * 2) = o;
+            if (a.stats) {
+              const float vr = m0 + row < Mc ? __uint_as_float((unsigned)o << 16) : 0.f;
+              sv += vr;
+              qv = fmaf(vr, vr, qv);
+            }
+          }
+        if (a.stats) {
+          sv += __shfl_xor(sv, 32, 64);
+          qv += __shfl_xor(qv, 32, 64);
+          if (h == 0 && n0 + col < a.N) {
+            double* st = a.stats + (size_t)((logical / a.ntiles) % a.nslab) * 2 * a.N + n0 + col;
+            atomicAdd(st, (double)sv);
+            atomicAdd(st + a.N, (double)qv);
+          }
+        }
+      }
+      __syncthreads();
+      constexpr int CPR = BN / 8;
+      const int ldd = a.dst_ld ? a.dst_ld : a.N;
+      constexpr int ROWS = BM * CPR / 256;
+      u32x4 zr[ROWS];
+      if (a.relu_z) {
+#pragma unroll
+        for (int j = 0; j < ROWS; ++j) {
+          const int c = tid + 256 * j;
+          const int row = c / CPR, ch = c - row * CPR;
+          const int dp = dpix[row];
+          const int n = n0 + ch * 8;
+          zr[j] = (dp >= 0 && n < a.N) ? *reinterpret_cast<const u32x4*>(a.relu_z + (size_t)dp * a.N + n) : u32x4{0u, 0u, 0u, 0u};
+        }
+      }
+#pragma unroll
+      for (int j = 0; j < BM * CPR / 256; ++j) {
+        const int c = tid + 256 * j;
+        const int row = c / CPR, ch = c - row * CPR;
+        const int dp = dpix[row];
+        const int n = n0 + ch * 8;
+        if (dp < 0 || n >= a.N) continue;
+        u32x4* out = reinterpret_cast<u32x4*>(reinterpret_cast<unsigned char*>(a.dst) + ((size_t)dp * ldd + n) * 2);
+        if (a.dst2) {
+          const bool hi = n >= a.split_c;
+          out = reinterpret_cast<u32x4*>(reinterpret_cast<unsigned char*>(hi ? a.dst2 : a.dst) +
+                                         ((size_t)dp * (hi ? a.N - a.split_c : a.split_c) + (hi ? n - a.split_c : n)) * 2);
+        }
+        u32x4 v = *reinterpret_cast<const u32x4*>(smem + row * OP + ch * 16);
+        if (a.relu_z) v = relu_mask8(v, zr[j]);
+        if (a.out_f32 & 4) {
+          const u32x4 old = *out;
+#pragma unroll
+          for (int q = 0; q < 4; ++q) {
+            float lo = __uint_as_float(v[q] << 16) + __uint_as_float(old[q] << 16);
+            float hi = __uint_as_float(v[q] & 0xffff0000u) + __uint_as_float(old[q] & 0xffff0000u);
+            if (a.out_f32 & 2) { lo = lo > 0.f ? lo : 0.f; hi = hi > 0.f ? hi : 0.f; }
+            v[q] = (unsigned)f2bf_bits(lo) | ((unsigned)f2bf_bits(hi) << 16);
+          }
+        }
+        *out = v;
+      }
+      return;
+    }
+  }
+#pragma unroll
+  for (int u = 0; u < NT; ++u) {
+    const int n = n0 + wn + 32 * u + r;
+    if (n >= a.N) continue;
+    const float bv = a.bias ? a.bias[n] : 0.f;
+#pragma unroll
+    for (int t = 0; t < 2; ++t) {
+#pragma unroll
+      for (int g = 0; g < 16; ++g) {
+        int row = wm + 32 * t + (g & 3) + 8 * (g >> 2) + 4 * h;
+        int dp = dpix[row];
+        if (dp < 0) continue;
+        float v = acc[t][u][g] + bv;
+        if (a.out_f32 & 4) {
+          const size_t o = (size_t)dp * a.N + n;
+          v += (a.out_f32 & 1) ? reinterpret_cast<const float*>(a.dst)[o]
+                               : __uint_as_float((unsigned)reinterpret_cast<const unsigned short*>(a.dst)[o] << 16);
+        }
+        if (a.out_f32 & 2) v = v > 0.f ? v : 0.f;
+        if (a.out_f32 & 1)
+          reinterpret_cast<float*>(a.dst)[(size_t)dp * a.N + n] = v;
+        else
+          reinterpret_cast<unsigned short*>(a.dst)[(size_t)dp * a.N + n] = f2bf_bits(v);
+      }
+    }
+  }
diff --git a/ws-mgmap_amd/csrc/wsmg_conv_bf16_wgrad.inc b/ws-mgmap_amd/csrc/wsmg_conv_bf16_wgrad.inc
--- /dev/null
+++ b/ws-mgmap_amd/csrc/wsmg_conv_bf16_wgrad.inc
@@ -0,0 +1,152 @@
+  constexpr int WCO = 32 * TC;
+  constexpr int WUN = 4 * TU;
+  constexpr int NG = WUN / UPT;
+  constexpr int D_LD = TC == 4 ? 320 : 192;
+  constexpr int DSEG = 4 * TC;
+  constexpr int DROWS = 256 / DSEG;
+  static_assert(wgrad_d_bytes<TC>() == WKP * D_LD && wgrad_x_bytes<TU>() == WUN * WKP * X_LD, "LDS sizes");
+  const int lane = tid & 63, wave = tid >> 6;
+  const int logical = xcd_swizzle(bid, nblocks);
+  const int gxy = a.gx * a.gy;
+  const int bz = logical / gxy, bxy = logical - bz * gxy;
+  const int u0 = (bxy % a.gx) * WUN;
+  const int co0 = (bxy / a.gx) * WCO;
+  const int64_t p_begin = (int64_t)bz * a.chunk;
+  int64_t p_end = p_begin + a.chunk;
+  if (p_end > a.npix) p_end = a.npix;
+  const int cchunks = a.Cin / 32;
+  const int ohw = a.OH * a.OW;
+
+  int gky[NG], gkx[NG], gci[NG];
+  bool gok[NG];
+#pragma unroll
+  for (int g = 0; g < NG; ++g) {
+    int uu = u0 + g * UPT;
+    gok[g] = uu < a.units;
+    int t = gok[g] ? uu / cchunks : 0;
+    gci[g] = gok[g] ? (uu - t * cchunks) * 32 : 0;
+    gky[g] = t / a.KW;
+    gkx[g] = t - gky[g] * a.KW;
+  }
+  const int dpx = tid / DSEG, dseg = tid % DSEG;
+  const int xpx = tid >> 2, xseg = tid & 3;
+
+  f32x16 acc[TC][TU];
+#pragma unroll
+  for (int t = 0; t < TC; ++t)
+#pragma unroll
+    for (int u = 0; u < TU; ++u)
+#pragma unroll
+      for (int i = 0; i < 16; ++i) acc[t][u][i] = 0.f;
+
+  const __amdgpu_buffer_rsrc_t rs_x = make_rsrc(a.x, a.x_bytes);
+  const __amdgpu_buffer_rsrc_t rs_dy = make_rsrc(a.dy, a.dy_bytes);
+  const bool co_ok = (co0 + dseg * 8) < a.Cout;
+  int gdelta[NG];
+#pragma unroll
+  for (int g = 0; g < NG; ++g) gdelta[g] = (gky[g] * a.W + gkx[g]) * a.Cin + gci[g] + xseg * 8;
+  int it_b, it_oy, it_ox;
+  {
+    int64_t p = p_begin + xpx;
+    if (p >= a.npix) p = a.npix - 1;
+    it_b = (int)(p / ohw);
+    int rem = (int)(p - (int64_t)it_b * ohw);
+    it_oy = rem / a.OW;
+    it_ox = rem - it_oy * a.OW;
+  }
+  const int adv_b = WKP / ohw, adv_rem = WKP - adv_b * ohw;
+  const int adv_oy = adv_rem / a.OW, adv_ox = adv_rem - adv_oy * a.OW;
+  int it_p = (int)p_begin;
+  const int pend = (int)p_end;
+  u32x4 rd[PF][TC], rx[PF][WUN];
+  auto gload = [&](u32x4 (&rd)[TC], u32x4 (&rx)[WUN]) {
+#pragma unroll
+    for (int i = 0; i < TC; ++i) {
+      int p = it_p + dpx + DROWS * i;
+      bool ok = co_ok && p < pend;
+      rd[i] = buf_load16(rs_dy, ok ? (p * a.Cout + co0 + dseg * 8) * 2 : -1);
+    }
+    const bool pok = (it_p + xpx) < pend;
+    const int y0 = it_oy * a.stride - a.pad, x0 = it_ox * a.stride - a.pad;
+    const int base = ((it_b * a.H + y0) * a.W + x0) * a.Cin;
+#pragma unroll
+    for (int g = 0; g < NG; ++g) {
+      bool ok = pok && gok[g] && (unsigned)(y0 + gky[g]) < (unsigned)a.H && (unsigned)(x0 + gkx[g]) < (unsigned)a.W;
+      const int off = ok ? (base + gdelta[g]) * 2 : (int)0x80000000;
+#pragma unroll
+      for (int j = 0; j < UPT; ++j) rx[g * UPT + j] = buf_load16(rs_x, off + 64 * j);
+    }
+    it_p += WKP;
+    it_ox += adv_ox;
+    if (it_ox >= a.OW) { it_ox -= a.OW; ++it_oy; }
+    it_oy += adv_oy;
+    if (it_oy >= a.OH) { it_oy -= a.OH; ++it_b; }
+    it_b += adv_b;
+  };
+  auto lstore = [&](const u32x4 (&rd)[TC], const u32x4 (&rx)[WUN]) {
+#pragma unroll
+    for (int i = 0; i < TC; ++i) *reinterpret_cast<u32x4*>(&Ds[(dpx + DROWS * i) * D_LD + dseg * 16]) = rd[i];
+#pragma unroll
+    for (int u = 0; u < WUN; ++u) *reinterpret_cast<u32x4*>(&Xs[(u * WKP + xpx) * X_LD + xseg * 16]) = rx[u];
+  };
+
+  const int li = lane & 15, q = li >> 2, p4 = li & 3;
+  const int half16 = (lane >> 4) & 1;
+  const int h = lane >> 5;
+  const unsigned char* a_base = &Ds[(8 * h + q) * D_LD + (half16 * 16 + p4 * 4) * 2];
+  const unsigned char* b_base = &Xs[(wave * TU * WKP + 8 * h + q) * X_LD + (half16 * 16 + p4 * 4) * 2];
+
+  gload(rd[0], rx[0]);
+  lstore(rd[0], rx[0]);
+  __syncthreads();
+#pragma unroll
+  for (int j = 1; j < PF; ++j) gload(rd[j], rx[j]);
+  for (int64_t pb = p_begin; pb < p_end; pb += (int64_t)PF * WKP) {
+#pragma unroll
+    for (int j = 0; j < PF; ++j) {
+      gload(rd[j], rx[j]);
+#pragma unroll
+      for (int ks = 0; ks < WKP / 16; ++ks) {
+        bf16x8 af[TC], bfr[TU];
+#pragma unroll
+        for (int t = 0; t < TC; ++t) {
+          bf16x4 l = tr_read(a_base + 64 * t + (16 * ks) * D_LD), hh = tr_read(a_base + 64 * t + (16 * ks + 4) * D_LD);
+          af[t] = __builtin_shufflevector(l, hh, 0, 1, 2, 3, 4, 5, 6, 7);
+        }
+#pragma unroll
+        for (int u = 0; u < TU; ++u) {
+          const unsigned char* bp = b_base + u * WKP * X_LD;
+          bf16x4 l = tr_read(bp + (16 * ks) * X_LD), hh = tr_read(bp + (16 * ks + 4) * X_LD);
+          bfr[u] = __builtin_shufflevector(l, hh, 0, 1, 2, 3, 4, 5, 6, 7);
+        }
+#pragma unroll
+        for (int u = 0; u < TU; ++u)
+#pragma unroll
+          for (int t = 0; t < TC; ++t) acc[t][u] = __builtin_amdgcn_mfma_f32_32x32x16_bf16(af[t], bfr[u], acc[t][u], 0, 0, 0);
+      }
+      __syncthreads();
+      lstore(rd[(j + 1) % PF], rx[(j + 1) % PF]);
+      __syncthreads();
+    }
+  }
+  const int r = lane & 31;
+  const int taps = a.KH * a.KW;
+#pragma unroll
+  for (int u = 0; u < TU; ++u) {
+    const int uu = u0 + wave * TU + u;
+    if (uu >= a.units) continue;
+    const int tap = uu / cchunks;
+    const int ci = (uu - tap * cchunks) * 32 + r;
+#pragma unroll
+    for (int t = 0; t < TC; ++t) {
+#pragma unroll
+      for (int g = 0; g < 16; ++g) {
+        int co = co0 + 32 * t + (g & 3) + 8 * (g >> 2) + 4 * h;
+        if (co < a.Cout) {
+          float* const q = a.dw + (size_t)bz * a.slab + ((size_t)co * taps + tap) * a.Cin + ci;
+          if (a.slab) *q = acc[t][u][g];
+          else atomicAdd(q, acc[t][u][g]);
+        }
+      }
+    }
+  }
diff --git a/ws-mgmap_amd/wsmgmap/_abi.py b/ws-mgmap_amd/wsmgmap/_abi.py
--- a/ws-mgmap_amd/wsmgmap/_abi.py
+++ b/ws-mgmap_amd/wsmgmap/_abi.py
@@ -94,6 +94,8 @@
 _SIG["wsmg_conv2d_bwd_weight_bf16_plan"] = list(_SIG["wsmg_conv2d_bwd_weight_plan"])
 _SIG["wsmg_conv2d_bwd_weight_slabs"] = [c_p, c_p, c_p, c_i, c_l] + [c_i] * 11 + [c_p]
 _SIG["wsmg_conv2d_bwd_weight_bf16_slabs"] = list(_SIG["wsmg_conv2d_bwd_weight_slabs"])
+_SIG["wsmg_conv2d_bwd_pair_bf16_plan"] = [c_i] * 11 + [c_p, c_p, c_p]
+_SIG["wsmg_conv2d_bwd_pair_bf16"] = [c_p, c_p, c_p, c_p, c_p, c_i, c_l] + [c_i] * 11 + [c_p]
 _SIG["wsmg_weight_grad_reduce_oihw"] = [c_p, c_i, c_i, c_i, c_i, c_i, c_i, c_p, c_p]
 _SIG["wsmg_update_heads_fwd"] = [c_p] * 6 + [c_i] * 3 + [c_p] * 3 + [c_p]
 _SIG["wsmg_update_heads_bwd"] = [c_p] * 8 + [c_i] * 3 + [c_p] * 5 + [c_p]
diff --git a/ws-mgmap_amd/wsmgmap/debug.py b/ws-mgmap_amd/wsmgmap/debug.py
--- a/ws-mgmap_amd/wsmgmap/debug.py
+++ b/ws-mgmap_amd/wsmgmap/debug.py
@@ -17,6 +17,7 @@
     ("conv_into_cat", "WSMG_CONV_INTO_CAT", True, bool, "map_encoded / map_classified_linear write straight into their slices of the concatenation (round 6)"),
     ("strided_grads", "WSMG_STRIDED_GRADS", True, bool, "channel slices of a concatenation's gradient read in place"),
     ("wgrad_atomics", "WSMG_WGRAD_ATOMICS", False, bool, "weight gradients through float atomics instead of slabs + ordered reduce (not bit-reproducible)"),
+    ("conv_bwd_pair", "WSMG_CONV_BWD_PAIR", True, bool, "backward-data + weight gradient of the small generic-kernel layers as one launch (wsmg_conv2d_bwd_pair_bf16); 0: two launches"),
     ("conv_splitk", "WSMG_CONV_SPLITK", True, bool, "split-K for rollout-size layers"),
     ("rows_linear", "WSMG_ROWS_LINEAR", True, bool, "one-launch dense layers for <= 16 rows"),
     ("bev_fused", "WSMG_BEV_FUSED", True, bool, "scatter + rotation in one launch, plane-consuming fuse"),
diff --git a/ws-mgmap_amd/wsmgmap/ops/conv.py b/ws-mgmap_amd/wsmgmap/ops/conv.py
--- a/ws-mgmap_amd/wsmgmap/ops/conv.py
+++ b/ws-mgmap_amd/wsmgmap/ops/conv.py
@@ -80,6 +80,38 @@
     return out
 
 
+PAIR_MAX_WG_PER_CU = 6
+_cu_count = {}
+
+
+def _bwd_pair_plan(dims, device, limit=True):
+    nsplit, floats, wgs = ctypes.c_int(0), ctypes.c_longlong(0), ctypes.c_longlong(0)
+    rc = _abi.lib().wsmg_conv2d_bwd_pair_bf16_plan(*dims, ctypes.cast(ctypes.byref(nsplit), ctypes.c_void_p),
+                                                   ctypes.cast(ctypes.byref(floats), ctypes.c_void_p),
+                                                   ctypes.cast(ctypes.byref(wgs), ctypes.c_void_p))
+    if rc != 0:
+        return None
+    if limit:
+        cus = _cu_count.get(device.index)
+        if cus is None:
+            cus = _cu_count[device.index] = torch.cuda.get_device_properties(device).multi_processor_count
+        if wgs.value > PAIR_MAX_WG_PER_CU * cus:
+            return None
+    return nsplit.value, floats.value
+
+
+def _bwd_pair(x, dy, w_ihwo, dims, fl, Cin_w, plan):
+    B, H, W, Cin, Cout, KH, KW, stride, pad, OH, OW = dims
+    nsplit, floats = plan
+    dx = torch.empty_like(x)
+    ws = _wgrad_workspace(x.device, floats)
+    _launch("wsmg_conv2d_bwd_pair_bf16", 2.0 * fl, _p(dy), _p(w_ihwo), _p(dx), _p(x), _p(ws), nsplit, floats, *dims, _stream())
+    dw = torch.empty(Cout, Cin_w, KH, KW, device=x.device, dtype=torch.float32)
+    _launch("wsmg_weight_grad_reduce_oihw", 0.0, _p(ws), nsplit, Cout, Cin_w, KH, KW, Cin, _p(dw), _stream(),
+            prof_as="wsmg_conv2d_bwd_weight_bf16_slabs")
+    return dx, dw
+
+
 class ReluSink:
 
     def __init__(self):
@@ -155,14 +187,20 @@
             dy = dy.contiguous()
         dx = dw = db = None
         fl = 2.0 * B * OH * OW * Cout * Cin * KH * KW
-        if ctx.needs_input_grad[0]:
+        pair = None
+        if sfx and ctx.needs_input_grad[0] and ctx.needs_input_grad[1] and sw.conv_bwd_pair and not sw.wgrad_atomics:
+            pair = _bwd_pair_plan(dims, x.device)
+        if pair is not None:
+            dx, dw = _bwd_pair(x, dy, w_ihwo, tuple(dims), fl, Cin_w, pair)
+        elif ctx.needs_input_grad[0]:
             dx = torch.empty_like(x)
             if sfx:
                 _launch("wsmg_conv2d_bwd_data_bf16", fl, _p(dy), _p(w_ihwo), _p(dx), 0, *dims, _stream())
             else:
                 _launch("wsmg_conv2d_bwd_data", fl, _p(dy), _p(w_ihwo), _p(dx), *dims, _stream())
         if ctx.needs_input_grad[1]:
-            dw = _weight_grad(sfx, x, dy, dims, fl, Cin_w)
+            if pair is None:
+                dw = _weight_grad(sfx, x, dy, dims, fl, Cin_w)
             lo = ctx.lo_sink.take() if ctx.lo_sink is not None else None
             if lo is not None and lo.shape == dy.shape:
                 dw = dw + _weight_grad(sfx, x, lo, dims, fl, Cin_w)
diff --git a/ws-mgmap_amd/wsmgmap/ops/core.py b/ws-mgmap_amd/wsmgmap/ops/core.py
--- a/ws-mgmap_amd/wsmgmap/ops/core.py
+++ b/ws-mgmap_amd/wsmgmap/ops/core.py
@@ -74,7 +74,7 @@
 _prof = None
 
 def _prof_key(name):
-    return name.replace("_stats", "").replace("_slabs", "").replace("_ex", "")
+    return name.replace("_stats", "").replace("_slabs", "").replace("_ex", "").replace("_bwd_pair_bf16", "_bwd_weight_bf16")
 
 
 KERNEL_OF = {
```

Result: no change. 52440 (median of 6 runs) (+1.0%).
